# yosungho/LineTR

Hardware: AMD Instinct MI355X
Metric: line_descriptors_per_sec (higher is better)
Workload: dtype f32 in/out; GEMMs as 6 bf16-split MFMA products, fp32 accumulate (fp32-faithful); 1 GPU; cfg3: 64 pairs/GPU of 640x480, 200 lines/image -> 199 sub-lines x 21 tokens, d_model=256, seeded weights; pairs_per_gpu=64, collective=none

## Files before the change

include/linetr_hip.h:

```cpp
#ifndef LINETR_HIP_H
#define LINETR_HIP_H

#include <stdint.h>

#ifdef __cplusplus
extern "C" {
#endif

#define LINETR_ABI_VERSION 6

enum {
  LINETR_OK = 0,
  LINETR_E_ARG = -1,
  LINETR_E_HIP = -2,
  LINETR_E_WEIGHTS = -3,
  LINETR_E_ASSERT = -4,
  LINETR_E_WORKSPACE = -5,
  LINETR_E_CAPACITY = -6
};

typedef struct LinetrHandle LinetrHandle;

typedef struct {
  int32_t d_model;
  int32_t n_heads;
  int32_t d_inner;
  int32_t n_sig_layers;
  int32_t n_desc_layers;
  int32_t enc_channels[4];
  int32_t norm_height;
  int32_t norm_width;
  int32_t bn_batch_stats;
} LinetrModelConfig;

typedef struct {
  double sp[2];
  double ep[2];
  double length;
  double angle[2];
  int32_t first_sub;
  int32_t n_tok;
  int32_t n_sub;
  int32_t image;
  int32_t line_local;
  int32_t first_tok;
} LinetrLineRec;

typedef struct {
  float* klines;
  float* length;
  float* angles;
  float* sublines;
  float* pnt;
  float* mask;
  float* resp;
  float* angle_sub;
  float* desc;
  float* score;
  float* mat;
  const int32_t* h_cu_klines;
} LinetrTokens;


int linetr_abi_version(void);
const char* linetr_last_error(void);

int linetr_create(const LinetrModelConfig* cfg, int32_t n_tensors, const char* const* names,
                  const float* const* h_data, const int64_t* numel, int32_t device,
                  LinetrHandle** out);
void linetr_destroy(LinetrHandle* h);


int linetr_prefilter(const double* h_lines6, int32_t K, int32_t height, int32_t width, int32_t border,
                     double min_length, int32_t max_keylines, const double* h_valid_mask,
                     double token_distance, int32_t max_tokens, int32_t image_index, int32_t sub_base,
                     int32_t tok_base, LinetrLineRec* h_recs, int32_t capacity, int32_t* k_out, int32_t* n_out);

int linetr_prefilter_batch(const double* h_lines6, const int32_t* h_line_off, int32_t n_images, int32_t height,
                           int32_t width, int32_t border, double min_length, int32_t max_keylines,
                           const double* const* h_valid_masks, double token_distance, int32_t max_tokens,
                           int32_t n_threads, LinetrLineRec* h_recs, int32_t capacity, int32_t* h_cu_k,
                           int32_t* h_cu_n);

int32_t linetr_prefilter_tied_images(int32_t* h_images, int32_t capacity);

int linetr_pack_lines(const double* h_klines, const double* h_length, const double* h_angles, int32_t K,
                      double token_distance, int32_t max_tokens, int32_t image_index, int32_t sub_base,
                      int32_t tok_base, LinetrLineRec* h_recs, int32_t* n_out);


int64_t linetr_tokenize_workspace_bytes(int32_t n_images, int32_t height, int32_t width, int32_t N);

int linetr_tokenize(LinetrHandle* h, const LinetrLineRec* d_recs, int32_t K, int32_t N,
                    double token_distance, int32_t max_tokens, const float* d_dense_desc,
                    const float* d_dense_score, int32_t n_images, int32_t height, int32_t width,
                    int32_t clip_height, int32_t clip_width, int32_t align_corners, int32_t dense_is_nhwc,
                    LinetrTokens out, int32_t* d_sub2line, void* d_workspace, int64_t workspace_bytes, void* stream);

int64_t linetr_sample_descriptors_workspace_bytes(int32_t Hc, int32_t Wc, int32_t dense_is_nhwc);
int linetr_sample_descriptors(LinetrHandle* h, const float* d_points, int64_t n, const float* d_dense_desc, int32_t Hc,
                              int32_t Wc, int32_t align_corners, int32_t dense_is_nhwc, float* d_out, void* d_workspace,
                              int64_t workspace_bytes, void* stream);


int64_t linetr_forward_workspace_bytes(const LinetrHandle* h, int32_t N, int32_t max_tokens);

int linetr_forward(LinetrHandle* h, const LinetrTokens* tok, const int32_t* h_cu_sub, const int32_t* d_cu_sub,
                   int32_t n_images, int32_t max_tokens, float* d_line_desc, void* d_workspace,
                   int64_t workspace_bytes, void* stream);


int64_t linetr_bn_stats_floats(const LinetrHandle* h);
int64_t linetr_forward_train_workspace_bytes(const LinetrHandle* h, int32_t N, int32_t max_tokens);
int linetr_forward_train(LinetrHandle* h, const LinetrTokens* tok, const int32_t* h_cu_sub, const int32_t* d_cu_sub,
                         int32_t n_images, int32_t max_tokens, float momentum, float* d_bn_running, float* d_bn_batch,
                         float* d_line_desc, void* d_workspace, int64_t workspace_bytes, void* stream);

int64_t linetr_describe_workspace_bytes(const LinetrHandle* h, int32_t n_images, int32_t height, int32_t width,
                                        int32_t N, int64_t n_real_tokens);

int linetr_describe(LinetrHandle* h, const LinetrLineRec* d_recs, int32_t K, int32_t N, int64_t n_real_tokens,
                    const int32_t* h_cu_sub, const int32_t* d_cu_sub, int32_t n_images, double token_distance,
                    int32_t max_tokens, const float* d_dense_desc, const float* d_dense_score, int32_t height,
                    int32_t width, int32_t align_corners, int32_t dense_is_nhwc, LinetrTokens out,
                    int32_t* d_sub2line, float* d_line_desc, void* d_workspace, int64_t workspace_bytes,
                    void* stream);

int linetr_describe_submit(LinetrHandle* h, const LinetrLineRec* d_recs, int32_t K, int32_t N, int64_t n_real_tokens,
                           const int32_t* h_cu_sub, const int32_t* d_cu_sub, int32_t n_images, double token_distance,
                           int32_t max_tokens, const float* d_dense_desc, const float* d_dense_score, int32_t height,
                           int32_t width, int32_t align_corners, int32_t dense_is_nhwc, LinetrTokens out,
                           int32_t* d_sub2line, float* d_line_desc, void* d_workspace, int64_t workspace_bytes,
                           int32_t slot, int32_t n_slots, void* stream);
int32_t linetr_pipeline_max_slots(void);
int linetr_describe_join(LinetrHandle* h, int32_t slot, void* stream);


int64_t linetr_match_workspace_bytes(int32_t n_pairs, int64_t sum_n0n1, int64_t sum_k0k1, int64_t sum_k);

int linetr_match(LinetrHandle* h, int32_t n_pairs, const int32_t* h_dims, const float* d_desc0,
                 const int64_t* h_off_n0, const int32_t* d_sub2line0, const float* d_desc1,
                 const int64_t* h_off_n1, const int32_t* d_sub2line1, float nn_thresh, int32_t mutual,
                 float* d_dk, const int64_t* h_off_dk, int32_t* d_match01, const int64_t* h_off_k0,
                 void* d_workspace, int64_t workspace_bytes, void* stream);

int linetr_match_gathered(LinetrHandle* h, int32_t n_pairs, const int32_t* h_dims, const float* d_desc0,
                          const int64_t* h_off_n0, const int32_t* d_sub2line0, const int64_t* h_off_s0,
                          const float* d_desc1, const int64_t* h_off_n1, const int32_t* d_sub2line1,
                          const int64_t* h_off_s1, float nn_thresh, int32_t mutual, float* d_dk,
                          const int64_t* h_off_dk, int32_t* d_match01, const int64_t* h_off_k0, void* d_workspace,
                          int64_t workspace_bytes, void* stream);

int64_t linetr_match_distmat_workspace_bytes(int32_t n0, int32_t n1);
int linetr_match_distmat(LinetrHandle* h, const float* d_dist, int32_t n0, int32_t n1, float nn_thresh,
                         int32_t mutual, int32_t* d_match01, void* d_workspace, int64_t workspace_bytes,
                         void* stream);

int64_t linetr_match_distmat_f64_workspace_bytes(int32_t n0, int32_t n1);
int linetr_match_distmat_f64(LinetrHandle* h, const double* d_dist, int32_t n0, int32_t n1, double nn_thresh, int32_t mutual,
                             int32_t* d_match01, void* d_workspace, int64_t workspace_bytes, void* stream);

int64_t linetr_pool_distmat_workspace_bytes(int32_t k0, int32_t k1);
int linetr_pool_distmat(LinetrHandle* h, const float* d_dist, int32_t n0, int32_t n1, const int32_t* d_sub2line0, int32_t k0,
                        const int32_t* d_sub2line1, int32_t k1, float* d_dk, void* d_workspace, int64_t workspace_bytes,
                        void* stream);

int64_t linetr_pool_distmat_dense_workspace_bytes(int32_t k0, int32_t n0, int32_t k1, int32_t n1);
int linetr_pool_distmat_dense(LinetrHandle* h, const float* d_dist, int32_t n0, int32_t n1, const float* d_A0, int32_t k0,
                              const float* d_A1, int32_t k1, float* d_dk, void* d_workspace, int64_t workspace_bytes,
                              void* stream);

int linetr_match_points(LinetrHandle* h, const float* d_desc0_cn, int32_t n0, const float* d_desc1_cn,
                        int32_t n1, float nn_thresh, int32_t mutual, float* d_dist, int32_t* d_match01,
                        void* d_workspace, int64_t workspace_bytes, void* stream);

int64_t linetr_pair_tail_workspace_bytes(int32_t np0, int32_t np1, int32_t n0, int32_t k0, int32_t n1, int32_t k1);
int64_t linetr_pair_tail_output_bytes(int32_t np0, int32_t np1, int32_t k0, int32_t k1, int64_t* h_offsets);
int linetr_pair_tail(LinetrHandle* h, const float* d_pdesc0_cn, int32_t np0, const float* d_pdesc1_cn, int32_t np1, float nn_thresh_points,
                     const float* d_ldesc0, int32_t n0, const int32_t* d_sub2line0, int32_t k0, const float* d_ldesc1, int32_t n1,
                     const int32_t* d_sub2line1, int32_t k1, float nn_thresh_lines, int32_t mutual, void* h_pinned_out,
                     int64_t pinned_bytes, void* d_workspace, int64_t workspace_bytes, void* stream);


int64_t linetr_val_step_workspace_bytes(int32_t B, int32_t n);
int64_t linetr_val_step_output_bytes(int32_t B, int64_t* h_offsets);
int linetr_val_step(LinetrHandle* h, const float* d_desc0, int32_t n0, const float* d_desc1, int32_t n1, const float* d_assign, int32_t B,
                    double nn_thresh, int32_t mutual, float* d_row_pos, float* d_row_neg, int32_t* d_match01, void* h_pinned_out,
                    int64_t pinned_bytes, void* d_workspace, int64_t workspace_bytes, void* stream);

int linetr_assign_from_matches(LinetrHandle* h, const int32_t* d_lmatches, int32_t B, int32_t M, int32_t n, float* d_assign, void* stream);


enum { LINETR_COORD_F32 = 0, LINETR_COORD_F64 = 1 };
int64_t linetr_gt_assign_workspace_bytes(int32_t B, int32_t n0, int32_t n1);
int linetr_gt_assign(LinetrHandle* h, int32_t coord_type, const void* d_lines0, int32_t n0, const void* d_lines1, int32_t n1,
                     const double* d_H, int32_t B, const int32_t* d_count0, const int32_t* d_count1, double thres_reprojected,
                     double thres_angdiff, double min_overlap_ratio, int32_t pad, float* d_assign, int32_t* d_lmatches, int32_t M,
                     int32_t* d_found, uint8_t* d_match_dir, void* d_overlap_dir, void* d_proj0, void* d_proj1, void* d_workspace,
                     int64_t workspace_bytes, void* stream);


int linetr_superpoint_heads(LinetrHandle* h, const float* d_score_logits, const float* d_desc_raw, int32_t B,
                            int32_t Hc, int32_t Wc, float* d_dense_score, float* d_dense_desc_nhwc,
                            float* d_dense_desc_nchw, void* stream);


int64_t linetr_superpoint_keypoints_workspace_bytes(int32_t B, int32_t H, int32_t W, int32_t cap_per_image);
int linetr_superpoint_keypoints(LinetrHandle* h, const float* d_dense_score, int32_t B, int32_t H, int32_t W, int32_t nms_radius,
                                float keypoint_threshold, int32_t remove_borders, int32_t max_keypoints, int32_t cap_per_image,
                                float* d_keypoints, float* d_scores, int32_t* d_cu_kp, int32_t* d_found, void* d_workspace,
                                int64_t workspace_bytes, void* stream);

int64_t linetr_point_descriptors_workspace_bytes(int32_t B, int32_t Hc, int32_t Wc, int32_t dense_is_nhwc);
int linetr_point_descriptors(LinetrHandle* h, const float* d_keypoints, const int32_t* d_cu_kp, int32_t B, int64_t n_total,
                             const float* d_dense_desc, int32_t Hc, int32_t Wc, int32_t align_corners, int32_t dense_is_nhwc,
                             float* d_desc_cn, void* d_workspace, int64_t workspace_bytes, void* stream);


enum { LINETR_PREC_F32 = 0, LINETR_PREC_BF16X3 = 1, LINETR_PREC_BF16X6 = 2, LINETR_PREC_F16X3 = 3 };
int linetr_set_precision(LinetrHandle* h, int32_t mode);
int linetr_get_precision(const LinetrHandle* h);


int linetr_debug_posenc(LinetrHandle* h, int32_t which, const float* d_in0, const float* d_in1, const float* d_in2,
                           int64_t rows, float* d_out, void* stream);

int linetr_debug_gemm(LinetrHandle* h, const float* d_A, int32_t lda, const float* d_W, const float* d_bias,
                      const float* d_residual, float* d_Y, int32_t ldy, int32_t M, int32_t N, int32_t K,
                      int32_t act, int32_t cache_weights, void* stream);

#define LINETR_GEMM_TILE_WS 100
typedef struct {
  const float* A;   int32_t lda;
  const float* A2;  int32_t lda2;  int32_t K1;
  const float* W;
  const float* bias;
  const float* R;
  float* Y;         int32_t ldy;
  int32_t M, N, K, act;
  int32_t groups;   int64_t gA, gY;
  int32_t norm;     const float* gamma;  const float* beta;  const float* add2;  float eps;
  int32_t via_row_norm;
  int32_t tile;
} LinetrGemmCase;
int linetr_debug_gemm_case(LinetrHandle* h, const LinetrGemmCase* c, int32_t* tile_used, void* stream);

int linetr_debug_sig_attention(LinetrHandle* h, int32_t kernel, int32_t layer, const float* d_in, int32_t ld_in,
                               const int32_t* h_cu_sub, int32_t n_images, float* d_msg, int32_t* kernel_used, void* stream);

int linetr_debug_tok_mlp(LinetrHandle* h, int32_t variant, const float* d_pnt, const float* d_score, int64_t rows_word,
                         const float* d_sublines, const float* d_resp, const float* d_angle, int64_t rows_line,
                         float* d_out_word, float* d_out_line, int32_t max_blocks, int32_t* variant_used, void* stream);

int linetr_debug_cls_pool(LinetrHandle* h, int32_t kernel, const LinetrLineRec* d_recs, int32_t K, const int32_t* d_sub2line,
                          int32_t N, int32_t T, const float* d_cpnt, const float* d_a4, int64_t first_pad, int32_t n_images,
                          const float* d_map, int32_t dense_is_nhwc, int32_t Hc, int32_t Wc, int32_t align_corners,
                          const float* d_desc_dense, float* d_pooled, int32_t* kernel_used, void* stream);

#ifdef LINETR_EXPERIMENTS
int64_t linetr_st_bytes(int64_t rows, int32_t K);
int linetr_debug_to_st(LinetrHandle* h, const float* d_X, int32_t ld, int32_t rows, int32_t K, void* d_st, void* stream);
int linetr_debug_from_st(LinetrHandle* h, const void* d_st, int32_t rows, int32_t K, float* d_X, int32_t ld, void* stream);
int linetr_debug_gemm_st(LinetrHandle* h, const void* d_A1, int32_t K1, const void* d_A2, int32_t K2, const void* d_W,
                         const float* d_bias, const void* d_R, void* d_Yst, float* d_Y, int32_t ldy, int32_t M, int32_t N,
                         int32_t act, void* stream);
int linetr_debug_pairnet_stamps(LinetrHandle* h, unsigned long long* d_buf);
#endif

int linetr_allgather_desc(void* nccl_comm, const void* d_slab, void* d_out, int64_t slab_bytes, void* stream);

int linetr_set_allgather_fn(void* nccl_allgather_fn);

int linetr_pack_slab(const float* d_line_desc, int32_t N, const int32_t* d_cu_n, const int32_t* d_cu_k, int32_t n_images,
                     const int32_t* d_sub2line, int32_t n_images_cap, int32_t rows_cap, int32_t zero_tail, float* d_slab,
                     void* stream);


typedef struct {
  const char* name;
  int32_t calls;
  float ms;
  double flops;
  double bytes;
} LinetrProfileEntry;
int linetr_set_profiling(LinetrHandle* h, int32_t on);
int linetr_get_profile(LinetrHandle* h, LinetrProfileEntry* out, int32_t max_entries, int32_t* n_out);

#ifdef __cplusplus
}
#endif
#endif
```

linetr_amd/_native.py:

```python
from __future__ import annotations

import ctypes as C
import os

import numpy as np

_HERE = os.path.dirname(os.path.abspath(__file__))
LIB_PATH = os.path.join(_HERE, "csrc", "liblinetr_hip.so")
EXPERIMENTS_LIB_PATH = os.path.join(os.path.dirname(_HERE), "experiments", "liblinetr_hip_experiments.so")

E_ASSERT = -4


class ModelConfig(C.Structure):
    _fields_ = [("d_model", C.c_int32), ("n_heads", C.c_int32), ("d_inner", C.c_int32),
                ("n_sig_layers", C.c_int32), ("n_desc_layers", C.c_int32), ("enc_channels", C.c_int32 * 4),
                ("norm_height", C.c_int32), ("norm_width", C.c_int32), ("bn_batch_stats", C.c_int32)]


class LineRec(C.Structure):
    _fields_ = [("sp", C.c_double * 2), ("ep", C.c_double * 2), ("length", C.c_double),
                ("angle", C.c_double * 2), ("first_sub", C.c_int32), ("n_tok", C.c_int32),
                ("n_sub", C.c_int32), ("image", C.c_int32), ("line_local", C.c_int32), ("first_tok", C.c_int32)]


REC_DTYPE = np.dtype([("sp", "<f8", 2), ("ep", "<f8", 2), ("length", "<f8"), ("angle", "<f8", 2),
                      ("first_sub", "<i4"), ("n_tok", "<i4"), ("n_sub", "<i4"), ("image", "<i4"),
                      ("line_local", "<i4"), ("first_tok", "<i4")])
assert REC_DTYPE.itemsize == C.sizeof(LineRec) == 80


class Tokens(C.Structure):
    _fields_ = [(k, C.c_void_p) for k in ("klines", "length", "angles", "sublines", "pnt", "mask", "resp",
                                          "angle_sub", "desc", "score", "mat", "h_cu_klines")]


class GemmCase(C.Structure):
    _fields_ = [("A", C.c_void_p), ("lda", C.c_int32), ("A2", C.c_void_p), ("lda2", C.c_int32), ("K1", C.c_int32),
                ("W", C.c_void_p), ("bias", C.c_void_p), ("R", C.c_void_p), ("Y", C.c_void_p), ("ldy", C.c_int32),
                ("M", C.c_int32), ("N", C.c_int32), ("K", C.c_int32), ("act", C.c_int32), ("groups", C.c_int32),
                ("gA", C.c_int64), ("gY", C.c_int64), ("norm", C.c_int32), ("gamma", C.c_void_p), ("beta", C.c_void_p),
                ("add2", C.c_void_p), ("eps", C.c_float), ("via_row_norm", C.c_int32), ("tile", C.c_int32)]


class ProfileEntry(C.Structure):
    _fields_ = [("name", C.c_char_p), ("calls", C.c_int32), ("ms", C.c_float), ("flops", C.c_double),
                ("bytes", C.c_double)]


_libs = {}


def lib(path=None):
    import torch
    path = os.path.abspath(path or os.environ.get("LINETR_LIB", LIB_PATH))
    if path in _libs:
        return _libs[path]
    if not os.path.exists(path):
        raise RuntimeError(
            f"{path} is missing: the HIP extension has not been built (run `python -m linetr_amd.build`). "
            "linetr_amd has no CPU fallback.")
    L = C.CDLL(path)
    vp, i32, i64, f64, f32 = C.c_void_p, C.c_int32, C.c_int64, C.c_double, C.c_float
    L.linetr_abi_version.restype = i32
    L.linetr_last_error.restype = C.c_char_p
    L.linetr_create.argtypes = [C.POINTER(ModelConfig), i32, C.POINTER(C.c_char_p), C.POINTER(vp), C.POINTER(i64), i32,
                                C.POINTER(vp)]
    L.linetr_destroy.argtypes = [vp]
    L.linetr_destroy.restype = None
    L.linetr_prefilter.argtypes = [vp, i32, i32, i32, i32, f64, i32, vp, f64, i32, i32, i32, i32, vp, i32, C.POINTER(i32),
                                   C.POINTER(i32)]
    L.linetr_prefilter_batch.argtypes = [vp, vp, i32, i32, i32, i32, f64, i32, vp, f64, i32, i32, vp, i32, vp, vp]
    L.linetr_prefilter_tied_images.argtypes = [vp, i32]
    L.linetr_prefilter_tied_images.restype = i32
    L.linetr_pack_lines.argtypes = [vp, vp, vp, i32, f64, i32, i32, i32, i32, vp, C.POINTER(i32)]
    L.linetr_describe_workspace_bytes.argtypes = [vp, i32, i32, i32, i32, i64]
    L.linetr_describe_workspace_bytes.restype = i64
    L.linetr_describe.argtypes = [vp, vp, i32, i32, i64, vp, vp, i32, f64, i32, vp, vp, i32, i32, i32, i32, Tokens, vp, vp,
                                  vp, i64, vp]
    L.linetr_describe_submit.argtypes = [vp, vp, i32, i32, i64, vp, vp, i32, f64, i32, vp, vp, i32, i32, i32, i32, Tokens, vp, vp,
                                         vp, i64, i32, i32, vp]
    L.linetr_describe_join.argtypes = [vp, i32, vp]
    L.linetr_pipeline_max_slots.argtypes = []
    L.linetr_tokenize_workspace_bytes.argtypes = [i32, i32, i32, i32]
    L.linetr_tokenize_workspace_bytes.restype = i64
    L.linetr_tokenize.argtypes = [vp, vp, i32, i32, f64, i32, vp, vp, i32, i32, i32, i32, i32, i32, i32, Tokens, vp, vp, i64, vp]
    L.linetr_forward_workspace_bytes.argtypes = [vp, i32, i32]
    L.linetr_forward_workspace_bytes.restype = i64
    L.linetr_forward.argtypes = [vp, C.POINTER(Tokens), vp, vp, i32, i32, vp, vp, i64, vp]
    L.linetr_bn_stats_floats.argtypes = [vp]
    L.linetr_bn_stats_floats.restype = i64
    L.linetr_forward_train_workspace_bytes.argtypes = [vp, i32, i32]
    L.linetr_forward_train_workspace_bytes.restype = i64
    L.linetr_forward_train.argtypes = [vp, C.POINTER(Tokens), vp, vp, i32, i32, f32, vp, vp, vp, vp, i64, vp]
    L.linetr_match_workspace_bytes.argtypes = [i32, i64, i64, i64]
    L.linetr_match_workspace_bytes.restype = i64
    L.linetr_match.argtypes = [vp, i32, vp, vp, vp, vp, vp, vp, vp, f32, i32, vp, vp, vp, vp, vp, i64, vp]
    L.linetr_match_gathered.argtypes = [vp, i32, vp, vp, vp, vp, vp, vp, vp, vp, vp, f32, i32, vp, vp, vp, vp, vp, i64, vp]
    L.linetr_match_points.argtypes = [vp, vp, i32, vp, i32, f32, i32, vp, vp, vp, i64, vp]
    L.linetr_match_distmat.argtypes = [vp, vp, i32, i32, f32, i32, vp, vp, i64, vp]
    L.linetr_match_distmat_workspace_bytes.argtypes = [i32, i32]
    L.linetr_match_distmat_workspace_bytes.restype = i64
    L.linetr_match_distmat_f64.argtypes = [vp, vp, i32, i32, f64, i32, vp, vp, i64, vp]
    L.linetr_match_distmat_f64_workspace_bytes.argtypes = [i32, i32]
    L.linetr_match_distmat_f64_workspace_bytes.restype = i64
    L.linetr_pair_tail_workspace_bytes.argtypes = [i32, i32, i32, i32, i32, i32]
    L.linetr_pair_tail_workspace_bytes.restype = i64
    L.linetr_pair_tail_output_bytes.argtypes = [i32, i32, i32, i32, vp]
    L.linetr_pair_tail_output_bytes.restype = i64
    L.linetr_pair_tail.argtypes = [vp, vp, i32, vp, i32, f32, vp, i32, vp, i32, vp, i32, vp, i32, f32, i32, vp, i64, vp, i64, vp]
    L.linetr_val_step_workspace_bytes.argtypes = [i32, i32]
    L.linetr_val_step_workspace_bytes.restype = i64
    L.linetr_val_step_output_bytes.argtypes = [i32, vp]
    L.linetr_val_step_output_bytes.restype = i64
    L.linetr_val_step.argtypes = [vp, vp, i32, vp, i32, vp, i32, f64, i32, vp, vp, vp, vp, i64, vp, i64, vp]
    L.linetr_assign_from_matches.argtypes = [vp, vp, i32, i32, i32, vp, vp]
    L.linetr_gt_assign_workspace_bytes.argtypes = [i32, i32, i32]
    L.linetr_gt_assign_workspace_bytes.restype = i64
    L.linetr_gt_assign.argtypes = [vp, i32, vp, i32, vp, i32, vp, i32, vp, vp, f64, f64, f64, i32, vp, vp, i32, vp, vp, vp, vp, vp, vp,
                                   i64, vp]
    L.linetr_superpoint_heads.argtypes = [vp, vp, vp, i32, i32, i32, vp, vp, vp, vp]
    L.linetr_superpoint_keypoints_workspace_bytes.argtypes = [i32, i32, i32, i32]
    L.linetr_superpoint_keypoints_workspace_bytes.restype = i64
    L.linetr_superpoint_keypoints.argtypes = [vp, vp, i32, i32, i32, i32, f32, i32, i32, i32, vp, vp, vp, vp, vp, i64, vp]
    L.linetr_point_descriptors_workspace_bytes.argtypes = [i32, i32, i32, i32]
    L.linetr_point_descriptors_workspace_bytes.restype = i64
    L.linetr_point_descriptors.argtypes = [vp, vp, vp, i32, i64, vp, i32, i32, i32, i32, vp, vp, i64, vp]
    L.linetr_set_precision.argtypes = [vp, i32]
    L.linetr_get_precision.argtypes = [vp]
    L.linetr_debug_posenc.argtypes = [vp, i32, vp, vp, vp, i64, vp, vp]
    L.linetr_debug_gemm.argtypes = [vp, vp, i32, vp, vp, vp, vp, i32, i32, i32, i32, i32, i32, vp]
    L.linetr_debug_gemm_case.argtypes = [vp, C.POINTER(GemmCase), vp, vp]
    L.linetr_debug_sig_attention.argtypes = [vp, i32, i32, vp, i32, vp, i32, vp, vp, vp]
    L.linetr_debug_tok_mlp.argtypes = [vp, i32, vp, vp, i64, vp, vp, vp, i64, vp, vp, i32, vp, vp]
    L.linetr_debug_cls_pool.argtypes = [vp, i32, vp, i32, vp, i32, i32, vp, vp, i64, i32, vp, i32, i32, i32, i32, vp, vp, vp, vp]
    if hasattr(L, "linetr_debug_gemm_st"):
        L.linetr_st_bytes.argtypes = [i64, i32]
        L.linetr_st_bytes.restype = i64
        L.linetr_debug_to_st.argtypes = [vp, vp, i32, i32, i32, vp, vp]
        L.linetr_debug_from_st.argtypes = [vp, vp, i32, i32, vp, i32, vp]
        L.linetr_debug_gemm_st.argtypes = [vp, vp, i32, vp, i32, vp, vp, vp, vp, vp, i32, i32, i32, i32, vp]
        L.linetr_debug_pairnet_stamps.argtypes = [vp, vp]
    L.linetr_allgather_desc.argtypes = [vp, vp, vp, i64, vp]
    L.linetr_set_allgather_fn.argtypes = [vp]
    L.linetr_pack_slab.argtypes = [vp, i32, vp, vp, i32, vp, i32, i32, i32, vp, vp]
    L.linetr_sample_descriptors_workspace_bytes.argtypes = [i32, i32, i32]
    L.linetr_sample_descriptors_workspace_bytes.restype = i64
    L.linetr_sample_descriptors.argtypes = [vp, vp, i64, vp, i32, i32, i32, i32, vp, vp, i64, vp]
    L.linetr_pool_distmat_workspace_bytes.argtypes = [i32, i32]
    L.linetr_pool_distmat_workspace_bytes.restype = i64
    L.linetr_pool_distmat.argtypes = [vp, vp, i32, i32, vp, i32, vp, i32, vp, vp, i64, vp]
    L.linetr_pool_distmat_dense_workspace_bytes.argtypes = [i32, i32, i32, i32]
    L.linetr_pool_distmat_dense_workspace_bytes.restype = i64
    L.linetr_pool_distmat_dense.argtypes = [vp, vp, i32, i32, vp, i32, vp, i32, vp, vp, i64, vp]
    L.linetr_set_profiling.argtypes = [vp, i32]
    L.linetr_get_profile.argtypes = [vp, C.POINTER(ProfileEntry), i32, C.POINTER(i32)]
    if L.linetr_abi_version() != 6:
        raise RuntimeError("liblinetr_hip.so ABI version mismatch")
    _libs[path] = L
    return L


EXPORTS = ["linetr_abi_version", "linetr_last_error", "linetr_create", "linetr_destroy", "linetr_prefilter",
           "linetr_prefilter_batch", "linetr_prefilter_tied_images", "linetr_pack_lines", "linetr_tokenize_workspace_bytes", "linetr_tokenize", "linetr_forward_workspace_bytes",
           "linetr_forward", "linetr_bn_stats_floats", "linetr_forward_train_workspace_bytes", "linetr_forward_train", "linetr_describe_workspace_bytes", "linetr_describe", "linetr_describe_submit", "linetr_describe_join", "linetr_pipeline_max_slots", "linetr_match_workspace_bytes", "linetr_match", "linetr_match_gathered", "linetr_match_points",
           "linetr_match_distmat", "linetr_match_distmat_workspace_bytes", "linetr_match_distmat_f64", "linetr_match_distmat_f64_workspace_bytes", "linetr_pair_tail_workspace_bytes", "linetr_pair_tail_output_bytes", "linetr_pair_tail", "linetr_val_step_workspace_bytes", "linetr_val_step_output_bytes", "linetr_val_step", "linetr_assign_from_matches", "linetr_gt_assign_workspace_bytes", "linetr_gt_assign", "linetr_superpoint_heads", "linetr_superpoint_keypoints_workspace_bytes", "linetr_superpoint_keypoints",
           "linetr_point_descriptors_workspace_bytes", "linetr_point_descriptors", "linetr_set_precision", "linetr_get_precision", "linetr_debug_posenc", "linetr_debug_gemm", "linetr_debug_gemm_case", "linetr_debug_sig_attention", "linetr_debug_tok_mlp", "linetr_debug_cls_pool", "linetr_allgather_desc", "linetr_set_allgather_fn", "linetr_pack_slab", "linetr_sample_descriptors_workspace_bytes",
           "linetr_sample_descriptors", "linetr_pool_distmat_workspace_bytes", "linetr_pool_distmat", "linetr_pool_distmat_dense_workspace_bytes", "linetr_pool_distmat_dense", "linetr_set_profiling", "linetr_get_profile"]


EXPERIMENT_EXPORTS = ["linetr_st_bytes", "linetr_debug_to_st", "linetr_debug_from_st", "linetr_debug_gemm_st", "linetr_debug_pairnet_stamps"]


class NativeError(RuntimeError):
    pass


def check(code: int, L=None):
    if code == 0:
        return
    msg = (L if L is not None else lib()).linetr_last_error().decode("utf-8", "replace")
    if code == E_ASSERT:
        raise AssertionError(msg)
    raise NativeError(f"liblinetr_hip error {code}: {msg}")


def np_ptr(a: np.ndarray):
    return a.ctypes.data_as(C.c_void_p)
```

linetr_amd/csrc/linetr_net.hip:

```cpp
#include <algorithm>
#include <array>
#include <numeric>
#include <set>

#include "lt_handle.h"
#include "lt_gemm.h"
#include "lt_gemm_split.h"
#include "lt_gemm_split16.h"
#include "lt_st_image.h"
#include "lt_gemm_small.h"
#include "lt_model.h"
#include "lt_attn.h"
#include "lt_attn_fused.h"
#include "lt_gemm_ws.h"
#include "lt_tokmlp.h"
#include "lt_token.h"
#include "lt_bntrain.h"

using namespace lt;

namespace {

const char* gemm_class_name(int precision, int tile, const GemmArgs& g, int groups) {
  static const auto names = [] {
    const char* kind[4] = {"gemm_f32", "gemm_bf16x3", "gemm_bf16x6", "gemm_f16x3"};
    std::array<std::array<std::string, (int)SplitTile::count>, 4> n;
    for (int p = 0; p < 4; ++p)
      for (int t = 0; t < (p ? (int)SplitTile::count : (int)F32Tile::count); ++t)
        n[p][t] = std::string(kind[p]) + "_" + (p ? tile_name((SplitTile)t) : tile_name((F32Tile)t));
    return n;
  }();
  const std::string& name = names[precision][tile];
  static const bool by_shape = LT_XENV("LINETR_PROFILE_SHAPES") != nullptr;
  if (!by_shape) return name.c_str();
  static std::mutex mu;
  static std::set<std::string> shapes;
  char buf[160];
  snprintf(buf, sizeof buf, "%s[M=%d,N=%d,K=%d,g=%d]", name.c_str(), g.M, g.N, g.K, groups);
  std::lock_guard<std::mutex> lock(mu);
  return shapes.insert(buf).first->c_str();
}

struct GemmA { const float* p; int ld; const float* p2 = nullptr; int ld2 = 0, K1 = 0; };
struct GemmY { float* p; int ld; };
struct GemmGroups { int n, N; int64_t gA, gY; };

struct NormSpec {
  int mode = 0;
  const float* gamma = nullptr;
  const float* beta = nullptr;
  const float* add2 = nullptr;
  float eps = 0.f;
};

#ifdef LINETR_EXPERIMENTS
int x_gemm(LinetrHandle*, hipStream_t, SplitGemmArgs& sa, const GemmW& w, int groups, const NormSpec*, double fl, double by, bool& done);
int x_split_weights(LinetrHandle* H, std::vector<GemmWSpec>& weights);
int64_t x_ws_bytes(const LinetrHandle* h, int N);
#endif

int gemm_args(const GemmW& w, int M, const GemmA& A, const GemmY& Y, int act, const float* R, const GemmGroups* grp,
              const NormSpec* ns, GemmArgs& g) {
  const int groups = grp ? grp->n : 1, N = grp ? grp->N : w.rows;
  if (A.p2 && (A.K1 <= 0 || A.K1 >= w.K)) return fail(LINETR_E_ARG, "gemm: split point K1 = %d outside (0, K = %d)", A.K1, w.K);
  if ((int64_t)N * groups > w.rows) return fail(LINETR_E_ARG, "gemm: %d groups of %d rows exceed the weight's %d", groups, N, w.rows);
  if (groups > 1 && (R || ns)) return fail(LINETR_E_ARG, "gemm: a grouped launch takes no residual and no row normalisation");
  g = GemmArgs{};
  g.A = A.p; g.lda = A.ld; g.A2 = A.p2; g.lda2 = A.ld2; g.K1 = A.K1;
  g.W = w.W; g.ldw = w.K; g.bias = w.b; g.R = R; g.ldr = Y.ld; g.Y = Y.p; g.ldy = Y.ld;
  g.M = M; g.N = N; g.K = w.K; g.act = act;
  if (grp) { g.gA = grp->gA; g.gW = (int64_t)N * w.K; g.gBias = N; g.gY = grp->gY; }
  if (ns) { g.norm = ns->mode; g.gamma = ns->gamma; g.beta = ns->beta; g.add2 = ns->add2; g.ldadd2 = D; g.eps = ns->eps; }
  return LINETR_OK;
}

bool gemm_ws_able(const LinetrHandle* h, const GemmArgs& g, const GemmW& w, int groups, const NormSpec* fused_norm) {
  return h->precision == LINETR_PREC_BF16X6 && groups == 1 && !g.A2 && !g.R && !fused_norm && w.st &&
         gemm_ws_can(g.N, g.K, g.lda, g.ldy, g.act);
}
bool gemm_ws_takes(const LinetrHandle* h, const GemmArgs& g, const GemmW& w, int groups, const NormSpec* fused_norm) {
  return gemm_ws_able(h, g, w, groups, fused_norm) && gemm_ws_fits(g.M, g.N, g.K, g.lda, g.ldy, g.act) && !LT_XENV("LINETR_NO_GEMM_WS");
}

struct GemmForce { int tile = -1; int* used = nullptr; bool launch = true; };

int run_gemm(LinetrHandle* h, hipStream_t st, const GemmW& w, int M, const GemmA& A, const GemmY& Y, int act, const float* R = nullptr,
             const GemmGroups* grp = nullptr, const NormSpec* fused_norm = nullptr, const GemmForce* force = nullptr) {
  GemmArgs g;
  if (int e = gemm_args(w, M, A, Y, act, R, grp, fused_norm, g)) return e;
  const int groups = grp ? grp->n : 1;
  const int forced = force ? force->tile : -1;
  const bool launch = !force || force->launch;
  auto report = [&](int tile) { if (force && force->used) *force->used = tile; };
  const double fl = 2.0 * M * (double)g.N * g.K * groups;
  const double by = 4.0 * groups * ((double)M * g.K + (double)g.N * g.K + (double)M * g.N);
  if (h->precision == LINETR_PREC_F32) {
    if (forced >= (int)F32Tile::count) return fail(LINETR_E_ARG, "gemm: the f32 mode has no tile %d", forced);
    if (fused_norm) return fail(LINETR_E_ARG, "gemm: the f32 kernels have no fused row normalisation");
    const F32Tile tile = f32_tile_launched(g, forced < 0 ? f32_tile(g, groups) : (F32Tile)forced);
    report((int)tile);
    if (!launch) return LINETR_OK;
    ProfScope ps(h, st, gemm_class_name(LINETR_PREC_F32, (int)tile, g, groups), fl, by);
    return gemm_launch(g, groups, tile, st);
  }
  SplitGemmArgs sa;
  sa.g = g;
#ifdef LINETR_EXPERIMENTS
  if (!force) {
    bool done = false;
    if (int e = x_gemm(h, st, sa, w, groups, fused_norm, fl, by, done); e || done) return e;
  }
#endif
  if (forced == LINETR_GEMM_TILE_WS && !gemm_ws_able(h, g, w, groups, fused_norm))
    return fail(LINETR_E_ARG, "gemm: the weight-stationary kernel runs act(A[M,128] W[256,128]^T + b) in bf16x6 only, act none / ReLU");
  if (forced == LINETR_GEMM_TILE_WS || (forced < 0 && gemm_ws_takes(h, g, w, groups, fused_norm))) {
    report(LINETR_GEMM_TILE_WS);
    if (!launch) return LINETR_OK;
    WsGemmArgs a;
    a.A = A.p; a.lda = A.ld; a.Wst = w.st; a.bias = w.b ? w.b : h->zeros; a.Y = Y.p; a.ldy = Y.ld; a.M = M; a.act = act;
    ProfScope ps(h, st, "gemm_bf16x6_ws64x256", fl, by);
    return gemm_ws_launch(a, st);
  }
  const int pl = h->precision == LINETR_PREC_BF16X6 ? 3 : 2;
  SplitTile tile;
  if (forced >= (int)SplitTile::count) return fail(LINETR_E_ARG, "gemm: no split tile %d", forced);
  if (forced >= 0) tile = (SplitTile)forced;
  else if (int e = pick_split_tile(g, groups, pl, tile)) return e;
  if (int e = split_tile_launched(g, groups, pl, tile)) return e;
  report((int)tile);
  if (!launch) return LINETR_OK;
  ProfScope ps(h, st, gemm_class_name(h->precision, (int)tile, g, groups), fl, by);
  switch (h->precision) {
    case LINETR_PREC_BF16X3: sa.Wsp = w.s2; sa.gWsp = g.gW * 4; return gemm_split_launch<2>(sa, groups, tile, st);
    case LINETR_PREC_F16X3: sa.Wsp = w.h2; sa.gWsp = g.gW * 4; return gemm_split_launch<2, 1>(sa, groups, tile, st);
    default: sa.Wsp = w.s3; sa.gWsp = g.gW * 6; return gemm_split_launch<3>(sa, groups, tile, st);
  }
}

bool gemm_norm_fuses(const LinetrHandle* h, const GemmW& w, int M, const GemmA& A, const float* R, float* Y) {
  GemmArgs g;
  return !LT_XENV("LINETR_NO_FUSED_NORM") && h->precision != LINETR_PREC_F32 && !LT_XENV("LINETR_GEMM_TILE") &&
         !gemm_args(w, M, A, {Y, D}, ACT_NONE, R, nullptr, nullptr, g) &&
         split_tile(g, 1, h->precision == LINETR_PREC_BF16X6 ? 3 : 2) == SplitTile::t128x256;
}

int row_norm(LinetrHandle* h, hipStream_t st, const float* x, int M, const NormSpec& ns, float* Y) {
  ProfScope ps(h, st, "row_norm", 0, (double)M * D * (ns.add2 ? 12 : 8));
  hipLaunchKernelGGL(row_norm_kernel, dim3(cdiv(M, 4)), dim3(256), 0, st, x, M, ns.mode == 2 ? 1 : 0, ns.gamma, ns.beta,
                     ns.add2, ns.eps, Y);
  LT_LAUNCH_CHECK();
  return 0;
}

int run_gemm_norm(LinetrHandle* h, hipStream_t st, const GemmW& w, int M, const GemmA& A, const float* R, float* tmp, float* Y,
                  const NormSpec& ns) {
  if (w.rows != D) return fail(LINETR_E_ARG, "gemm_norm: the weight has %d rows, not %d", w.rows, D);
  if (gemm_norm_fuses(h, w, M, A, R, Y)) return run_gemm(h, st, w, M, A, {Y, D}, ACT_NONE, R, nullptr, &ns);
  if (int e = run_gemm(h, st, w, M, A, {tmp, D}, ACT_NONE, R)) return e;
  return row_norm(h, st, tmp, M, ns, Y);
}

struct SplitOffsets { int64_t s2, s3, h2, st = -1; };
SplitOffsets split_offsets(int64_t rows, int K, bool with_st, int64_t& off) {
  SplitOffsets o;
  o.s2 = off; off += align_up(rows * K * 4, 256);
  o.s3 = off; off += align_up(rows * K * 6, 256);
  o.h2 = off; off += align_up(rows * K * 4, 256);
  if (with_st) { off = align_up(off, 1024); o.st = off; off += st_bytes(rows, K); }
  return o;
}

void split_copies(GemmW& w, unsigned char* base, const SplitOffsets& o, bool make, hipStream_t st) {
  w.s2 = base + o.s2; w.s3 = base + o.s3; w.h2 = base + o.h2;
  w.st = o.st >= 0 ? base + o.st : nullptr;
  if (!make) return;
  const dim3 grid((unsigned)cdiv((int)((int64_t)w.rows * w.K / 4), 256));
  hipLaunchKernelGGL(split_rows_kernel<2>, grid, dim3(256), 0, st, w.W, base + o.s2, (int64_t)w.rows, w.K);
  hipLaunchKernelGGL(split_rows_kernel<3>, grid, dim3(256), 0, st, w.W, base + o.s3, (int64_t)w.rows, w.K);
  hipLaunchKernelGGL((split_rows_kernel<2, 1>), grid, dim3(256), 0, st, w.W, base + o.h2, (int64_t)w.rows, w.K);
  if (o.st >= 0) {
    const int64_t thr = st_row_blocks(w.rows) * (w.K / 16) * 32;
    hipLaunchKernelGGL(to_st_kernel, dim3((unsigned)((thr + 255) / 256)), dim3(256), 0, st, w.W, w.K, w.rows, w.K / 16, base + o.st);
  }
}

}

int lt::make_split_copies(LinetrHandle* H, std::vector<GemmWSpec> weights) {
#ifdef LINETR_EXPERIMENTS
  if (int e = x_split_weights(H, weights)) return e;
#endif
  int64_t total = 0;
  std::vector<SplitOffsets> at;
  for (auto& s : weights) at.push_back(split_offsets(s.w->rows, s.w->K, s.st && s.w->rows % 16 == 0 && s.w->K % 32 == 0, total));
  LT_HIP(hipMalloc((void**)&H->split_arena, total));
  LT_HIP(hipMalloc((void**)&H->zeros, 4096 * sizeof(float)));
  LT_HIP(hipMemset(H->zeros, 0, 4096 * sizeof(float)));
  for (size_t i = 0; i < weights.size(); ++i) split_copies(*weights[i].w, H->split_arena, at[i], true, 0);
  LT_LAUNCH_CHECK();
  LT_HIP(hipDeviceSynchronize());
  return LINETR_OK;
}


namespace {
int k2s_table(const LinetrTokens& out, int n_images, int K, int N, const int32_t* h_cu_sub, K2sTable& tab, const char* who) {
  tab = K2sTable{};
  if (!out.mat) return 0;
  if (n_images > K2S_MAX_IMAGES) return fail(LINETR_E_ARG, "%s: mat_klines2sublines is written for calls of up to %d images", who, K2S_MAX_IMAGES);
  if (n_images == 1) {
    for (int i = 0; i < K2S_MAX_IMAGES; ++i) tab.img[i] = K2sImage{0, N, 0};
    return 0;
  }
  if (!out.h_cu_klines || !h_cu_sub) return fail(LINETR_E_ARG, "%s: mat_klines2sublines of several images needs the host prefix sums of key-lines and sub-lines", who);
  if (out.h_cu_klines[n_images] != K) return fail(LINETR_E_ARG, "%s: h_cu_klines does not end at K", who);
  int64_t off = 0;
  for (int i = 0; i < n_images; ++i) {
    const int ki = out.h_cu_klines[i + 1] - out.h_cu_klines[i], ni = h_cu_sub[i + 1] - h_cu_sub[i];
    if (ki < 0 || ni < 0) return fail(LINETR_E_ARG, "%s: prefix sums not monotone", who);
    tab.img[i] = K2sImage{off, ni, h_cu_sub[i]};
    off += (int64_t)ki * ni;
  }
  return 0;
}

int nhwc_map(LinetrHandle* h, hipStream_t st, const float* dense_desc, int dense_is_nhwc, int n_images, int P, float* buf,
             const float*& nhwc) {
  nhwc = dense_desc;
  if (dense_is_nhwc) return LINETR_OK;
  ProfScope ps(h, st, "nchw_to_nhwc", 0, 2.0 * n_images * P * D * 4);
  hipLaunchKernelGGL(nchw_to_nhwc_kernel, dim3(cdiv(P, 64), D / 64, n_images), dim3(256), 0, st, dense_desc, buf, D, P);
  LT_LAUNCH_CHECK();
  nhwc = buf;
  return LINETR_OK;
}

struct TokenFront {
  const LinetrLineRec* recs; int K, N; double td; int T;
  const float *dense_desc, *dense_score;
  int n_images, height, width, align_corners, dense_is_nhwc;
  double clip_x, clip_y;
  float *sublines, *resp, *angle_sub;
  int* s2l_g;
  float* nhwc_buf;
  bool map_always;
  double tokenize_bytes;
  float *cpnt = nullptr, *cscore = nullptr; int n_pad_images = 0; int64_t first_pad = 0;
};
int token_front(LinetrHandle* h, hipStream_t st, const TokenFront& a, const LinetrTokens& out, const K2sTable& k2s, int32_t* d_sub2line,
                const float*& nhwc) {
  {
    ProfScope ps(h, st, "line_fill", 0, (double)a.K * 80 + (double)a.N * 8);
    hipLaunchKernelGGL(line_fill_kernel, dim3(cdiv(a.K, 256)), dim3(256), 0, st, a.recs, a.K, a.clip_x, a.clip_y, out.klines, out.length,
                       out.angles, a.s2l_g, d_sub2line);
    LT_LAUNCH_CHECK();
  }
  {
    ProfScope ps(h, st, "tokenize", 0, a.tokenize_bytes);
    hipLaunchKernelGGL(tokenize_kernel, dim3(a.N + cdiv(a.n_pad_images, 64) + (out.mat ? a.K : 0)), dim3(64), 0, st, a.recs, a.s2l_g, a.N,
                       a.td, a.T, a.height, a.width, a.clip_x, a.clip_y, a.dense_score, a.sublines, out.pnt, out.mask, a.resp, a.angle_sub,
                       out.score, a.cpnt, a.cscore, a.n_pad_images, a.first_pad, out.mat, k2s);
    LT_LAUNCH_CHECK();
  }
  const int Hc = a.height / 8, Wc = a.width / 8;
  nhwc = nullptr;
  if (a.map_always || out.desc)
    if (int e = nhwc_map(h, st, a.dense_desc, a.dense_is_nhwc, a.n_images, Hc * Wc, a.nhwc_buf, nhwc)) return e;
  if (out.desc) {
    const int64_t ntok = (int64_t)a.N * a.T;
    ProfScope ps(h, st, "sample_desc", 0, (double)ntok * D * 4 * 2);
    hipLaunchKernelGGL(sample_desc_kernel, dim3((unsigned)((ntok + 3) / 4)), dim3(256), 0, st, out.pnt, a.s2l_g, a.recs, ntok, a.T, nhwc,
                       Hc, Wc, a.align_corners, out.desc);
    LT_LAUNCH_CHECK();
  }
  return LINETR_OK;
}
}

extern "C" int64_t linetr_tokenize_workspace_bytes(int32_t n_images, int32_t height, int32_t width, int32_t N) {
  const int64_t P = (int64_t)(height / 8) * (width / 8);
  return align_up(n_images * P * D * 4, 256) + align_up((int64_t)std::max(N, 1) * 4, 256) + 256;
}

extern "C" int linetr_tokenize(LinetrHandle* h, const LinetrLineRec* d_recs, int32_t K, int32_t N, double td,
                               int32_t T, const float* d_dense_desc, const float* d_dense_score, int32_t n_images,
                               int32_t height, int32_t width, int32_t clip_height, int32_t clip_width, int32_t align_corners,
                               int32_t dense_is_nhwc, LinetrTokens out, int32_t* d_sub2line, void* d_ws, int64_t ws_bytes,
                               void* stream) {
  if (K <= 0 || N <= 0) return LINETR_OK;
  if (clip_height <= 0) clip_height = height;
  if (clip_width <= 0) clip_width = width;
  if (!d_recs || !d_dense_score || !out.sublines || !out.pnt || !out.mask || !out.resp || !out.angle_sub ||
      !out.score || (out.desc && !d_dense_desc))
    return fail(LINETR_E_ARG, "tokenize: null pointer");
  if (T < 1 || T > 4096 || height % 8 || width % 8) return fail(LINETR_E_ARG, "tokenize: bad max_tokens / image size");
  if (out.mat && n_images != 1) return fail(LINETR_E_ARG, "tokenize: mat_klines2sublines of several images: use linetr_describe (it has the sub-line prefix sums)");
  K2sTable k2s;
  if (int e = k2s_table(out, n_images, K, N, nullptr, k2s, "tokenize")) return e;
  if (ws_bytes < linetr_tokenize_workspace_bytes(n_images, height, width, N))
    return fail(LINETR_E_WORKSPACE, "tokenize: workspace too small");
  hipStream_t st = (hipStream_t)stream;
  if (h) LT_HIP(hipSetDevice(h->device));
  const int64_t P = (int64_t)(height / 8) * (width / 8);
  TokenFront f{d_recs, K, N, td, T, d_dense_desc, d_dense_score, n_images, height, width, align_corners, dense_is_nhwc,
               (double)clip_width - 0.6, (double)clip_height - 0.6, out.sublines, out.resp, out.angle_sub};
  f.nhwc_buf = (float*)d_ws;
  f.s2l_g = (int*)((char*)d_ws + align_up(n_images * P * D * 4, 256));
  f.map_always = false;
  f.tokenize_bytes = (double)N * T * 16;
  const float* nhwc;
  return token_front(h, st, f, out, k2s, d_sub2line, nhwc);
}

extern "C" int64_t linetr_sample_descriptors_workspace_bytes(int32_t Hc, int32_t Wc, int32_t dense_is_nhwc) {
  return dense_is_nhwc ? 0 : align_up((int64_t)Hc * Wc * D * 4, 256);
}

extern "C" int linetr_sample_descriptors(LinetrHandle* h, const float* d_points, int64_t n, const float* d_dense_desc, int32_t Hc,
                                         int32_t Wc, int32_t align_corners, int32_t dense_is_nhwc, float* d_out, void* d_ws,
                                         int64_t ws_bytes, void* stream) {
  if (n < 0 || Hc <= 0 || Wc <= 0) return fail(LINETR_E_ARG, "sample_descriptors: bad shape");
  if (n == 0) return LINETR_OK;
  if (!d_points || !d_dense_desc || !d_out) return fail(LINETR_E_ARG, "sample_descriptors: null pointer");
  if (ws_bytes < linetr_sample_descriptors_workspace_bytes(Hc, Wc, dense_is_nhwc) || (!dense_is_nhwc && !d_ws))
    return fail(LINETR_E_WORKSPACE, "sample_descriptors: workspace too small");
  hipStream_t st = (hipStream_t)stream;
  if (h) LT_HIP(hipSetDevice(h->device));
  const float* nhwc;
  if (int e = nhwc_map(h, st, d_dense_desc, dense_is_nhwc, 1, Hc * Wc, (float*)d_ws, nhwc)) return e;
  ProfScope ps(h, st, "sample_desc", 0, (double)n * D * 4 * 2);
  hipLaunchKernelGGL(sample_desc_kernel, dim3((unsigned)((n + 3) / 4)), dim3(256), 0, st, d_points, (const int*)nullptr,
                     (const LinetrLineRec*)nullptr, n, 1, nhwc, Hc, Wc, align_corners, d_out);
  LT_LAUNCH_CHECK();
  return LINETR_OK;
}

extern "C" int64_t linetr_point_descriptors_workspace_bytes(int32_t B, int32_t Hc, int32_t Wc, int32_t dense_is_nhwc) {
  return dense_is_nhwc ? 0 : align_up((int64_t)std::max(B, 0) * std::max(Hc, 0) * std::max(Wc, 0) * D * 4, 256);
}

extern "C" int linetr_point_descriptors(LinetrHandle* h, const float* d_keypoints, const int32_t* d_cu_kp, int32_t B, int64_t n_total,
                                        const float* d_dense_desc, int32_t Hc, int32_t Wc, int32_t align_corners, int32_t dense_is_nhwc,
                                        float* d_desc_cn, void* d_ws, int64_t ws_bytes, void* stream) {
  if (B < 0 || n_total < 0 || Hc <= 0 || Wc <= 0 || n_total > INT32_MAX) return fail(LINETR_E_ARG, "point_descriptors: bad shape");
  if (B == 0 || n_total == 0) return LINETR_OK;
  if (!d_keypoints || !d_cu_kp || !d_dense_desc || !d_desc_cn) return fail(LINETR_E_ARG, "point_descriptors: null pointer");
  if (ws_bytes < linetr_point_descriptors_workspace_bytes(B, Hc, Wc, dense_is_nhwc) || (!dense_is_nhwc && !d_ws))
    return fail(LINETR_E_WORKSPACE, "point_descriptors: workspace too small");
  hipStream_t st = (hipStream_t)stream;
  if (h) LT_HIP(hipSetDevice(h->device));
  LT_HIP(allow_dynamic_lds<sp_kp_desc_kernel>((int)KP_DESC_LDS));
  const float* nhwc;
  if (int e = nhwc_map(h, st, d_dense_desc, dense_is_nhwc, B, Hc * Wc, (float*)d_ws, nhwc)) return e;
  ProfScope ps(h, st, "sp_kp_desc", 0, (double)n_total * D * 4 * 5);
  hipLaunchKernelGGL(sp_kp_desc_kernel, dim3((unsigned)((n_total + KP_DESC_N - 1) / KP_DESC_N + B)), dim3(256), KP_DESC_LDS, st, d_keypoints,
                     d_cu_kp, B, nhwc, Hc, Wc, align_corners, d_desc_cn);
  LT_LAUNCH_CHECK();
  return LINETR_OK;
}


namespace {
constexpr int SIG_FOLD_MAX_ROWS = 960;
struct FwdWs {
  float* act[2][4];
  float *pooled, *att, *fc, *o, *f1, *f2, *lpos, *zA, *zB, *qkv, *msgp, *msg, *hid;
  float *zqA, *zqB;
  int* cu;
  char* x = nullptr;
  int64_t total;
};
FwdWs fwd_layout(const LinetrHandle* h, int N, int64_t rows, int n_images, char* base) {
  const LinetrModelConfig& c = h->cfg;
  FwdWs w;
  int64_t off = 0;
  auto take = [&](int64_t floats) { float* p = (float*)(base + off); off += align_up(floats * 4, 256); return p; };
  for (int i = 0; i < 4; ++i) w.act[ENC_WORD][i] = take(rows * c.enc_channels[i]);
  w.pooled = take((int64_t)N * HEADS * POOLW);
  w.att = take((int64_t)N * D); w.fc = take((int64_t)N * D); w.o = take((int64_t)N * D);
  w.f1 = take((int64_t)N * c.d_inner); w.f2 = take((int64_t)N * D);
  for (int i = 0; i < 4; ++i) w.act[ENC_LINE][i] = take((int64_t)N * c.enc_channels[i]);
  w.lpos = take((int64_t)N * D);
  w.zA = take((int64_t)N * D); w.zB = take((int64_t)N * D);
  w.qkv = take((int64_t)N * 3 * D); w.msgp = take((int64_t)N * D); w.msg = take((int64_t)N * D);
  w.hid = take((int64_t)N * 2 * D);
  const int64_t nq = N <= SIG_FOLD_MAX_ROWS ? (int64_t)N * 4 * D : 0;
  w.zqA = take(nq); w.zqB = take(nq);
  w.cu = (int*)take(n_images + 1);
#ifdef LINETR_EXPERIMENTS
  w.x = base + off; off += x_ws_bytes(h, N);
#endif
  w.total = off;
  return w;
}
}

extern "C" int64_t linetr_forward_workspace_bytes(const LinetrHandle* h, int32_t N, int32_t T) {
  if (!h) return -1;
  return fwd_layout(h, std::max(N, 1), (int64_t)std::max(N, 1) * T, std::max(N, 1), nullptr).total;
}

namespace {
enum {
  CUT_TOKENS = 0,
  CUT_MLP = 1,
  CUT_POOL = 2,
  CUT_SENTENCE = 3,
  CUT_SIG0 = 4
};
struct PipeStages {
  hipStream_t stream[LinetrHandle::PIPE_STREAMS];
  hipEvent_t ev[LinetrHandle::PIPE_STREAMS - 1];
  int cut[LinetrHandle::PIPE_STREAMS - 1];
  int n_cuts = 0, next = 0;
};
int pipe_boundary(PipeStages* p, int pos, hipStream_t& st) {
  if (!p || p->next >= p->n_cuts || p->cut[p->next] != pos) return LINETR_OK;
  LT_HIP(hipEventRecord(p->ev[p->next], st));
  LT_HIP(hipStreamWaitEvent(p->stream[p->next + 1], p->ev[p->next], 0));
  st = p->stream[++p->next];
  return LINETR_OK;
}

struct TokenStage {
  const float *pnt = nullptr, *score = nullptr, *desc = nullptr;
  const float *cpnt = nullptr, *cscore = nullptr, *nhwc = nullptr;
  const LinetrLineRec* recs = nullptr;
  const int* sub2line_g = nullptr;
  int64_t rows = 0;
  int64_t first_pad = 0;
  int Hc = 0, Wc = 0, align_corners = 0;
  const BnTrain* bn = nullptr;
  PipeStages* pipe = nullptr;
};

bool fused_mlp_enabled(const LinetrModelConfig& c) { return c.enc_channels[1] == 64 && c.enc_channels[2] == 128; }

int mlp123_rows_per_wave(int64_t rows) {
  const int64_t waves = 256 * 4;
  return (int)std::max<int64_t>(cdiv((int)cdiv((int)rows, (int)waves), 32) * 32, 32);
}

double attn_flops(const int32_t* h_cu, int n_images) {
  double fl = 0;
  for (int i = 0; i < n_images; ++i) { const double n = h_cu[i + 1] - h_cu[i]; fl += 2.0 * 2.0 * n * n * D; }
  return fl;
}

struct EncCall {
  int which;
  const float *p0, *p1, *p2;
  int64_t rows;
  float* const* act;
};
constexpr struct { int in, in_bytes; const char *tok_mlp, *mlp123; } ENC_KIND[2] = {{3, 12, "tok_mlp_bf16x6", "mlp123"},
                                                                                   {5, 28, "line_mlp_bf16x6", "mlp123_line"}};

struct EncNorm { float cx, cy, scale; };
EncNorm enc_norm(const LinetrModelConfig& c) {
  return {c.norm_width / 2.f, c.norm_height / 2.f, (float)std::max(c.norm_width, c.norm_height) * 0.7f};
}

template <bool RELU>
int enc_layer1(LinetrHandle* h, hipStream_t st, const EncCall& c, float* out) {
  const PosEncoder& E = h->enc[c.which];
  const EncNorm n = enc_norm(h->cfg);
  const dim3 grid((unsigned)cdiv((int)(c.rows * 8), 256));
  if (c.which == ENC_WORD)
    hipLaunchKernelGGL(word_mlp1_kernel<RELU>, grid, dim3(256), 0, st, c.p0, c.p1, c.rows, n.cx, n.cy, n.scale, E.W1, E.b1, out);
  else
    hipLaunchKernelGGL(line_mlp1_kernel<RELU>, grid, dim3(256), 0, st, c.p0, c.p1, c.p2, (int)c.rows, n.cx, n.cy, n.scale, E.W1, E.b1, out);
  LT_LAUNCH_CHECK();
  return LINETR_OK;
}

int enc_mlp123(LinetrHandle* h, hipStream_t st, const EncCall& c, float* out) {
  const PosEncoder& E = h->enc[c.which];
  const EncNorm n = enc_norm(h->cfg);
  const int rpw = mlp123_rows_per_wave(c.rows);
  const dim3 grid((unsigned)cdiv((int)cdiv((int)c.rows, rpw), 4));
  if (c.which == ENC_WORD)
    hipLaunchKernelGGL(mlp123_kernel<true>, grid, dim3(256), 0, st, c.p0, c.p1, c.p2, c.rows, rpw, n.cx, n.cy, n.scale, E.W1, E.b1,
                       E.W2.W, E.W2.b, E.W3.W, E.W3.b, out);
  else
    hipLaunchKernelGGL(mlp123_kernel<false>, grid, dim3(256), 0, st, c.p0, c.p1, c.p2, c.rows, rpw, n.cx, n.cy, n.scale, E.W1, E.b1,
                       E.W2.W, E.W2.b, E.W3.W, E.W3.b, out);
  LT_LAUNCH_CHECK();
  return LINETR_OK;
}

TokMlpArgs tok_mlp_args(const LinetrHandle* h, const EncCall& c) {
  const PosEncoder& E = h->enc[c.which];
  const EncNorm n = enc_norm(h->cfg);
  TokMlpArgs a;
  a.p0 = c.p0; a.p1 = c.p1; a.p2 = c.p2; a.rows = c.rows; a.cx = n.cx; a.cy = n.cy; a.scale = n.scale;
  a.W1 = E.W1; a.b1 = E.b1; a.W2st = E.W2.st; a.b2 = E.W2.b; a.W3st = E.W3.st; a.b3 = E.W3.b; a.W4st = E.W4.st; a.b4 = E.W4.b;
  a.Y = c.act[3]; a.ldy = h->cfg.enc_channels[3];
  return a;
}

int pos_encoder(LinetrHandle* h, hipStream_t st, const EncCall& c, bool tok_mlp) {
  const int *ch = h->cfg.enc_channels, e0 = ch[0], e1 = ch[1], e2 = ch[2], e3 = ch[3];
  const PosEncoder& E = h->enc[c.which];
  const auto& kind = ENC_KIND[c.which];
  const int64_t rows = c.rows;
  int e;
  if (tok_mlp) {
    ProfScope ps(h, st, kind.tok_mlp, 2.0 * rows * (kind.in * e0 + e0 * e1 + e1 * e2 + e2 * e3), (double)rows * (kind.in_bytes + 4 * e3));
    return tok_mlp_launch(tok_mlp_args(h, c), c.which == ENC_WORD, st);
  }
  if (fused_mlp_enabled(h->cfg)) {
    ProfScope ps(h, st, kind.mlp123, 2.0 * rows * (kind.in * e0 + e0 * e1 + e1 * e2), (double)rows * (kind.in_bytes + 4 * e2));
    if ((e = enc_mlp123(h, st, c, c.act[2]))) return e;
  } else {
    {
      ProfScope ps(h, st, "mlp_first", 2.0 * rows * kind.in * e0, (double)rows * (kind.in_bytes + 4 * e0));
      if ((e = enc_layer1<true>(h, st, c, c.act[0]))) return e;
    }
    if ((e = run_gemm(h, st, E.W2, (int)rows, {c.act[0], e0}, {c.act[1], e1}, ACT_RELU))) return e;
    if ((e = run_gemm(h, st, E.W3, (int)rows, {c.act[1], e1}, {c.act[2], e2}, ACT_RELU))) return e;
  }
  return run_gemm(h, st, E.W4, (int)rows, {c.act[2], e2}, {c.act[3], e3}, ACT_RELU);
}

int pos_encoder_bn(LinetrHandle* h, hipStream_t st, const EncCall& c, const BnTrain& bt, int64_t& off) {
  const PosEncoder& E = h->enc[c.which];
  const GemmW* const W[4] = {nullptr, &E.W2, &E.W3, &E.W4};
  const int* ch = h->cfg.enc_channels;
  int e;
  for (int i = 0; i < 4; ++i) {
    e = i == 0 ? enc_layer1<false>(h, st, c, c.act[0])
               : run_gemm(h, st, *W[i], (int)c.rows, {c.act[i - 1], ch[i - 1]}, {c.act[i], ch[i]}, ACT_NONE);
    if (e) return e;
    const int layer = 4 * c.which + i;
    if ((e = bn_train_layer(st, bt, c.act[i], c.rows, ch[i], ch[i], h->bn_g[layer], h->bn_b[layer], off))) return e;
    off += 2 * ch[i];
  }
  return LINETR_OK;
}

enum { TOKV_WORD = 0, TOKV_LINE = 1, TOKV_DUAL = 2, TOKV_SEQ = 3, TOKV_CHAIN = 4 };
struct TokMlpPlan { bool word, line; int both; };
bool tok_mlp_has_images(const PosEncoder& E) { return E.W2.st && E.W3.st && E.W4.st; }
TokMlpPlan tok_mlp_plan(const LinetrHandle* h, int64_t rows_word, int64_t rows_line) {
  const int* ch = h->cfg.enc_channels;
  const bool ok = fused_mlp_enabled(h->cfg) && h->precision == LINETR_PREC_BF16X6 && ch[0] == 32 && ch[1] == 64 && ch[2] == 128 && ch[3] == 256 &&
                  !LT_XENV("LINETR_NO_TOKMLP");
  TokMlpPlan p;
  p.word = ok && tok_mlp_has_images(h->enc[ENC_WORD]);
  p.line = ok && tok_mlp_has_images(h->enc[ENC_LINE]);
  p.both = !(p.word && p.line && rows_word > 0 && rows_line > 0) ? -1 : tok_mlp_dual_fits(rows_word, rows_line) ? TOKV_DUAL : TOKV_SEQ;
  return p;
}

int pos_encoders(LinetrHandle* h, hipStream_t& st, const TokenStage& ts, const float* sublines, const float* resp,
                 const float* angle_sub, int N, FwdWs& w) {
  const LinetrModelConfig& c = h->cfg;
  const int e0 = c.enc_channels[0], e1 = c.enc_channels[1], e2 = c.enc_channels[2], e3 = c.enc_channels[3];
  const EncCall word{ENC_WORD, ts.cpnt ? ts.cpnt : ts.pnt, ts.cpnt ? ts.cscore : ts.score, nullptr, ts.rows, w.act[ENC_WORD]};
  const EncCall line{ENC_LINE, sublines, resp, angle_sub, N, w.act[ENC_LINE]};
  const int64_t rows = ts.rows;
  int e;
  const TokMlpPlan plan = tok_mlp_plan(h, rows, N);
  if (ts.bn) {
    int64_t off = 0;
    if ((e = pos_encoder_bn(h, st, word, *ts.bn, off))) return e;
    if ((e = pos_encoder_bn(h, st, line, *ts.bn, off))) return e;
  } else if (plan.both >= 0) {
    ProfScope ps(h, st, "pos_mlp_dual_bf16x6", 2.0 * rows * (3 * e0 + e0 * e1 + e1 * e2 + e2 * e3) + 2.0 * N * (5 * e0 + e0 * e1 + e1 * e2 + e2 * e3),
                 (double)rows * (12 + 4 * e3) + (double)N * (28 + 4 * e3));
    if ((e = tok_mlp_launch_dual(tok_mlp_args(h, word), tok_mlp_args(h, line), st))) return e;
  } else {
    if ((e = pos_encoder(h, st, word, plan.word))) return e;
    if ((e = pos_encoder(h, st, line, plan.line))) return e;
  }
  return run_gemm(h, st, h->lW5, N, {w.act[ENC_LINE][3], e3}, {w.lpos, D}, ACT_NONE);
}

enum { POOLK_DENSE = 0, POOLK_ONLINE = 1, POOLK_ONLINE_REV = 2, POOLK_SPLIT4 = 3 };
int cls_pool_plan(bool online, int N) { return !online ? POOLK_DENSE : N <= 2048 ? POOLK_SPLIT4 : POOLK_ONLINE_REV; }

int cls_pool_launch(LinetrHandle* h, hipStream_t st, int kernel, const TokenStage& ts, int n_images, int N, int T, const float* a4,
                    float* pooled) {
  const int64_t rows = ts.rows;
  if (kernel != POOLK_DENSE) {
    const double tap_bytes = std::min((double)n_images * ts.Hc * ts.Wc * D * 4, (double)rows * D * 4 * 4);
    ProfScope ps(h, st, "cls_pool_online", 2.0 * rows * (2.0 * HEADS * D * 2), tap_bytes + (double)rows * D * 4 + (double)N * HEADS * POOLW * 4);
    if (kernel == POOLK_SPLIT4)
      hipLaunchKernelGGL(cls_pool_online_kernel<4>, dim3(N), dim3(256), 0, st, ts.recs, ts.sub2line_g, ts.cpnt,
                         a4, ts.first_pad, N, T, ts.nhwc, ts.Hc, ts.Wc, ts.align_corners, h->pool, pooled, 0);
    else
      hipLaunchKernelGGL(cls_pool_online_kernel<1>, dim3(cdiv(N, 4)), dim3(256), 0, st, ts.recs, ts.sub2line_g, ts.cpnt,
                         a4, ts.first_pad, N, T, ts.nhwc, ts.Hc, ts.Wc, ts.align_corners, h->pool, pooled, kernel == POOLK_ONLINE_REV ? 1 : 0);
    LT_LAUNCH_CHECK();
  } else {
    ProfScope ps(h, st, "cls_pool", 2.0 * rows * (2.0 * HEADS * D * 2), (double)rows * D * 8);
    hipLaunchKernelGGL(cls_pool_kernel, dim3(N), dim3(256), HEADS * (T + 1) * sizeof(float), st, ts.desc, a4, T, h->pool, pooled);
    LT_LAUNCH_CHECK();
  }
  return LINETR_OK;
}

int cls_pooling(LinetrHandle* h, hipStream_t& st, const TokenStage& ts, int n_images, int N, int T, FwdWs& w) {
  if (int e = cls_pool_launch(h, st, cls_pool_plan(ts.cpnt != nullptr, N), ts, n_images, N, T, w.act[ENC_WORD][3], w.pooled)) return e;
  const GemmGroups heads{HEADS, DH, POOLW, DH};
  return run_gemm(h, st, h->Watt, N, {w.pooled, HEADS * POOLW}, {w.att, D}, ACT_NONE, nullptr, &heads);
}

int sentence(LinetrHandle* h, hipStream_t& st, int N, FwdWs& w) {
  const LinetrModelConfig& c = h->cfg;
  int e;
  {
    NormSpec ns; ns.mode = 1; ns.gamma = h->ln1g; ns.beta = h->ln1b; ns.eps = 1e-6f;
    if ((e = run_gemm_norm(h, st, h->Wfc, N, {w.att, D}, nullptr, w.fc, w.o, ns))) return e;
  }
  if ((e = run_gemm(h, st, h->Wf1, N, {w.o, D}, {w.f1, c.d_inner}, ACT_GELU))) return e;
  NormSpec ns; ns.mode = 1; ns.gamma = h->ln2g; ns.beta = h->ln2b; ns.add2 = w.lpos; ns.eps = 1e-6f;
  return run_gemm_norm(h, st, h->Wf2, N, {w.f1, c.d_inner}, w.o, w.f2, w.zA, ns);
}

enum { SIGK_F32 = 0, SIGK_SMALL = 1, SIGK_SPLIT4 = 2, SIGK_SPLIT8 = 3, SIGK_FUSED = 4 };
struct SigAttnPlan {
  int attn;
  bool fold_next, fused;
  int kernel() const { return fused ? SIGK_FUSED : attn; }
};
SigAttnPlan sig_attn_plan(const LinetrHandle* h, int n_images, int N, int max_n) {
  SigAttnPlan p;
  const bool small_attn = h->precision != LINETR_PREC_F32 && (int64_t)n_images * HEADS * cdiv(max_n, 256) < 64;
  p.attn = h->precision == LINETR_PREC_F32 ? SIGK_F32 : small_attn ? SIGK_SMALL : max_n <= 128 ? SIGK_SPLIT4 : SIGK_SPLIT8;
  p.fold_next = small_attn && N <= SIG_FOLD_MAX_ROWS && !LT_XENV("LINETR_NO_SIG_FOLD");
  p.fused = !p.fold_next && !LT_XENV("LINETR_NO_FUSED_QKV_ATTN") && h->precision == LINETR_PREC_BF16X6 && max_n <= 256 &&
            (int64_t)n_images * HEADS >= 128;
  return p;
}

int sig_attention(LinetrHandle* h, hipStream_t st, int kernel, const float* qkv, int ldq, const int* cu_dev, int n_images, int N,
                  int max_n, double fl, float* msg) {
  if (kernel == SIGK_F32) {
    ProfScope ps(h, st, "sig_attn", fl, (double)N * D * 16);
    hipLaunchKernelGGL(sig_attn_kernel, dim3(n_images, HEADS, cdiv(max_n, ATT_QT)), dim3(256), 0, st, qkv, cu_dev, msg);
  } else {
    ProfScope ps(h, st, "sig_attn_bf16x6", fl, (double)N * D * 16);
    if (kernel == SIGK_SMALL)
      hipLaunchKernelGGL(sig_attn_small_kernel, dim3(n_images, HEADS, cdiv(max_n, 32)), dim3(256), 0, st, qkv, cu_dev, msg, ldq);
    else if (kernel == SIGK_SPLIT4)
      hipLaunchKernelGGL(sig_attn_split_kernel<4>, dim3(n_images, HEADS, cdiv(max_n, ATT_QT)), dim3(256), 0, st, qkv, cu_dev, msg);
    else
      hipLaunchKernelGGL(sig_attn_split_kernel<8>, dim3(n_images, HEADS, cdiv(max_n, 256)), dim3(512), 0, st, qkv, cu_dev, msg);
  }
  LT_LAUNCH_CHECK();
  return LINETR_OK;
}

int sig_qkv_attention(LinetrHandle* h, hipStream_t st, const SigLayer& S, const float* z, const int* cu_dev, int n_images, int N,
                      double attn_fl, float* msg) {
  LT_HIP(allow_dynamic_lds<sig_qkv_attn_kernel>(FQA_LDS));
  ProfScope ps(h, st, "sig_qkv_attn_bf16x6", 2.0 * N * 3.0 * D * D + attn_fl, (double)N * D * 8);
  hipLaunchKernelGGL(sig_qkv_attn_kernel, dim3(n_images, HEADS), dim3(512), FQA_LDS, st, z, S.Wqkv.st, S.Wqkv.b,
                     cu_dev, msg);
  LT_LAUNCH_CHECK();
  return LINETR_OK;
}

int sig_network(LinetrHandle* h, hipStream_t& st, const TokenStage& ts, const int32_t* h_cu, const int* cu_dev, int n_images, int N,
                float* d_line_desc, FwdWs& w) {
  const LinetrModelConfig& c = h->cfg;
  int max_n = 0;
  for (int i = 0; i < n_images; ++i) max_n = std::max(max_n, h_cu[i + 1] - h_cu[i]);
  int e;
  const double attn_fl = attn_flops(h_cu, n_images);
  const int64_t sig_bn_off = 4 * (int64_t)(c.enc_channels[0] + c.enc_channels[1] + c.enc_channels[2] + c.enc_channels[3]);
  const SigAttnPlan plan = sig_attn_plan(h, n_images, N, max_n);
  const bool fold_next = plan.fold_next, fused_qkv_attn = plan.fused;
  float *z = w.zA, *zn = w.zB;
  int ldz = D;
  float *zq = w.zqA, *zq_next = w.zqB;
  const float* qkv = w.qkv;
  int ldq = 3 * D;
  for (size_t l = 0; l < h->sig.size(); ++l) {
    const SigLayer& S = h->sig[l];
    if (fused_qkv_attn && S.Wqkv.st) {
      if ((e = sig_qkv_attention(h, st, S, z, cu_dev, n_images, N, attn_fl, w.msgp))) return e;
    } else {
      if (!fold_next || l == 0)
        if ((e = run_gemm(h, st, S.Wqkv, N, {z, ldz}, {w.qkv, 3 * D}, ACT_NONE))) return e;
      if ((e = sig_attention(h, st, plan.attn, qkv, ldq, cu_dev, n_images, N, max_n, attn_fl, w.msgp))) return e;
    }
    if ((e = run_gemm(h, st, S.W1, N, {z, ldz, w.msgp, D, D}, {w.hid, 2 * D}, ts.bn ? ACT_NONE : ACT_RELU))) return e;
    if (ts.bn && (e = bn_train_layer(st, *ts.bn, w.hid, N, 2 * D, 2 * D, h->bn_g[8 + l], h->bn_b[8 + l], sig_bn_off + (int64_t)l * 4 * D))) return e;
    if (l + 1 == h->sig.size()) break;
    if (fold_next) {
      if ((e = run_gemm(h, st, S.Wnext, N, {z, ldz, w.hid, 2 * D, D}, {zq, 4 * D}, ACT_NONE))) return e;
      z = zq; ldz = 4 * D; qkv = zq + D; ldq = 4 * D;
      std::swap(zq, zq_next);
    } else {
      if ((e = run_gemm(h, st, S.W2, N, {w.hid, 2 * D}, {zn, D}, ACT_NONE, z))) return e;
      std::swap(z, zn);
    }
    if ((e = pipe_boundary(ts.pipe, CUT_SIG0 + (int)l, st))) return e;
  }
  NormSpec l2; l2.mode = 2;
  if (h->sig.empty()) return run_gemm_norm(h, st, h->Wfin, N, {z, D}, nullptr, zn, d_line_desc, l2);
  return run_gemm_norm(h, st, h->Wfin2, N, {z, ldz, w.hid, 2 * D, D}, nullptr, zn, d_line_desc, l2);
}
}

#ifdef LINETR_EXPERIMENTS
#include "lt_x_net.h"
#endif

namespace {
int forward_core(LinetrHandle* h, hipStream_t st, const TokenStage& ts, const float* sublines, const float* resp,
                 const float* angle_sub, const int32_t* h_cu, const int* cu_dev, int n_images, int N, int T,
                 float* d_line_desc, FwdWs& w) {
  int e;
#ifdef LINETR_EXPERIMENTS
  XPath xp;
  if ((e = x_begin(h, st, n_images, N, h_cu, w, xp))) return e;
#endif
  if ((e = pos_encoders(h, st, ts, sublines, resp, angle_sub, N, w))) return e;
  if ((e = pipe_boundary(ts.pipe, CUT_MLP, st))) return e;
  if ((e = cls_pooling(h, st, ts, n_images, N, T, w))) return e;
  if ((e = pipe_boundary(ts.pipe, CUT_POOL, st))) return e;
#ifdef LINETR_EXPERIMENTS
  if (xp != X_NONE) return x_rest(h, st, ts, h_cu, cu_dev, n_images, N, d_line_desc, w, xp);
#endif
  if ((e = sentence(h, st, N, w))) return e;
  if ((e = pipe_boundary(ts.pipe, CUT_SENTENCE, st))) return e;
  return sig_network(h, st, ts, h_cu, cu_dev, n_images, N, d_line_desc, w);
}

int check_cu(const int32_t* h_cu, int n_images) {
  if (!h_cu || n_images < 1) return fail(LINETR_E_ARG, "null / empty cu_sub");
  if (h_cu[0] != 0) return fail(LINETR_E_ARG, "cu_sub[0] != 0");
  for (int i = 0; i < n_images; ++i)
    if (h_cu[i + 1] < h_cu[i]) return fail(LINETR_E_ARG, "cu_sub not monotone");
  return 0;
}

int cu_on_device(const int32_t* h_cu, const int32_t* d_cu, int n_images, const FwdWs& w, hipStream_t st, const int*& cu_dev) {
  cu_dev = d_cu;
  if (cu_dev) return LINETR_OK;
  LT_HIP(hipMemcpyAsync(w.cu, h_cu, (n_images + 1) * sizeof(int), hipMemcpyHostToDevice, st));
  cu_dev = w.cu;
  return LINETR_OK;
}

int forward_dense(LinetrHandle* h, const char* who, const LinetrTokens& tok, const int32_t* h_cu, const int32_t* d_cu, int n_images,
                  int T, float* d_line_desc, void* d_ws, int64_t ws_bytes, hipStream_t st, BnTrain* bt) {
  if (int e = check_cu(h_cu, n_images)) return e;
  const int N = h_cu[n_images];
  if (N <= 0) return LINETR_OK;
  if (!tok.sublines || !tok.pnt || !tok.resp || !tok.angle_sub || !tok.desc || !tok.score || !d_line_desc)
    return fail(LINETR_E_ARG, "%s: null tensor", who);
  if (ws_bytes < (bt ? linetr_forward_train_workspace_bytes(h, N, T) : linetr_forward_workspace_bytes(h, N, T)))
    return fail(LINETR_E_WORKSPACE, "%s: workspace too small", who);
  if ((int64_t)N * T > INT32_MAX / 8) return fail(LINETR_E_ARG, "%s: batch too large", who);
  LT_HIP(hipSetDevice(h->device));
  FwdWs w = fwd_layout(h, N, (int64_t)N * T, std::max(N, 1), (char*)d_ws);
  if (bt) {
    bt->partial = (double*)((char*)d_ws + align_up(w.total, 256));
    bt->affine = (float*)((char*)bt->partial + (int64_t)BN_MAX_BLOCKS * 2 * BN_MAX_CHANNELS * 8);
  }
  const int* cu_dev;
  if (int e = cu_on_device(h_cu, d_cu, n_images, w, st, cu_dev)) return e;
  TokenStage ts;
  ts.pnt = tok.pnt; ts.score = tok.score; ts.desc = tok.desc; ts.rows = (int64_t)N * T;
  ts.bn = bt;
  return forward_core(h, st, ts, tok.sublines, tok.resp, tok.angle_sub, h_cu, cu_dev, n_images, N, T, d_line_desc, w);
}
}

extern "C" int linetr_forward(LinetrHandle* h, const LinetrTokens* tok, const int32_t* h_cu, const int32_t* d_cu,
                              int32_t n_images, int32_t T, float* d_line_desc, void* d_ws, int64_t ws_bytes,
                              void* stream) {
  if (!h || !tok) return fail(LINETR_E_ARG, "forward: null argument");
  if (h->cfg.bn_batch_stats) return fail(LINETR_E_ARG, "forward: a training-mode handle (bn_batch_stats = 1) runs linetr_forward_train only");
  return forward_dense(h, "forward", *tok, h_cu, d_cu, n_images, T, d_line_desc, d_ws, ws_bytes, (hipStream_t)stream, nullptr);
}

extern "C" int64_t linetr_bn_stats_floats(const LinetrHandle* h) {
  if (!h) return -1;
  const LinetrModelConfig& c = h->cfg;
  return 4 * (int64_t)(c.enc_channels[0] + c.enc_channels[1] + c.enc_channels[2] + c.enc_channels[3]) + (int64_t)c.n_sig_layers * 4 * D;
}

extern "C" int64_t linetr_forward_train_workspace_bytes(const LinetrHandle* h, int32_t N, int32_t T) {
  if (!h) return -1;
  return linetr_forward_workspace_bytes(h, N, T) + (int64_t)BN_MAX_BLOCKS * 2 * BN_MAX_CHANNELS * 8 + 2 * BN_MAX_CHANNELS * 4 + 512;
}

extern "C" int linetr_forward_train(LinetrHandle* h, const LinetrTokens* tok, const int32_t* h_cu, const int32_t* d_cu, int32_t n_images,
                                    int32_t T, float momentum, float* d_bn_running, float* d_bn_batch, float* d_line_desc, void* d_ws,
                                    int64_t ws_bytes, void* stream) {
  if (!h || !tok) return fail(LINETR_E_ARG, "forward_train: null argument");
  if (!h->cfg.bn_batch_stats) return fail(LINETR_E_ARG, "forward_train: the handle was created for inference (bn_batch_stats = 0)");
  if (!d_bn_running) return fail(LINETR_E_ARG, "forward_train: null running statistics");
  if (!(momentum >= 0.f && momentum <= 1.f)) return fail(LINETR_E_ARG, "forward_train: momentum out of [0, 1]");
  BnTrain bt;
  bt.running = d_bn_running; bt.batch = d_bn_batch; bt.momentum = momentum;
  return forward_dense(h, "forward_train", *tok, h_cu, d_cu, n_images, T, d_line_desc, d_ws, ws_bytes, (hipStream_t)stream, &bt);
}


namespace {
struct DescWs { float *nhwc, *cpnt, *cscore, *sublines, *resp, *angle_sub; int* s2l_g; int64_t fwd_off, total; };
DescWs desc_layout(int n_images, int height, int width, int N, int64_t rows, char* base) {
  DescWs d;
  int64_t off = 0;
  auto take = [&](int64_t bytes) { char* p = base + off; off += align_up(bytes, 256); return p; };
  const int64_t P = (int64_t)(height / 8) * (width / 8);
  d.nhwc = (float*)take(n_images * P * D * 4);
  d.cpnt = (float*)take(rows * 8);
  d.cscore = (float*)take(rows * 4);
  d.sublines = (float*)take((int64_t)N * 16);
  d.resp = (float*)take((int64_t)N * 4);
  d.angle_sub = (float*)take((int64_t)N * 8);
  d.s2l_g = (int*)take((int64_t)N * 4);
  d.fwd_off = off;
  d.total = off;
  return d;
}
}

extern "C" int64_t linetr_describe_workspace_bytes(const LinetrHandle* h, int32_t n_images, int32_t height, int32_t width,
                                                   int32_t N, int64_t n_real) {
  if (!h) return -1;
  const int64_t rows = n_real + n_images;
  return desc_layout(n_images, height, width, std::max(N, 1), rows, nullptr).total +
         fwd_layout(h, std::max(N, 1), rows, n_images, nullptr).total;
}

namespace {
int describe_impl(LinetrHandle* h, const LinetrLineRec* d_recs, int32_t K, int32_t N, int64_t n_real,
                  const int32_t* h_cu, const int32_t* d_cu, int32_t n_images, double td, int32_t T,
                  const float* d_dense_desc, const float* d_dense_score, int32_t height, int32_t width,
                  int32_t align_corners, int32_t dense_is_nhwc, const LinetrTokens& out, int32_t* d_sub2line,
                  float* d_line_desc, void* d_ws, int64_t ws_bytes, hipStream_t st, PipeStages* pipe) {
  if (!h) return fail(LINETR_E_ARG, "describe: null handle");
  if (h->cfg.bn_batch_stats) return fail(LINETR_E_ARG, "describe: a training-mode handle (bn_batch_stats = 1) runs linetr_forward_train only");
  if (int e = check_cu(h_cu, n_images)) return e;
  if (h_cu[n_images] != N) return fail(LINETR_E_ARG, "describe: cu_sub does not end at N");
  if (K <= 0 || N <= 0) return LINETR_OK;
  if (!d_recs || !d_dense_desc || !d_dense_score || !d_line_desc || !d_ws) return fail(LINETR_E_ARG, "describe: null pointer");
  if (T < 1 || T > 4096 || height % 8 || width % 8) return fail(LINETR_E_ARG, "describe: bad max_tokens / image size");
  if (n_real < N || n_real > (int64_t)N * T) return fail(LINETR_E_ARG, "describe: implausible real-token count");
  if (out.desc && !out.pnt) return fail(LINETR_E_ARG, "describe: out.desc requires out.pnt");
  K2sTable k2s;
  if (int e = k2s_table(out, n_images, K, N, h_cu, k2s, "describe")) return e;
  if (ws_bytes < linetr_describe_workspace_bytes(h, n_images, height, width, N, n_real))
    return fail(LINETR_E_WORKSPACE, "describe: workspace too small");
  const int64_t rows = n_real + n_images;
  if (rows > INT32_MAX / 8) return fail(LINETR_E_ARG, "describe: batch too large");
  LT_HIP(hipSetDevice(h->device));
  DescWs dw = desc_layout(n_images, height, width, N, rows, (char*)d_ws);
  FwdWs w = fwd_layout(h, N, rows, n_images, (char*)d_ws + dw.fwd_off);
  const int* cu_dev;
  if (int e = cu_on_device(h_cu, d_cu, n_images, w, st, cu_dev)) return e;
  TokenFront f{d_recs, K, N, td, T, d_dense_desc, d_dense_score, n_images, height, width, align_corners, dense_is_nhwc,
               (double)width - 0.6, (double)height - 0.6, out.sublines ? out.sublines : dw.sublines, out.resp ? out.resp : dw.resp,
               out.angle_sub ? out.angle_sub : dw.angle_sub};
  f.s2l_g = dw.s2l_g; f.nhwc_buf = dw.nhwc;
  f.map_always = true;
  f.tokenize_bytes = (double)n_real * 16;
  f.cpnt = dw.cpnt; f.cscore = dw.cscore; f.n_pad_images = n_images; f.first_pad = n_real;
  const float* nhwc_map;
  if (int e = token_front(h, st, f, out, k2s, d_sub2line, nhwc_map)) return e;
  TokenStage ts;
  ts.cpnt = dw.cpnt; ts.cscore = dw.cscore; ts.nhwc = nhwc_map; ts.recs = d_recs; ts.sub2line_g = dw.s2l_g;
  ts.rows = rows; ts.first_pad = n_real; ts.Hc = height / 8; ts.Wc = width / 8; ts.align_corners = align_corners;
  ts.pipe = pipe;
  if (int e = pipe_boundary(pipe, CUT_TOKENS, st)) return e;
  return forward_core(h, st, ts, f.sublines, f.resp, f.angle_sub, h_cu, cu_dev, n_images, N, T, d_line_desc, w);
}

int pipe_ready(LinetrHandle* h) {
  LinetrHandle::Pipe& p = h->pipe;
  if (p.stream[0]) return LINETR_OK;
  if (p.failed) return fail(LINETR_E_HIP, "describe_submit: the pipeline's streams could not be created");
  constexpr int NS = LinetrHandle::PIPE_STREAMS, NL = LinetrHandle::PIPE_SLOTS, NE = NL * (NS + 1);
  hipStream_t s[NS] = {};
  hipEvent_t ev[NE] = {};
  bool ok = true;
  for (int i = 0; ok && i < NS; ++i) ok = hipStreamCreateWithFlags(&s[i], hipStreamNonBlocking) == hipSuccess;
  for (int i = 0; ok && i < NE; ++i) ok = hipEventCreateWithFlags(&ev[i], hipEventDisableTiming) == hipSuccess;
  if (!ok) {
    for (hipEvent_t e : ev) if (e) (void)hipEventDestroy(e);
    for (hipStream_t x : s) if (x) (void)hipStreamDestroy(x);
    (void)hipGetLastError();
    p.failed = true;
    return fail(LINETR_E_HIP, "describe_submit: the pipeline's streams could not be created");
  }
  for (int i = 0; i < NS; ++i) p.stream[i] = s[i];
  for (int l = 0, k = 0; l < NL; ++l) {
    p.fork[l] = ev[k++]; p.done[l] = ev[k++];
    for (int c = 0; c < NS - 1; ++c) p.cut[l][c] = ev[k++];
  }
  return LINETR_OK;
}

struct PipePlan { int n_cuts = 0; int cut[LinetrHandle::PIPE_STREAMS - 1] = {0, 0, 0}; };
PipePlan pipe_plan(const LinetrHandle* h, int n_slots) {
  PipePlan pl;
  const int n_sig = (int)h->sig.size();
  if (n_slots == 2 || n_sig < 5) { pl.n_cuts = 1; pl.cut[0] = n_sig >= 3 ? CUT_SIG0 + 2 : CUT_SENTENCE; }
  else { pl.n_cuts = 2; pl.cut[0] = CUT_SIG0; pl.cut[1] = CUT_SIG0 + 3; }
  return pl;
}
}

extern "C" int linetr_describe(LinetrHandle* h, const LinetrLineRec* d_recs, int32_t K, int32_t N, int64_t n_real,
                               const int32_t* h_cu, const int32_t* d_cu, int32_t n_images, double td, int32_t T,
                               const float* d_dense_desc, const float* d_dense_score, int32_t height, int32_t width,
                               int32_t align_corners, int32_t dense_is_nhwc, LinetrTokens out, int32_t* d_sub2line,
                               float* d_line_desc, void* d_ws, int64_t ws_bytes, void* stream) {
  return describe_impl(h, d_recs, K, N, n_real, h_cu, d_cu, n_images, td, T, d_dense_desc, d_dense_score, height, width, align_corners,
                       dense_is_nhwc, out, d_sub2line, d_line_desc, d_ws, ws_bytes, (hipStream_t)stream, nullptr);
}

extern "C" int32_t linetr_pipeline_max_slots(void) { return LinetrHandle::PIPE_SLOTS; }

extern "C" int linetr_describe_submit(LinetrHandle* h, const LinetrLineRec* d_recs, int32_t K, int32_t N, int64_t n_real,
                                      const int32_t* h_cu, const int32_t* d_cu, int32_t n_images, double td, int32_t T,
                                      const float* d_dense_desc, const float* d_dense_score, int32_t height, int32_t width,
                                      int32_t align_corners, int32_t dense_is_nhwc, LinetrTokens out, int32_t* d_sub2line,
                                      float* d_line_desc, void* d_ws, int64_t ws_bytes, int32_t slot, int32_t n_slots, void* stream) {
  if (!h) return fail(LINETR_E_ARG, "describe_submit: null handle");
  if (n_slots < 1 || n_slots > LinetrHandle::PIPE_SLOTS || slot < 0 || slot >= n_slots)
    return fail(LINETR_E_ARG, "describe_submit: need 0 <= slot < n_slots <= %d", LinetrHandle::PIPE_SLOTS);
  LT_HIP(hipSetDevice(h->device));
  if (int e = pipe_ready(h)) return e;
  LinetrHandle::Pipe& p = h->pipe;
  hipStream_t st = (hipStream_t)stream;
  if (p.submitted[slot]) LT_HIP(hipEventSynchronize(p.done[slot]));
  const PipePlan plan = pipe_plan(h, n_slots);
  PipeStages stg;
  for (int i = 0; i < LinetrHandle::PIPE_STREAMS; ++i) stg.stream[i] = p.stream[i];
  stg.n_cuts = plan.n_cuts;
  for (int i = 0; i < plan.n_cuts; ++i) { stg.cut[i] = plan.cut[i]; stg.ev[i] = p.cut[slot][i]; }
  LT_HIP(hipEventRecord(p.fork[slot], st));
  LT_HIP(hipStreamWaitEvent(stg.stream[0], p.fork[slot], 0));
  const int e = describe_impl(h, d_recs, K, N, n_real, h_cu, d_cu, n_images, td, T, d_dense_desc, d_dense_score, height, width,
                              align_corners, dense_is_nhwc, out, d_sub2line, d_line_desc, d_ws, ws_bytes, stg.stream[0], &stg);
  if (e) {
    for (hipStream_t x : p.stream) (void)hipStreamSynchronize(x);
    p.submitted[slot] = false;
    return e;
  }
  LT_HIP(hipEventRecord(p.done[slot], stg.stream[stg.next]));
  p.submitted[slot] = true;
  return LINETR_OK;
}

extern "C" int linetr_describe_join(LinetrHandle* h, int32_t slot, void* stream) {
  if (!h) return fail(LINETR_E_ARG, "describe_join: null handle");
  if (slot < 0 || slot >= LinetrHandle::PIPE_SLOTS) return fail(LINETR_E_ARG, "describe_join: bad slot");
  if (!h->pipe.stream[0] || !h->pipe.submitted[slot]) return fail(LINETR_E_ARG, "describe_join: nothing was submitted to this slot");
  LT_HIP(hipStreamWaitEvent((hipStream_t)stream, h->pipe.done[slot], 0));
  return LINETR_OK;
}

extern "C" int linetr_debug_posenc(LinetrHandle* h, int32_t which, const float* d_in0, const float* d_in1,
                                      const float* d_in2, int64_t rows, float* d_out, void* stream) {
  if (!h || !d_in0 || !d_in1 || !d_out || (which == 1 && !d_in2) || which < 0 || which > 1)
    return fail(LINETR_E_ARG, "debug_posenc: bad argument");
  if (!fused_mlp_enabled(h->cfg)) return fail(LINETR_E_ARG, "debug_posenc: needs keyline_encoder [32,64,128,256]");
  if (rows <= 0) return LINETR_OK;
  LT_HIP(hipSetDevice(h->device));
  return enc_mlp123(h, (hipStream_t)stream, EncCall{which, d_in0, d_in1, which == ENC_WORD ? nullptr : d_in2, rows, nullptr}, d_out);
}

extern "C" int linetr_debug_gemm(LinetrHandle* h, const float* A, int32_t lda, const float* W, const float* bias,
                                 const float* R, float* Y, int32_t ldy, int32_t M, int32_t N, int32_t K, int32_t act,
                                 int32_t cache_weights, void* stream) {
  if (lda < K || ldy < N || lda % 4 || ldy % 4) return fail(LINETR_E_ARG, "debug_gemm: bad leading dimension");
  if (!h || !A || !W || !Y) return fail(LINETR_E_ARG, "debug_gemm: null argument");
  if (K % 32 || N % 64) return fail(LINETR_E_ARG, "debug_gemm: N %% 64 == 0 and K %% 32 == 0 required");
  LT_HIP(hipSetDevice(h->device));
  hipStream_t st = (hipStream_t)stream;
  GemmW w;
  w.W = W; w.b = bias; w.rows = N; w.K = K;
  unsigned char* buf = nullptr;
  if (h->precision != LINETR_PREC_F32) {
    int64_t bytes = 0;
    const SplitOffsets at = split_offsets(N, K, N == WS_N && K == WS_K, bytes);
    auto it = h->debug_split.find(W);
    const bool make = it == h->debug_split.end();
    if (make) LT_HIP(hipMalloc((void**)&buf, bytes));
    split_copies(w, make ? buf : it->second, at, make, st);
    LT_LAUNCH_CHECK();
    if (make && cache_weights) { h->debug_split[W] = buf; buf = nullptr; }
  }
  const int e = run_gemm(h, st, w, M, {A, lda}, {Y, ldy}, act, R);
  if (buf) {
    (void)hipStreamSynchronize(st);
    (void)hipFree(buf);
  }
  return e;
}

extern "C" int linetr_debug_gemm_case(LinetrHandle* h, const LinetrGemmCase* c, int32_t* tile_used, void* stream) {
  if (!h || !c) return fail(LINETR_E_ARG, "debug_gemm_case: null argument");
  const bool query = !c->A && !c->W && !c->Y;
  const int M = c->M, N = c->N, K = c->K, groups = c->groups;
  if (M < 0 || N <= 0 || K <= 0 || groups < 1) return fail(LINETR_E_ARG, "debug_gemm_case: bad shape M=%d N=%d K=%d groups=%d", M, N, K, groups);
  if (K % 32 || N % 64) return fail(LINETR_E_ARG, "debug_gemm_case: N %% 64 == 0 and K %% 32 == 0 required");
  if (c->lda % 4 || c->ldy % 4 || c->ldy < N || (c->A2 && (c->lda2 % 4 || c->lda2 < K - c->K1)) || c->lda < (c->A2 ? c->K1 : K))
    return fail(LINETR_E_ARG, "debug_gemm_case: bad leading dimension");
  if (c->A2 && (c->K1 <= 0 || c->K1 >= K || c->K1 % 32))
    return fail(LINETR_E_ARG, "debug_gemm_case: the split point K1 = %d must be a multiple of 32 inside (0, K = %d)", c->K1, K);
  if (c->gA % 4 || c->gY % 4 || c->gA < 0 || c->gY < 0) return fail(LINETR_E_ARG, "debug_gemm_case: group strides must be non-negative multiples of 4 floats");
  if (c->act < ACT_NONE || c->act > ACT_DIST) return fail(LINETR_E_ARG, "debug_gemm_case: act must be 0 .. 3");
  if (c->tile < -1 || (c->tile >= (int)SplitTile::count && c->tile != LINETR_GEMM_TILE_WS))
    return fail(LINETR_E_ARG, "debug_gemm_case: no tile %d", c->tile);
  NormSpec ns;
  if (c->norm) {
    if (c->norm != 1 && c->norm != 2) return fail(LINETR_E_ARG, "debug_gemm_case: norm must be 0, 1 (LayerNorm) or 2 (L2)");
    if (N != D || c->ldy != D || groups != 1) return fail(LINETR_E_ARG, "debug_gemm_case: a row normalisation needs N = ldy = 256 and one group");
    if (!query && c->norm == 1 && (!c->gamma || !c->beta)) return fail(LINETR_E_ARG, "debug_gemm_case: LayerNorm needs gamma and beta");
    ns.mode = c->norm; ns.gamma = c->gamma; ns.beta = c->beta; ns.add2 = c->add2; ns.eps = c->eps;
  } else if (c->via_row_norm) {
    return fail(LINETR_E_ARG, "debug_gemm_case: via_row_norm without a norm");
  }
  if (!query) {
    if (!c->A || !c->W || !c->Y) return fail(LINETR_E_ARG, "debug_gemm_case: null tensor");
    uintptr_t al = (uintptr_t)c->A | (uintptr_t)c->A2 | (uintptr_t)c->W | (uintptr_t)c->bias | (uintptr_t)c->R | (uintptr_t)c->Y |
                   (uintptr_t)c->gamma | (uintptr_t)c->beta | (uintptr_t)c->add2;
    if (al % 16) return fail(LINETR_E_ARG, "debug_gemm_case: tensors must be 16-byte aligned");
  }
  const int64_t rows = (int64_t)N * groups;
  const bool with_st = groups == 1 && N == WS_N && K == WS_K;
  GemmW w;
  w.W = c->W; w.b = c->bias; w.rows = (int)rows; w.K = K;
  const GemmA A{c->A, c->lda, c->A2, c->lda2, c->A2 ? c->K1 : 0};
  const GemmGroups grp{groups, N, c->gA, c->gY};
  const GemmGroups* pg = groups > 1 ? &grp : nullptr;
  GemmForce force;
  force.tile = c->tile; force.used = tile_used; force.launch = false;
  const bool fuse = c->norm && !c->via_row_norm && (c->tile >= 0 || gemm_norm_fuses(h, w, M, A, c->R, c->Y));
  if (with_st) w.st = reinterpret_cast<const unsigned char*>(h);
  if (int e = run_gemm(h, nullptr, w, M, A, {c->Y, c->ldy}, c->act, c->R, pg, fuse ? &ns : nullptr, &force)) return e;
  if (query || M == 0) return LINETR_OK;
  LT_HIP(hipSetDevice(h->device));
  hipStream_t st = (hipStream_t)stream;
  unsigned char* buf = nullptr;
  int64_t bytes = 0;
  SplitOffsets at{};
  if (h->precision != LINETR_PREC_F32) at = split_offsets(rows, K, with_st, bytes);
  bytes = align_up(bytes, 256);
  const int64_t tmp_at = bytes;
  if (c->norm && !fuse) bytes += (int64_t)M * D * sizeof(float);
  if (bytes > 0) LT_HIP(hipMalloc((void**)&buf, bytes));
  if (h->precision != LINETR_PREC_F32) split_copies(w, buf, at, true, st);
  int e = LINETR_OK;
  if (hipGetLastError() != hipSuccess) e = fail(LINETR_E_HIP, "debug_gemm_case: splitting the weights failed");
  force.launch = true;
  if (!e && c->norm && !fuse) {
    float* tmp = reinterpret_cast<float*>(buf + tmp_at);
    e = run_gemm(h, st, w, M, A, {tmp, D}, c->act, c->R, nullptr, nullptr, &force);
    if (!e) e = row_norm(h, st, tmp, M, ns, c->Y);
  } else if (!e) {
    e = run_gemm(h, st, w, M, A, {c->Y, c->ldy}, c->act, c->R, pg, fuse ? &ns : nullptr, &force);
  }
  (void)hipStreamSynchronize(st);
  if (buf) (void)hipFree(buf);
  return e;
}

extern "C" int linetr_debug_sig_attention(LinetrHandle* h, int32_t kernel, int32_t layer, const float* d_in, int32_t ld_in,
                                          const int32_t* h_cu, int32_t n_images, float* d_msg, int32_t* kernel_used, void* stream) {
  if (!h) return fail(LINETR_E_ARG, "debug_sig_attention: null handle");
  if (h->cfg.bn_batch_stats) return fail(LINETR_E_ARG, "debug_sig_attention: a training-mode handle (bn_batch_stats = 1) is not served");
  if (kernel < -1 || kernel > SIGK_FUSED) return fail(LINETR_E_ARG, "debug_sig_attention: kernel must be -1 .. 4");
  if (int e = check_cu(h_cu, n_images)) return e;
  const int N = h_cu[n_images];
  int max_n = 0;
  for (int i = 0; i < n_images; ++i) max_n = std::max(max_n, h_cu[i + 1] - h_cu[i]);
  const bool query_only = kernel == -1 && !d_in && !d_msg;
  if (kernel == -1) kernel = sig_attn_plan(h, n_images, N, max_n).kernel();
  if (kernel_used) *kernel_used = kernel;
  if (query_only) return LINETR_OK;
  if (kernel == SIGK_FUSED) {
    if (h->precision != LINETR_PREC_BF16X6) return fail(LINETR_E_ARG, "debug_sig_attention: the fused kernel runs in bf16x6 mode only");
    if (max_n > 256) return fail(LINETR_E_ARG, "debug_sig_attention: the fused kernel takes images of up to 256 sub-lines");
    if (layer < 0 || layer >= (int)h->sig.size()) return fail(LINETR_E_ARG, "debug_sig_attention: layer out of range");
    if (!h->sig[layer].Wqkv.st) return fail(LINETR_E_ARG, "debug_sig_attention: the layer has no split-tile weight image");
    if (ld_in != D) return fail(LINETR_E_ARG, "debug_sig_attention: the fused kernel reads z rows, ld_in must be 256");
  } else if (ld_in != 3 * D && !(kernel == SIGK_SMALL && ld_in == 4 * D)) {
    return fail(LINETR_E_ARG, "debug_sig_attention: ld_in must be 768 (or 1024, sig_attn_small only)");
  }
  if (N <= 0) return LINETR_OK;
  if (!d_in || !d_msg) return fail(LINETR_E_ARG, "debug_sig_attention: null tensor");
  if (((uintptr_t)d_in | (uintptr_t)d_msg) % 16) return fail(LINETR_E_ARG, "debug_sig_attention: tensors must be 16-byte aligned");
  LT_HIP(hipSetDevice(h->device));
  hipStream_t st = (hipStream_t)stream;
  int* cu_dev = nullptr;
  LT_HIP(hipMalloc((void**)&cu_dev, (n_images + 1) * sizeof(int)));
  int e = LINETR_OK;
  if (hipMemcpyAsync(cu_dev, h_cu, (n_images + 1) * sizeof(int), hipMemcpyHostToDevice, st) != hipSuccess)
    e = fail(LINETR_E_HIP, "debug_sig_attention: cu_sub upload failed");
  const double fl = attn_flops(h_cu, n_images);
  if (!e)
    e = kernel == SIGK_FUSED ? sig_qkv_attention(h, st, h->sig[layer], d_in, cu_dev, n_images, N, fl, d_msg)
                             : sig_attention(h, st, kernel, d_in, ld_in, cu_dev, n_images, N, max_n, fl, d_msg);
  (void)hipStreamSynchronize(st);
  (void)hipFree(cu_dev);
  return e;
}

extern "C" int linetr_debug_tok_mlp(LinetrHandle* h, int32_t variant, const float* d_pnt, const float* d_score, int64_t rows_word,
                                    const float* d_sublines, const float* d_resp, const float* d_angle, int64_t rows_line,
                                    float* d_out_word, float* d_out_line, int32_t max_blocks, int32_t* variant_used, void* stream) {
  if (!h) return fail(LINETR_E_ARG, "debug_tok_mlp: null handle");
  if (h->cfg.bn_batch_stats) return fail(LINETR_E_ARG, "debug_tok_mlp: a training-mode handle (bn_batch_stats = 1) is not served");
  if (variant < -1 || variant > TOKV_CHAIN) return fail(LINETR_E_ARG, "debug_tok_mlp: variant must be -1 .. 4");
  if (rows_word < 0 || rows_line < 0 || rows_word > INT32_MAX / 8 || rows_line > INT32_MAX / 8)
    return fail(LINETR_E_ARG, "debug_tok_mlp: row counts must be 0 .. %d", INT32_MAX / 8);
  if (max_blocks < 0) return fail(LINETR_E_ARG, "debug_tok_mlp: max_blocks must be 0 (one block per compute unit) or positive");
  if (!fused_mlp_enabled(h->cfg) || h->cfg.enc_channels[0] != 32 || h->cfg.enc_channels[3] != D)
    return fail(LINETR_E_ARG, "debug_tok_mlp: needs keyline_encoder [32,64,128,256]");
  const bool query_only = variant == -1 && !d_out_word && !d_out_line;
  bool word = rows_word > 0 && variant != TOKV_LINE, line = rows_line > 0 && variant != TOKV_WORD;
  if (variant == -1) {
    const TokMlpPlan plan = tok_mlp_plan(h, rows_word, rows_line);
    variant = plan.both >= 0 ? plan.both : (word && !plan.word) || (line && !plan.line) ? (int)TOKV_CHAIN : word ? (int)TOKV_WORD : line ? (int)TOKV_LINE : -1;
  }
  if (variant_used) *variant_used = variant;
  if (query_only || variant < 0) return LINETR_OK;
  if (variant == TOKV_DUAL || variant == TOKV_SEQ) {
    if (rows_word <= 0 || rows_line <= 0) return fail(LINETR_E_ARG, "debug_tok_mlp: the two-encoder launches need rows of both encoders");
    if (variant == TOKV_DUAL && !tok_mlp_dual_fits(rows_word, rows_line))
      return fail(LINETR_E_ARG, "debug_tok_mlp: %lld + %lld rows do not fit the chip side by side (one block per 64-row tile, %d compute units)",
                  (long long)rows_word, (long long)rows_line, cu_count());
  }
  if (variant != TOKV_CHAIN && ((word && !tok_mlp_has_images(h->enc[ENC_WORD])) || (line && !tok_mlp_has_images(h->enc[ENC_LINE]))))
    return fail(LINETR_E_ARG, "debug_tok_mlp: the encoder has no split-tile weight images");
  if (!word && !line) return LINETR_OK;
  if ((word && (!d_pnt || !d_score || !d_out_word)) || (line && (!d_sublines || !d_resp || !d_angle || !d_out_line)))
    return fail(LINETR_E_ARG, "debug_tok_mlp: null tensor");
  if (((uintptr_t)d_pnt | (uintptr_t)d_score | (uintptr_t)d_sublines | (uintptr_t)d_resp | (uintptr_t)d_angle) % 4 ||
      ((uintptr_t)d_out_word | (uintptr_t)d_out_line) % 16)
    return fail(LINETR_E_ARG, "debug_tok_mlp: outputs must be 16-byte aligned, inputs 4-byte aligned");
  LT_HIP(hipSetDevice(h->device));
  hipStream_t st = (hipStream_t)stream;
  float* scratch = nullptr;
  const int64_t off_line = align_up((word ? rows_word : 0) * h->cfg.enc_channels[2] * 4, 256);
  if (variant == TOKV_CHAIN) LT_HIP(hipMalloc((void**)&scratch, off_line + align_up((line ? rows_line : 0) * h->cfg.enc_channels[2] * 4, 256) + 256));
  float* act_w[4] = {nullptr, nullptr, scratch, d_out_word};
  float* act_l[4] = {nullptr, nullptr, scratch ? (float*)((char*)scratch + off_line) : nullptr, d_out_line};
  const EncCall cw{ENC_WORD, d_pnt, d_score, nullptr, rows_word, act_w};
  const EncCall cl{ENC_LINE, d_sublines, d_resp, d_angle, rows_line, act_l};
  int e = LINETR_OK;
  switch (variant) {
    case TOKV_WORD: e = tok_mlp_launch(tok_mlp_args(h, cw), true, st, max_blocks); break;
    case TOKV_LINE: e = tok_mlp_launch(tok_mlp_args(h, cl), false, st, max_blocks); break;
    case TOKV_DUAL: e = tok_mlp_launch_dual(tok_mlp_args(h, cw), tok_mlp_args(h, cl), st, max_blocks, 0); break;
    case TOKV_SEQ: e = tok_mlp_launch_dual(tok_mlp_args(h, cw), tok_mlp_args(h, cl), st, max_blocks, 1); break;
    default:
      if (word) e = pos_encoder(h, st, cw, false);
      if (!e && line) e = pos_encoder(h, st, cl, false);
  }
  (void)hipStreamSynchronize(st);
  if (scratch) (void)hipFree(scratch);
  return e;
}

extern "C" int linetr_debug_cls_pool(LinetrHandle* h, int32_t kernel, const LinetrLineRec* d_recs, int32_t K, const int32_t* d_sub2line,
                                     int32_t N, int32_t T, const float* d_cpnt, const float* d_a4, int64_t first_pad, int32_t n_images,
                                     const float* d_map, int32_t dense_is_nhwc, int32_t Hc, int32_t Wc, int32_t align_corners,
                                     const float* d_desc_dense, float* d_pooled, int32_t* kernel_used, void* stream) {
  if (!h) return fail(LINETR_E_ARG, "debug_cls_pool: null handle");
  if (h->cfg.bn_batch_stats) return fail(LINETR_E_ARG, "debug_cls_pool: a training-mode handle (bn_batch_stats = 1) is not served");
  if (kernel < -1 || kernel > POOLK_SPLIT4) return fail(LINETR_E_ARG, "debug_cls_pool: kernel must be -1 .. 3");
  if (N < 0) return fail(LINETR_E_ARG, "debug_cls_pool: negative sub-line count");
  if (kernel == -1) kernel = cls_pool_plan(d_desc_dense == nullptr, N);
  if (kernel_used) *kernel_used = kernel;
  if (!d_pooled) return LINETR_OK;
  if (T < 1 || T > 4096) return fail(LINETR_E_ARG, "debug_cls_pool: max_tokens must be 1 .. 4096");
  if (N == 0) return LINETR_OK;
  if (!d_a4) return fail(LINETR_E_ARG, "debug_cls_pool: null tensor");
  if (((uintptr_t)d_a4 | (uintptr_t)d_pooled) % 16) return fail(LINETR_E_ARG, "debug_cls_pool: tensors must be 16-byte aligned");
  hipStream_t st = (hipStream_t)stream;
  TokenStage ts;
  if (kernel == POOLK_DENSE) {
    if (!d_desc_dense || (uintptr_t)d_desc_dense % 16) return fail(LINETR_E_ARG, "debug_cls_pool: the dense kernel reads d_desc_dense [N][T][256], 16-byte aligned");
    if ((int64_t)N * T > INT32_MAX / 8) return fail(LINETR_E_ARG, "debug_cls_pool: batch too large");
    LT_HIP(hipSetDevice(h->device));
    ts.desc = d_desc_dense; ts.rows = (int64_t)N * T;
    const int e = cls_pool_launch(h, st, kernel, ts, 1, N, T, d_a4, d_pooled);
    (void)hipStreamSynchronize(st);
    return e;
  }
  if (!d_recs || !d_sub2line || !d_cpnt || !d_map) return fail(LINETR_E_ARG, "debug_cls_pool: null tensor");
  if (K < 1 || n_images < 1 || Hc < 1 || Wc < 1 || first_pad < 0 || first_pad > INT32_MAX / 8 || (int64_t)n_images * Hc * Wc > INT32_MAX / D)
    return fail(LINETR_E_ARG, "debug_cls_pool: bad shape");
  if ((uintptr_t)d_recs % 8 || ((uintptr_t)d_sub2line | (uintptr_t)d_cpnt | (uintptr_t)d_map) % 4 || (dense_is_nhwc && (uintptr_t)d_map % 16))
    return fail(LINETR_E_ARG, "debug_cls_pool: misaligned tensor (records 8 bytes, an NHWC map 16, the others 4)");
  LT_HIP(hipSetDevice(h->device));
  {
    std::vector<LinetrLineRec> recs(K);
    std::vector<int32_t> s2l(N);
    LT_HIP(hipStreamSynchronize(st));
    LT_HIP(hipMemcpy(recs.data(), d_recs, (size_t)K * sizeof(LinetrLineRec), hipMemcpyDeviceToHost));
    LT_HIP(hipMemcpy(s2l.data(), d_sub2line, (size_t)N * sizeof(int32_t), hipMemcpyDeviceToHost));
    for (int n = 0; n < N; ++n) {
      if (s2l[n] < 0 || s2l[n] >= K) return fail(LINETR_E_ARG, "debug_cls_pool: sub-line %d maps to key-line %d, outside [0, %d)", n, s2l[n], K);
      const LinetrLineRec& r = recs[s2l[n]];
      const int64_t j = (int64_t)n - r.first_sub;
      if (j < 0 || j >= r.n_sub || j * T >= r.n_tok)
        return fail(LINETR_E_ARG, "debug_cls_pool: sub-line %d is not one of key-line %d's (first_sub %d, n_sub %d, n_tok %d)", n, s2l[n], r.first_sub, r.n_sub, r.n_tok);
      if (r.first_tok < 0 || (int64_t)r.first_tok + r.n_tok > first_pad)
        return fail(LINETR_E_ARG, "debug_cls_pool: key-line %d's tokens [%d, %d + %d) reach past first_pad = %lld", s2l[n], r.first_tok, r.first_tok, r.n_tok, (long long)first_pad);
      if (r.image < 0 || r.image >= n_images) return fail(LINETR_E_ARG, "debug_cls_pool: key-line %d's image %d outside [0, %d)", s2l[n], r.image, n_images);
    }
  }
  float* buf = nullptr;
  if (!dense_is_nhwc) LT_HIP(hipMalloc((void**)&buf, (size_t)n_images * Hc * Wc * D * sizeof(float)));
  ts.cpnt = d_cpnt; ts.recs = d_recs; ts.sub2line_g = d_sub2line; ts.rows = first_pad + n_images; ts.first_pad = first_pad;
  ts.Hc = Hc; ts.Wc = Wc; ts.align_corners = align_corners;
  int e = nhwc_map(h, st, d_map, dense_is_nhwc, n_images, Hc * Wc, buf, ts.nhwc);
  if (!e) e = cls_pool_launch(h, st, kernel, ts, n_images, N, T, d_a4, d_pooled);
  (void)hipStreamSynchronize(st);
  if (buf) (void)hipFree(buf);
  return e;
}
```

linetr_amd/csrc/lt_model.h:

```cpp
#pragma once
#include "lt_common.h"
#include "lt_token.h"
#include "lt_gemm_split.h"

namespace lt {

template <bool RELU = true>
__global__ void word_mlp1_kernel(const float* __restrict__ pnt, const float* __restrict__ score, int64_t rows,
                                 float cx, float cy, float scale, const float* __restrict__ W ,
                                 const float* __restrict__ b, float* __restrict__ out ) {
#pragma clang fp contract(off)
  const int64_t gid = (int64_t)blockIdx.x * blockDim.x + threadIdx.x;
  const int64_t row = gid >> 3;
  if (row >= rows) return;
  const int c0 = (int)(gid & 7) * 4;
  const float x = (pnt[row * 2 + 0] - cx) / scale;
  const float y = (pnt[row * 2 + 1] - cy) / scale;
  const float s = score[row];
  f32x4 o;
#pragma unroll
  for (int c = 0; c < 4; ++c) {
    const float* w = W + (c0 + c) * 3;
    float v = b[c0 + c] + w[0] * x + w[1] * y + w[2] * s;
    o[c] = RELU ? fmaxf(v, 0.f) : v;
  }
  *reinterpret_cast<f32x4*>(out + row * 32 + c0) = o;
}

template <bool RELU = true>
__global__ void line_mlp1_kernel(const float* __restrict__ sublines , const float* __restrict__ resp,
                                 const float* __restrict__ angle, int N, float cx, float cy, float scale,
                                 const float* __restrict__ W , const float* __restrict__ b,
                                 float* __restrict__ out ) {
#pragma clang fp contract(off)
  const int gid = blockIdx.x * blockDim.x + threadIdx.x;
  const int row = gid >> 3;
  if (row >= N) return;
  const int c0 = (gid & 7) * 4;
  const float* sl = sublines + (int64_t)row * 4;
  const float sx = (sl[0] - cx) / scale, sy = (sl[1] - cy) / scale;
  const float ex = (sl[2] - cx) / scale, ey = (sl[3] - cy) / scale;
  const float in[5] = {(sx + ex) / 2.f, (sy + ey) / 2.f, resp[row], angle[row * 2], angle[row * 2 + 1]};
  f32x4 o;
#pragma unroll
  for (int c = 0; c < 4; ++c) {
    const float* w = W + (c0 + c) * 5;
    float v = b[c0 + c];
#pragma unroll
    for (int i = 0; i < 5; ++i) v += w[i] * in[i];
    o[c] = RELU ? fmaxf(v, 0.f) : v;
  }
  *reinterpret_cast<f32x4*>(out + (int64_t)row * 32 + c0) = o;
}

__device__ __forceinline__ void word_feat(const float* __restrict__ pnt, const float* __restrict__ score, int64_t row,
                                          float cx, float cy, float scale, float (&in)[3]) {
#pragma clang fp contract(off)
  in[0] = (pnt[row * 2 + 0] - cx) / scale;
  in[1] = (pnt[row * 2 + 1] - cy) / scale;
  in[2] = score[row];
}
__device__ __forceinline__ void line_feat(const float* __restrict__ sublines, const float* __restrict__ resp,
                                          const float* __restrict__ angle, int64_t row, float cx, float cy, float scale,
                                          float (&in)[5]) {
#pragma clang fp contract(off)
  const float* sl = sublines + row * 4;
  const float sx = (sl[0] - cx) / scale, sy = (sl[1] - cy) / scale;
  const float ex = (sl[2] - cx) / scale, ey = (sl[3] - cy) / scale;
  in[0] = (sx + ex) / 2.f; in[1] = (sy + ey) / 2.f; in[2] = resp[row]; in[3] = angle[row * 2]; in[4] = angle[row * 2 + 1];
}

template <bool WORD>
__global__ __launch_bounds__(256) void mlp123_kernel(const float* __restrict__ p0, const float* __restrict__ p1,
                                                     const float* __restrict__ p2, int64_t rows, int rows_per_wave,
                                                     float cx, float cy, float scale,
                                                     const float* __restrict__ W1 , const float* __restrict__ b1,
                                                     const float* __restrict__ W2 , const float* __restrict__ b2,
                                                     const float* __restrict__ W3 , const float* __restrict__ b3,
                                                     float* __restrict__ out ) {
  constexpr int IN = WORD ? 3 : 5;
  const int lane = threadIdx.x & 63, col = lane & 31, h = lane >> 5;
  const int64_t wave = (int64_t)blockIdx.x * 4 + (threadIdx.x >> 6);
  const int64_t r_begin = wave * rows_per_wave;
  const int64_t r_end = r_begin + rows_per_wave < rows ? r_begin + rows_per_wave : rows;
  __shared__ __attribute__((aligned(16))) float sAll[64 * 33 + 128 * 65];
  __shared__ __attribute__((aligned(16))) float sW1[32 * 8];
  __shared__ __attribute__((aligned(16))) float sB[64 + 128];
  float* sW2 = sAll;
  float* sW3 = sAll + 64 * 33;
  float* stg = sAll + (threadIdx.x >> 6) * (32 * 68);
  static_assert(4 * 32 * 68 <= 64 * 33 + 128 * 65, "staging tiles must fit into the dead weight images");
  {
    f32x4 v2[2], v3[8];
#pragma unroll
    for (int u = 0; u < 2; ++u) v2[u] = *reinterpret_cast<const f32x4*>(W2 + (threadIdx.x + 256 * u) * 4);
#pragma unroll
    for (int u = 0; u < 8; ++u) v3[u] = *reinterpret_cast<const f32x4*>(W3 + (threadIdx.x + 256 * u) * 4);
#pragma unroll
    for (int u = 0; u < 2; ++u) {
      const int idx = threadIdx.x + 256 * u, r = idx / 8, c = (idx % 8) * 4;
#pragma unroll
      for (int q = 0; q < 4; ++q) sW2[r * 33 + c + q] = v2[u][q];
    }
#pragma unroll
    for (int u = 0; u < 8; ++u) {
      const int idx = threadIdx.x + 256 * u, r = idx / 16, c = (idx % 16) * 4;
#pragma unroll
      for (int q = 0; q < 4; ++q) sW3[r * 65 + c + q] = v3[u][q];
    }
  }
  {
    const int k = threadIdx.x >> 3, c = threadIdx.x & 7;
    sW1[threadIdx.x] = c < IN ? W1[k * IN + c] : (c == 7 ? b1[k] : 0.f);
  }
  if (threadIdx.x < 64) sB[threadIdx.x] = b2[threadIdx.x];
  else if (threadIdx.x < 192) sB[threadIdx.x] = b3[threadIdx.x - 64];
  __syncthreads();
  float w2[2][16], w3[4][32];
#pragma unroll
  for (int i = 0; i < 2; ++i)
#pragma unroll
    for (int s2 = 0; s2 < 16; ++s2) w2[i][s2] = sW2[(32 * i + col) * 33 + 2 * s2 + h];
#pragma unroll
  for (int j = 0; j < 4; ++j)
#pragma unroll
    for (int i = 0; i < 2; ++i)
#pragma unroll
      for (int r = 0; r < 16; ++r) w3[j][i * 16 + r] = sW3[(32 * j + col) * 65 + 32 * i + cd_row(r, h)];
  __syncthreads();
  if (r_begin >= r_end) return;
  float feat[IN], feat_next[IN];
  {
    int64_t row = r_begin + col;
    row = row < r_end ? row : r_end - 1;
    if constexpr (WORD) word_feat(p0, p1, row, cx, cy, scale, feat);
    else line_feat(p0, p1, p2, row, cx, cy, scale, feat);
  }
  for (int64_t base = r_begin; base < r_end; base += 32) {
    {
      int64_t row = base + 32 + col;
      row = row < r_end ? row : r_end - 1;
      if constexpr (WORD) word_feat(p0, p1, row, cx, cy, scale, feat_next);
      else line_feat(p0, p1, p2, row, cx, cy, scale, feat_next);
    }
    float a1[16];
    {
#pragma clang fp contract(off)
#pragma unroll
      for (int s1 = 0; s1 < 16; ++s1) {
        const float* wr = sW1 + (2 * s1 + h) * 8;
        const f32x4 wa = *reinterpret_cast<const f32x4*>(wr), wb = *reinterpret_cast<const f32x4*>(wr + 4);
        const float wv[8] = {wa[0], wa[1], wa[2], wa[3], wb[0], wb[1], wb[2], wb[3]};
        float t = wv[7];
#pragma unroll
        for (int i = 0; i < IN; ++i) t += wv[i] * feat[i];
        a1[s1] = fmaxf(t, 0.f);
      }
    }
    f32x16 acc2[2];
#pragma unroll
    for (int i = 0; i < 2; ++i)
#pragma unroll
      for (int r = 0; r < 16; r += 4) {
        const f32x4 bv = *reinterpret_cast<const f32x4*>(sB + 32 * i + cd_row(r, h));
        acc2[i][r] = bv[0]; acc2[i][r + 1] = bv[1]; acc2[i][r + 2] = bv[2]; acc2[i][r + 3] = bv[3];
      }
#pragma unroll
    for (int s2 = 0; s2 < 16; ++s2)
#pragma unroll
      for (int i = 0; i < 2; ++i) acc2[i] = __builtin_amdgcn_mfma_f32_32x32x2f32(w2[i][s2], a1[s2], acc2[i], 0, 0, 0);
#pragma unroll
    for (int i = 0; i < 2; ++i)
#pragma unroll
      for (int r = 0; r < 16; ++r) acc2[i][r] = fmaxf(acc2[i][r], 0.f);
#pragma unroll
    for (int jp = 0; jp < 2; ++jp) {
      f32x16 acc3[2];
#pragma unroll
      for (int q = 0; q < 2; ++q)
#pragma unroll
        for (int r = 0; r < 16; r += 4) {
          const f32x4 bv = *reinterpret_cast<const f32x4*>(sB + 64 + 32 * (2 * jp + q) + cd_row(r, h));
          acc3[q][r] = bv[0]; acc3[q][r + 1] = bv[1]; acc3[q][r + 2] = bv[2]; acc3[q][r + 3] = bv[3];
        }
#pragma unroll
      for (int i = 0; i < 2; ++i)
#pragma unroll
        for (int r = 0; r < 16; ++r)
#pragma unroll
          for (int q = 0; q < 2; ++q)
            acc3[q] = __builtin_amdgcn_mfma_f32_32x32x2f32(w3[2 * jp + q][i * 16 + r], acc2[i][r], acc3[q], 0, 0, 0);
#pragma unroll
      for (int q = 0; q < 2; ++q)
#pragma unroll
        for (int r = 0; r < 16; r += 4)
          *reinterpret_cast<f32x4*>(stg + col * 68 + 32 * q + cd_row(r, h)) =
              f32x4{fmaxf(acc3[q][r], 0.f), fmaxf(acc3[q][r + 1], 0.f), fmaxf(acc3[q][r + 2], 0.f), fmaxf(acc3[q][r + 3], 0.f)};
      __builtin_amdgcn_wave_barrier();
#pragma unroll
      for (int i = 0; i < 8; ++i) {
        const int t = 4 * i + (lane >> 4), pc = (lane & 15) * 4;
        if (base + t < r_end)
          *reinterpret_cast<f32x4*>(out + (base + t) * 128 + 64 * jp + pc) = *reinterpret_cast<const f32x4*>(stg + t * 68 + pc);
      }
      __builtin_amdgcn_wave_barrier();
    }
#pragma unroll
    for (int i = 0; i < IN; ++i) feat[i] = feat_next[i];
  }
}


__global__ __launch_bounds__(256) void cls_pool_kernel(const float* __restrict__ desc ,
                                                       const float* __restrict__ a4 , int T,
                                                       ClsPoolConst cc, float* __restrict__ pooled ) {
  extern __shared__ float sm[];
  const int S = T + 1;
  const int n = blockIdx.x;
  const int tid = threadIdx.x, lane = tid & 63, wave = tid >> 6;
  const float* dn = desc + (int64_t)n * T * D;
  const float* an = a4 + (int64_t)n * T * D;
  f32x4 u[4], u2[4];
#pragma unroll
  for (int h = 0; h < 4; ++h) {
    u[h] = *reinterpret_cast<const f32x4*>(cc.U + h * D + lane * 4);
    u2[h] = *reinterpret_cast<const f32x4*>(cc.U2 + h * D + lane * 4);
  }
  for (int j = wave; j < T; j += 4) {
    const f32x4 dv = *reinterpret_cast<const f32x4*>(dn + j * D + lane * 4);
    const f32x4 av = *reinterpret_cast<const f32x4*>(an + j * D + lane * 4);
#pragma unroll
    for (int h = 0; h < 4; ++h) {
      float p = 0.f;
#pragma unroll
      for (int c = 0; c < 4; ++c) p += dv[c] * u[h][c] + av[c] * u2[h][c];
      p = wave_sum(p);
      if (lane == 0) sm[h * S + 1 + j] = p + cc.c_tok[h];
    }
  }
  if (tid < 4) sm[tid * S] = cc.s_cls[tid];
  __syncthreads();
  if (tid < 4) {
    float* s = sm + tid * S;
    float mx = s[0];
    for (int j = 1; j < S; ++j) mx = fmaxf(mx, s[j]);
    float sum = 0.f;
    for (int j = 0; j < S; ++j) { s[j] = expf(s[j] - mx); sum += s[j]; }
    for (int j = 0; j < S; ++j) s[j] = s[j] / sum;
  }
  __syncthreads();
  float db[4] = {0.f, 0.f, 0.f, 0.f}, ab[4] = {0.f, 0.f, 0.f, 0.f};
  for (int j = 0; j < T; ++j) {
    const float dv = dn[j * D + tid], av = an[j * D + tid];
#pragma unroll
    for (int h = 0; h < 4; ++h) {
      const float p = sm[h * S + 1 + j];
      db[h] += p * dv;
      ab[h] += p * av;
    }
  }
  float* out = pooled + (int64_t)n * 4 * POOLW;
#pragma unroll
  for (int h = 0; h < 4; ++h) {
    out[h * POOLW + tid] = db[h];
    out[h * POOLW + 256 + tid] = ab[h];
  }
  if (tid < 4 * 32) {
    const int h = tid >> 5, i = tid & 31;
    out[h * POOLW + 512 + i] = i == 0 ? sm[h * S] : 0.f;
  }
}

template <int SPLIT>
__global__ __launch_bounds__(256, 3) void cls_pool_online_kernel(
    const LinetrLineRec* __restrict__ recs, const int* __restrict__ sub2line_g, const float* __restrict__ cpnt,
    const float* __restrict__ a4, int64_t first_pad, int N, int T, const float* __restrict__ nhwc, int Hc, int Wc,
    int align_corners, ClsPoolConst cc, float* __restrict__ pooled , int reverse) {
  const int lane = threadIdx.x & 63;
  const int wv = threadIdx.x >> 6;
  const int n_fwd = SPLIT == 1 ? blockIdx.x * 4 + wv : blockIdx.x;
  if (n_fwd >= N) return;
  const int n = reverse ? N - 1 - n_fwd : n_fwd;
  const LinetrLineRec r = recs[sub2line_g[n]];
  const int j = n - r.first_sub;
  const int n_valid = min(T, r.n_tok - j * T);
  const int n_pad = T - n_valid;
  const int ntk = n_valid + (n_pad > 0 ? 1 : 0);
  const int64_t tok0 = (int64_t)r.first_tok + (int64_t)j * T;
  const int64_t padrow = first_pad + r.image;
  const float* nhwc_img = nhwc + (int64_t)r.image * Hc * Wc * D;
  f32x4 u[4], u2[4];
#pragma unroll
  for (int h = 0; h < 4; ++h) {
    u[h] = *reinterpret_cast<const f32x4*>(cc.U + h * D + lane * 4);
    u2[h] = *reinterpret_cast<const f32x4*>(cc.U2 + h * D + lane * 4);
  }
  float m[4], l[4], w0[4];
  f32x4 db[4], ab[4];
#pragma unroll
  for (int h = 0; h < 4; ++h) {
    m[h] = cc.s_cls[h] * LOG2E; l[h] = 1.f; w0[h] = 1.f;
    if (SPLIT > 1 && wv != 0) { m[h] = -INFINITY; l[h] = 0.f; w0[h] = 0.f; }
    db[h] = f32x4{0.f, 0.f, 0.f, 0.f};
    ab[h] = f32x4{0.f, 0.f, 0.f, 0.f};
  }
  auto row_of = [&](int jj) -> int64_t { return jj < n_valid ? tok0 + jj : padrow; };
  int t_off[4];
  float t_w[4];
  auto fill_taps = [&](int chunk) {
    const int jj = chunk + lane;
    const int64_t row = row_of(jj < ntk ? jj : ntk - 1);
    tap_coords(cpnt[row * 2], cpnt[row * 2 + 1], Hc, Wc, align_corners, t_off, t_w);
  };
  auto issue = [&](int jj, TapSet& t, f32x4& a) {
    int off[4];
    float wt[4];
#pragma unroll
    for (int k = 0; k < 4; ++k) {
      off[k] = __builtin_amdgcn_readlane(t_off[k], jj & 63);
      wt[k] = __builtin_bit_cast(float, __builtin_amdgcn_readlane(__builtin_bit_cast(int, t_w[k]), jj & 63));
    }
    taps_load(nhwc_img, off, wt, lane, t);
    a = *reinterpret_cast<const f32x4*>(a4 + row_of(jj) * D + lane * 4);
  };
  TapSet cur, nxt;
  f32x4 a_cur, a_nxt;
  const int jj0 = SPLIT == 1 ? 0 : wv;
  fill_taps(0);
  if (jj0 < ntk) issue(jj0, cur, a_cur);
  for (int jj = jj0; jj < ntk; jj += SPLIT) {
    if (jj + SPLIT < ntk) {
      if (((jj + SPLIT) >> 6) != (jj >> 6)) fill_taps((jj + SPLIT) & ~63);
      issue(jj + SPLIT, nxt, a_nxt);
    }
    const f32x4 dv = taps_finish<true>(cur);
    const float mult = jj < n_valid ? 1.f : (float)n_pad;
    float sc[4];
#pragma unroll
    for (int h = 0; h < 4; ++h) {
      float p = 0.f;
#pragma unroll
      for (int c = 0; c < 4; ++c) p += dv[c] * u[h][c] + a_cur[c] * u2[h][c];
      sc[h] = p;
    }
    wave_sum_n<4>(sc);
#pragma unroll
    for (int h = 0; h < 4; ++h) {
      const float sh = (sc[h] + cc.c_tok[h]) * LOG2E;
      if (__any(sh > m[h])) {
        const float alpha = __builtin_amdgcn_exp2f(m[h] - sh);
        m[h] = sh;
        l[h] *= alpha;
        w0[h] *= alpha;
#pragma unroll
        for (int c = 0; c < 4; ++c) { db[h][c] *= alpha; ab[h][c] *= alpha; }
      }
      const float e = __builtin_amdgcn_exp2f(sh - m[h]) * mult;
      l[h] += e;
#pragma unroll
      for (int c = 0; c < 4; ++c) {
        db[h][c] += e * dv[c];
        ab[h][c] += e * a_cur[c];
      }
    }
    cur = nxt;
    a_cur = a_nxt;
  }
  float* out = pooled + (int64_t)n * 4 * POOLW;
  if constexpr (SPLIT > 1) {
    __shared__ float st_ml[4][4][4];
    __shared__ f32x4 st_v[4][4][2][64];
#pragma unroll
    for (int h = 0; h < 4; ++h) {
      if (lane == 0) { st_ml[wv][h][0] = m[h]; st_ml[wv][h][1] = l[h]; st_ml[wv][h][2] = w0[h]; }
      st_v[wv][h][0][lane] = db[h];
      st_v[wv][h][1][lane] = ab[h];
    }
    __syncthreads();
    const int h = wv;
    float M = st_ml[0][h][0];
#pragma unroll
    for (int w = 1; w < 4; ++w) M = fmaxf(M, st_ml[w][h][0]);
    float L = 0.f, W0 = 0.f;
    f32x4 d = {0.f, 0.f, 0.f, 0.f}, a = {0.f, 0.f, 0.f, 0.f};
#pragma unroll
    for (int w = 0; w < 4; ++w) {
      const float sc = __builtin_amdgcn_exp2f(st_ml[w][h][0] - M);
      L += st_ml[w][h][1] * sc;
      W0 += st_ml[w][h][2] * sc;
      const f32x4 dv = st_v[w][h][0][lane], av = st_v[w][h][1][lane];
#pragma unroll
      for (int c = 0; c < 4; ++c) { d[c] += dv[c] * sc; a[c] += av[c] * sc; }
    }
    const float inv = 1.f / L;
#pragma unroll
    for (int c = 0; c < 4; ++c) { d[c] *= inv; a[c] *= inv; }
    *reinterpret_cast<f32x4*>(out + h * POOLW + lane * 4) = d;
    *reinterpret_cast<f32x4*>(out + h * POOLW + 256 + lane * 4) = a;
    if (lane < 8) {
      f32x4 z = {0.f, 0.f, 0.f, 0.f};
      if (lane == 0) z[0] = W0 * inv;
      *reinterpret_cast<f32x4*>(out + h * POOLW + 512 + lane * 4) = z;
    }
    return;
  }
#pragma unroll
  for (int h = 0; h < 4; ++h) {
    const float inv = 1.f / l[h];
    f32x4 d = db[h], a = ab[h];
#pragma unroll
    for (int c = 0; c < 4; ++c) { d[c] *= inv; a[c] *= inv; }
    *reinterpret_cast<f32x4*>(out + h * POOLW + lane * 4) = d;
    *reinterpret_cast<f32x4*>(out + h * POOLW + 256 + lane * 4) = a;
    if (lane < 8) {
      f32x4 z = {0.f, 0.f, 0.f, 0.f};
      if (lane == 0) z[0] = w0[h] * inv;
      *reinterpret_cast<f32x4*>(out + h * POOLW + 512 + lane * 4) = z;
    }
  }
}

__global__ __launch_bounds__(256) void row_norm_kernel(const float* __restrict__ x, int rows, int mode,
                                                       const float* __restrict__ gamma, const float* __restrict__ beta,
                                                       const float* __restrict__ add, float eps, float* __restrict__ y) {
  const int row = blockIdx.x * 4 + (threadIdx.x >> 6);
  if (row >= rows) return;
  const int lane = threadIdx.x & 63;
  f32x4 v = *reinterpret_cast<const f32x4*>(x + (int64_t)row * D + lane * 4);
  f32x4 o;
  if (mode == 0) {
    float mean = wave_sum(v[0] + v[1] + v[2] + v[3]) * (1.f / D);
    float q = 0.f;
#pragma unroll
    for (int c = 0; c < 4; ++c) { float d = v[c] - mean; q += d * d; }
    const float rstd = 1.f / sqrtf(wave_sum(q) * (1.f / D) + eps);
    const f32x4 g = *reinterpret_cast<const f32x4*>(gamma + lane * 4);
    const f32x4 b = *reinterpret_cast<const f32x4*>(beta + lane * 4);
#pragma unroll
    for (int c = 0; c < 4; ++c) o[c] = (v[c] - mean) * rstd * g[c] + b[c];
  } else {
    float q = 0.f;
#pragma unroll
    for (int c = 0; c < 4; ++c) q += v[c] * v[c];
    const float nrm = fmaxf(sqrtf(wave_sum(q)), 1e-12f);
#pragma unroll
    for (int c = 0; c < 4; ++c) o[c] = v[c] / nrm;
  }
  if (add) {
    const f32x4 a = *reinterpret_cast<const f32x4*>(add + (int64_t)row * D + lane * 4);
#pragma unroll
    for (int c = 0; c < 4; ++c) o[c] += a[c];
  }
  *reinterpret_cast<f32x4*>(y + (int64_t)row * D + lane * 4) = o;
}

}
```

linetr_amd/csrc/lt_token.h:

```cpp
#pragma once
#include "lt_common.h"

namespace lt {

__global__ __launch_bounds__(256) void nchw_to_nhwc_kernel(const float* __restrict__ in, float* __restrict__ out,
                                                           int C, int P) {
  __shared__ float tile[64][65];
  const int b = blockIdx.z;
  const int p0 = blockIdx.x * 64, c0 = blockIdx.y * 64;
  const float* src = in + (int64_t)b * C * P;
  float* dst = out + (int64_t)b * C * P;
  const int tid = threadIdx.x;
  {
    const int pq = (tid & 15) * 4;
#pragma unroll
    for (int i = 0; i < 4; ++i) {
      const int c = (tid >> 4) + i * 16;
      const float* row = src + (int64_t)(c0 + c) * P + p0 + pq;
      f32x4 v;
      if (p0 + pq + 3 < P && (((uintptr_t)row) & 15) == 0) v = *reinterpret_cast<const f32x4*>(row);
      else {
#pragma unroll
        for (int k = 0; k < 4; ++k) v[k] = p0 + pq + k < P ? row[k] : 0.f;
      }
#pragma unroll
      for (int k = 0; k < 4; ++k) tile[c][pq + k] = v[k];
    }
  }
  __syncthreads();
  {
    const int cq = (tid & 15) * 4;
#pragma unroll
    for (int i = 0; i < 4; ++i) {
      const int p = (tid >> 4) + i * 16;
      if (p0 + p < P) {
        f32x4 v;
#pragma unroll
        for (int k = 0; k < 4; ++k) v[k] = tile[cq + k][p];
        *reinterpret_cast<f32x4*>(dst + (int64_t)(p0 + p) * C + c0 + cq) = v;
      }
    }
  }
}

__global__ void line_fill_kernel(const LinetrLineRec* __restrict__ recs, int K, double wclip, double hclip,
                                 float* __restrict__ klines, float* __restrict__ length,
                                 float* __restrict__ angles, int* __restrict__ sub2line_g,
                                 int* __restrict__ sub2line_l) {
  int k = blockIdx.x * blockDim.x + threadIdx.x;
  if (k >= K) return;
  const LinetrLineRec r = recs[k];
  if (klines) {
    klines[k * 4 + 0] = (float)r.sp[0];
    klines[k * 4 + 1] = (float)r.sp[1];
    klines[k * 4 + 2] = (float)fmin(r.ep[0], wclip);
    klines[k * 4 + 3] = (float)fmin(r.ep[1], hclip);
    length[k] = (float)r.length;
    angles[k * 2 + 0] = (float)r.angle[0];
    angles[k * 2 + 1] = (float)r.angle[1];
  }
  for (int s = 0; s < r.n_sub; ++s) {
    sub2line_g[r.first_sub + s] = k;
    if (sub2line_l) sub2line_l[r.first_sub + s] = r.line_local;
  }
}

constexpr int K2S_MAX_IMAGES = 8;
struct K2sImage { int64_t off; int n_sub; int sub_base; };
struct K2sTable { K2sImage img[K2S_MAX_IMAGES]; };

__device__ __forceinline__ void walk_along(const double sp[2], const double ep[2], double d, double& x, double& y) {
#pragma clang fp contract(off)
  const double vx = ep[0] - sp[0], vy = ep[1] - sp[1];
  double dx, dy;
  if (vx != 0.0) {
    const double m = vy / vx;
    dx = sqrt(d * d / (1.0 + m * m));
    dy = m * dx;
  } else {
    dx = 0.0;
    dy = vy > 0.0 ? d : -d;
  }
  x = dx + sp[0];
  y = dy + sp[1];
}

__global__ __launch_bounds__(64) void tokenize_kernel(
    const LinetrLineRec* __restrict__ recs, const int* __restrict__ sub2line_g, int N, double td, int T,
    int height, int width, double clip_x, double clip_y, const float* __restrict__ dense_score, float* __restrict__ sublines,
    float* __restrict__ pnt, float* __restrict__ mask, float* __restrict__ resp,
    float* __restrict__ angle_sub, float* __restrict__ score, float* __restrict__ cpnt,
    float* __restrict__ cscore, int n_pad_images, int64_t first_pad, float* __restrict__ mat_k2s, const K2sTable k2s) {
#pragma clang fp contract(off)
  const int n = blockIdx.x;
  if (n >= N) {
    const int pad_blocks = (n_pad_images + 63) / 64;
    if (n - N < pad_blocks) {
      const int i = (n - N) * 64 + threadIdx.x;
      if (i < n_pad_images) {
        cpnt[(first_pad + i) * 2 + 0] = 0.f;
        cpnt[(first_pad + i) * 2 + 1] = 0.f;
        cscore[first_pad + i] = dense_score[(int64_t)i * height * width];
      }
      return;
    }
    const int k = n - N - pad_blocks;
    const LinetrLineRec r = recs[k];
    const K2sImage im = k2s.img[r.image & (K2S_MAX_IMAGES - 1)];
    float* row = mat_k2s + im.off + (int64_t)r.line_local * im.n_sub;
    const float w = (float)(1.0 / (double)r.n_sub);
    const int j0 = r.first_sub - im.sub_base;
    for (int j = threadIdx.x; j < im.n_sub; j += 64) row[j] = (j >= j0 && j < j0 + r.n_sub) ? w : 0.f;
    return;
  }
  const LinetrLineRec r = recs[sub2line_g[n]];
  const int j = n - r.first_sub;
  const double epc[2] = {fmin(r.ep[0], clip_x), fmin(r.ep[1], clip_y)};
  for (int t = threadIdx.x; t < T; t += 64) {
    const int ti = j * T + t;
    double x = 0.0, y = 0.0;
    float mk = 0.f;
    if (ti < r.n_tok - 1) {
      walk_along(r.sp, r.ep, (double)ti * td, x, y);
      mk = 1.f;
    } else if (ti == r.n_tok - 1) {
      x = epc[0];
      y = epc[1];
      mk = 1.f;
    }
    const float fx = (float)x, fy = (float)y;
    const int64_t o = (int64_t)n * T + t;
    if (pnt) { pnt[o * 2 + 0] = fx; pnt[o * 2 + 1] = fy; }
    if (mask) mask[(int64_t)n * (T + 1) + 1 + t] = mk;
    int ix = (int)rintf(fx), iy = (int)rintf(fy);
    ix = ix < width - 1 ? ix : width - 1;
    iy = iy < height - 1 ? iy : height - 1;
    ix = ix < 0 ? 0 : ix;
    iy = iy < 0 ? 0 : iy;
    const float sc = dense_score[(int64_t)r.image * height * width + (int64_t)iy * width + ix];
    if (score) score[o] = sc;
    if (cpnt && mk != 0.f) {
      const int64_t c = (int64_t)r.first_tok + ti;
      cpnt[c * 2 + 0] = fx;
      cpnt[c * 2 + 1] = fy;
      cscore[c] = sc;
    }
  }
  if (threadIdx.x == 0) {
    if (mask) mask[(int64_t)n * (T + 1)] = 1.f;
    double s[2], e[2];
    if (j == 0) { s[0] = r.sp[0]; s[1] = r.sp[1]; }
    else walk_along(r.sp, r.ep, (double)(j * T - 1) * td, s[0], s[1]);
    if (j == r.n_sub - 1) { e[0] = epc[0]; e[1] = epc[1]; }
    else walk_along(r.sp, r.ep, (double)((j + 1) * T - 1) * td, e[0], e[1]);
    sublines[(int64_t)n * 4 + 0] = (float)s[0];
    sublines[(int64_t)n * 4 + 1] = (float)s[1];
    sublines[(int64_t)n * 4 + 2] = (float)e[0];
    sublines[(int64_t)n * 4 + 3] = (float)e[1];
    const double dx = e[0] - s[0], dy = e[1] - s[1];
    const double geo = sqrt(dx * dx + dy * dy);
    resp[n] = (float)(geo / (td * (double)T));
    angle_sub[(int64_t)n * 2 + 0] = (float)r.angle[0];
    angle_sub[(int64_t)n * 2 + 1] = (float)r.angle[1];
  }
}

struct TapSet { f32x4 v[4]; float w[4]; };

__device__ __forceinline__ float grid_unnormalize(float g, int size, int align_corners) {
#pragma clang fp contract(off)
  if (align_corners) return (g + 1.f) * ((float)(size - 1) / 2.f);
  return __builtin_fmaf(g + 1.f, (float)size / 2.f, -0.5f);
}

__device__ __forceinline__ void tap_coords(float px, float py, int Hc, int Wc, int align_corners, int (&off)[4],
                                           float (&wt)[4]) {
#pragma clang fp contract(off)
  const float s = 8.f;
  float gx = ((px - s / 2) + 0.5f) / ((float)Wc * s - s / 2 - 0.5f);
  float gy = ((py - s / 2) + 0.5f) / ((float)Hc * s - s / 2 - 0.5f);
  gx = gx * 2.f - 1.f;
  gy = gy * 2.f - 1.f;
  const float ix = grid_unnormalize(gx, Wc, align_corners), iy = grid_unnormalize(gy, Hc, align_corners);
  const float x_w = floorf(ix), y_n = floorf(iy);
  const float w = ix - x_w, e = 1.f - w, nn = iy - y_n, ss = 1.f - nn;
  const float wv[4] = {ss * e, ss * w, nn * e, nn * w};
  const int x0 = (int)x_w, y0 = (int)y_n;
#pragma unroll
  for (int k = 0; k < 4; ++k) {
    const int yy = y0 + (k >> 1), xx = x0 + (k & 1);
    const bool in = xx >= 0 && xx < Wc && yy >= 0 && yy < Hc;
    const int yc = min(max(yy, 0), Hc - 1), xc = min(max(xx, 0), Wc - 1);
    off[k] = yc * Wc + xc;
    wt[k] = in ? wv[k] : 0.f;
  }
}

__device__ __forceinline__ void taps_load(const float* __restrict__ nhwc_img, const int (&off)[4], const float (&wt)[4],
                                          int lane, TapSet& t) {
  const float* base = nhwc_img + lane * 4;
#pragma unroll
  for (int k = 0; k < 4; ++k) {
    t.v[k] = *reinterpret_cast<const f32x4*>(base + (int64_t)off[k] * D);
    t.w[k] = wt[k];
  }
}

__device__ __forceinline__ void taps_issue(float px, float py, const float* __restrict__ nhwc_img, int Hc, int Wc,
                                           int align_corners, int lane, TapSet& t) {
  int off[4];
  float wt[4];
  tap_coords(px, py, Hc, Wc, align_corners, off, wt);
  taps_load(nhwc_img, off, wt, lane, t);
}

template <bool RCP = false>
__device__ __forceinline__ f32x4 taps_finish(const TapSet& t) {
#pragma clang fp contract(off)
  f32x4 o;
  float sq = 0.f;
#pragma unroll
  for (int c = 0; c < 4; ++c) {
    float v = t.v[0][c] * t.w[0];
    v = __builtin_fmaf(t.v[1][c], t.w[1], v);
    v = __builtin_fmaf(t.v[2][c], t.w[2], v);
    v = __builtin_fmaf(t.v[3][c], t.w[3], v);
    o[c] = v;
    sq += v * v;
  }
  sq = wave_sum(sq);
  const float nrm = fmaxf(sqrtf(sq), 1e-12f);
  if constexpr (RCP) {
    const float inv = 1.f / nrm;
#pragma unroll
    for (int c = 0; c < 4; ++c) o[c] = o[c] * inv;
  } else {
#pragma unroll
    for (int c = 0; c < 4; ++c) o[c] = o[c] / nrm;
  }
  return o;
}

__device__ __forceinline__ f32x4 sample_one(float px, float py, const float* __restrict__ nhwc_img, int Hc, int Wc,
                                            int align_corners, int lane) {
#pragma clang fp contract(off)
  const float s = 8.f;
  float gx = ((px - s / 2) + 0.5f) / ((float)Wc * s - s / 2 - 0.5f);
  float gy = ((py - s / 2) + 0.5f) / ((float)Hc * s - s / 2 - 0.5f);
  gx = gx * 2.f - 1.f;
  gy = gy * 2.f - 1.f;
  const float ix = grid_unnormalize(gx, Wc, align_corners), iy = grid_unnormalize(gy, Hc, align_corners);
  const float x_w = floorf(ix), y_n = floorf(iy);
  const float w = ix - x_w, e = 1.f - w, nn = iy - y_n, ss = 1.f - nn;
  const float nw = ss * e, ne = ss * w, sw = nn * e, se = nn * w;
  const int x0 = (int)x_w, y0 = (int)y_n, x1 = x0 + 1, y1 = y0 + 1;
  const float* base = nhwc_img + lane * 4;
  auto tap = [&](int yy, int xx) -> f32x4 {
    if (xx < 0 || xx >= Wc || yy < 0 || yy >= Hc) return f32x4{0.f, 0.f, 0.f, 0.f};
    return *reinterpret_cast<const f32x4*>(base + ((int64_t)yy * Wc + xx) * D);
  };
  const f32x4 v_nw = tap(y0, x0), v_ne = tap(y0, x1), v_sw = tap(y1, x0), v_se = tap(y1, x1);
  f32x4 o;
  float sq = 0.f;
#pragma unroll
  for (int c = 0; c < 4; ++c) {
    float v = v_nw[c] * nw;
    v = __builtin_fmaf(v_ne[c], ne, v);
    v = __builtin_fmaf(v_sw[c], sw, v);
    v = __builtin_fmaf(v_se[c], se, v);
    o[c] = v;
    sq += v * v;
  }
  sq = wave_sum(sq);
  const float nrm = fmaxf(sqrtf(sq), 1e-12f);
#pragma unroll
  for (int c = 0; c < 4; ++c) o[c] = o[c] / nrm;
  return o;
}

__global__ __launch_bounds__(256) void sample_desc_kernel(
    const float* __restrict__ pnt, const int* __restrict__ sub2line_g, const LinetrLineRec* __restrict__ recs,
    int64_t n_tokens, int T, const float* __restrict__ nhwc, int Hc, int Wc, int align_corners,
    float* __restrict__ desc) {
  const int64_t tok = (int64_t)blockIdx.x * 4 + (threadIdx.x >> 6);
  if (tok >= n_tokens) return;
  const int lane = threadIdx.x & 63;
  const int n = (int)(tok / T);
  const int img = recs ? recs[sub2line_g[n]].image : 0;
  const f32x4 o = sample_one(pnt[tok * 2 + 0], pnt[tok * 2 + 1], nhwc + (int64_t)img * Hc * Wc * D, Hc, Wc,
                             align_corners, lane);
  *reinterpret_cast<f32x4*>(desc + tok * D + lane * 4) = o;
}

constexpr int KP_DESC_N = 64;
constexpr int KP_DESC_LS = KP_DESC_N + 1;
constexpr size_t KP_DESC_LDS = (size_t)D * KP_DESC_LS * 4;

__global__ __launch_bounds__(256) void sp_kp_desc_kernel(const float* __restrict__ kp, const int* __restrict__ cu_kp, int B,
                                                         const float* __restrict__ nhwc, int Hc, int Wc, int align_corners,
                                                         float* __restrict__ out) {
  extern __shared__ __attribute__((aligned(16))) float kp_tile[];
  int chunk = blockIdx.x, b = 0, start = 0, n_b = 0;
  for (; b < B; ++b) {
    start = cu_kp[b];
    n_b = cu_kp[b + 1] - start;
    const int nch = (n_b + KP_DESC_N - 1) / KP_DESC_N;
    if (chunk < nch) break;
    chunk -= nch;
  }
  if (b >= B) return;
  const int j0 = chunk * KP_DESC_N, nj = min(KP_DESC_N, n_b - j0);
  const int lane = threadIdx.x & 63, w = threadIdx.x >> 6;
  const float* img = nhwc + (int64_t)b * Hc * Wc * D;
  for (int j = w; j < nj; j += 4) {
    const int64_t g = (int64_t)start + j0 + j;
    const f32x4 o = sample_one(kp[g * 2 + 0], kp[g * 2 + 1], img, Hc, Wc, align_corners, lane);
#pragma unroll
    for (int c = 0; c < 4; ++c) kp_tile[(lane * 4 + c) * KP_DESC_LS + j] = o[c];
  }
  __syncthreads();
  float* dst = out + (int64_t)D * start + j0;
  if (lane < nj)
    for (int ch = w * 64; ch < w * 64 + 64; ++ch) dst[(int64_t)ch * n_b + lane] = kp_tile[ch * KP_DESC_LS + lane];
}

}
```

linetr_amd/engine.py:

```python
from __future__ import annotations

import ctypes as C
import math
from dataclasses import dataclass, field

import numpy as np
import torch

from . import _native as nat

D = 256

DEFAULT_MODEL = dict(descriptor_dim=256, keyline_encoder=[32, 64, 128, 256], n_heads=4,
                     n_line_descriptive_layers=1, d_inner=1024, n_sig_layers=7, image_shape=[480, 640], bn_batch_stats=False)


def _as_numpy_f32(v):
    if torch.is_tensor(v):
        v = v.detach().cpu().numpy()
    return np.ascontiguousarray(v, dtype=np.float32)


@dataclass
class TokenBatch:
# ... 754 lines not shown
        out = {"assign": assign, "lmatches": lm, "found": found}
        if directions:
            out["match_dir"], out["overlap_dir"] = mdir, odir
        if projected:
            out["proj0"], out["proj1"] = p0, p1
        return out

    def match_points(self, desc0_cn: torch.Tensor, desc1_cn: torch.Tensor, thr, mutual=True):
        d0, d1 = self._f32(desc0_cn), self._f32(desc1_cn)
        n0, n1 = int(d0.shape[1]), int(d1.shape[1])
        dist = torch.empty((n0, n1), dtype=torch.float32, device=self.device)
        m01 = torch.full((n0,), -1, dtype=torch.int32, device=self.device)
        if n0 == 0 or n1 == 0:
            return dist, m01
        need = 4 * (n0 + n1) * (D + 1) + 2048 + self._L.linetr_match_workspace_bytes(1, n0 * n1, 0, n0 + n1)
        ws = self._workspace("match", need)
        nat.check(self._L.linetr_match_points(self._h, d0.data_ptr(), n0, d1.data_ptr(), n1, float(thr),
                                              int(bool(mutual)), dist.data_ptr(), m01.data_ptr(), ws.data_ptr(),
                                              ws.numel(), self._stream()), self._L)
        return dist, m01

    def superpoint_heads(self, score_logits: torch.Tensor = None, desc_raw: torch.Tensor = None, *, nhwc=True,
                         nchw=False):
        sl = self._f32(score_logits) if score_logits is not None else None
        dr = self._f32(desc_raw) if desc_raw is not None else None
        ref = sl if sl is not None else dr
        if ref is None:
            raise ValueError("superpoint_heads needs at least one head")
        B, _, Hc, Wc = (int(v) for v in ref.shape)
        if sl is not None and tuple(sl.shape) != (B, 65, Hc, Wc):
            raise ValueError(f"score_logits must be [B,65,Hc,Wc], got {tuple(sl.shape)}")
        if dr is not None and tuple(dr.shape) != (B, D, Hc, Wc):
            raise ValueError(f"desc_raw must be [B,{D},Hc,Wc], got {tuple(dr.shape)}")
        score = torch.empty((B, Hc * 8, Wc * 8), dtype=torch.float32, device=self.device) if sl is not None else None
        o_nhwc = torch.empty((B, Hc, Wc, D), dtype=torch.float32, device=self.device) if (dr is not None and nhwc) else None
        o_nchw = torch.empty((B, D, Hc, Wc), dtype=torch.float32, device=self.device) if (dr is not None and nchw) else None
        ptr = lambda t: t.data_ptr() if t is not None else None
        with torch.cuda.device(self.device):
            nat.check(self._L.linetr_superpoint_heads(self._h, ptr(sl), ptr(dr), B, Hc, Wc, ptr(score), ptr(o_nhwc),
                                                      ptr(o_nchw), self._stream()), self._L)
        return score, o_nhwc, o_nchw

    def superpoint_keypoints(self, dense_score: torch.Tensor, dense_desc: torch.Tensor = None, *, nms_radius=4,
                             keypoint_threshold=0.005, remove_borders=4, max_keypoints=-1, align_corners=False,
                             dense_layout="nhwc"):
        ds = self._f32(dense_score)
        if ds.dim() != 3:
            raise ValueError(f"dense_score must be [B,H,W], got {tuple(ds.shape)}")
        B, H, W = (int(v) for v in ds.shape)
        r, k, border = int(nms_radius), int(max_keypoints), int(remove_borders)
        thr = float(np.float32(keypoint_threshold))
        if not 0 <= r <= 8:
            raise ValueError(f"nms_radius must be 0..8, got {r}")
        if k < -1 or k == 0 or k > 4096:
            raise ValueError(f"max_keypoints must be -1 (all) or 1..4096, got {k}")
        if not thr >= 0 or border < 0:
            raise ValueError("keypoint_threshold and remove_borders must be >= 0")
        if dense_layout not in ("nhwc", "nchw"):
            raise ValueError("dense_layout must be 'nhwc' or 'nchw'")
        dd = None
        if dense_desc is not None:
            dd = self._f32(dense_desc)
            nhwc = dense_layout == "nhwc"
            if dd.dim() != 4 or int(dd.shape[0]) != B or int(dd.shape[3 if nhwc else 1]) != D:
                raise ValueError(f"dense_desc must be [B,Hc,Wc,{D}] (nhwc) or [B,{D},Hc,Wc] (nchw), got {tuple(dd.shape)}")
            Hc, Wc = (int(dd.shape[1]), int(dd.shape[2])) if nhwc else (int(dd.shape[2]), int(dd.shape[3]))
        if B == 0 or H == 0 or W == 0:
            e = lambda *shape: torch.empty(shape, dtype=torch.float32, device=self.device)
            return ([e(0, 2) for _ in range(B)], [e(0) for _ in range(B)],
                    [e(D, 0) for _ in range(B)] if dd is not None else None)
        cap = min(H * W, -(-H // (r + 1)) * -(-W // (r + 1)))
        with torch.cuda.device(self.device):
            cu = torch.empty(B + 1, dtype=torch.int32, device=self.device)
            found = torch.empty(B, dtype=torch.int32, device=self.device)
            while True:
                kp = torch.empty((B * cap, 2), dtype=torch.float32, device=self.device)
                sc = torch.empty((B * cap,), dtype=torch.float32, device=self.device)
                ws = self._workspace("keypoints", self._L.linetr_superpoint_keypoints_workspace_bytes(B, H, W, cap))
                nat.check(self._L.linetr_superpoint_keypoints(self._h, ds.data_ptr(), B, H, W, r, thr, border, k, cap, kp.data_ptr(),
                                                              sc.data_ptr(), cu.data_ptr(), found.data_ptr(), ws.data_ptr(), ws.numel(),
                                                              self._stream()), self._L)
                h_cu, h_found = self.collect(self.to_host_async(cu, found))
                if int(h_found.max()) <= cap:
                    break
                cap = int(h_found.max())
            n_total = int(h_cu[-1])
            desc = None
            if dd is not None:
                desc = torch.empty((D * n_total,), dtype=torch.float32, device=self.device)
                if n_total > 0:
                    wd = self._workspace("sample", self._L.linetr_point_descriptors_workspace_bytes(B, Hc, Wc, int(nhwc)) + 256)
                    nat.check(self._L.linetr_point_descriptors(self._h, kp.data_ptr(), cu.data_ptr(), B, n_total, dd.data_ptr(), Hc, Wc,
                                                               int(bool(align_corners)), int(nhwc), desc.data_ptr(), wd.data_ptr(),
                                                               wd.numel(), self._stream()), self._L)
        o = h_cu.tolist()
        kps = [kp[o[b]:o[b + 1]] for b in range(B)]
        scs = [sc[o[b]:o[b + 1]] for b in range(B)]
        descs = [desc[D * o[b]:D * o[b + 1]].view(D, o[b + 1] - o[b]) for b in range(B)] if desc is not None else None
        return kps, scs, descs

    PRECISIONS = {"f32": 0, "bf16x3": 1, "bf16x6": 2, "f16x3": 3}

    def set_precision(self, mode: str):
        nat.check(self._L.linetr_set_precision(self._h, self.PRECISIONS[mode]), self._L)

    def get_precision(self) -> str:
        code = self._L.linetr_get_precision(self._h)
        return {v: k for k, v in self.PRECISIONS.items()}[code]

    def debug_posenc(self, which: str, in0, in1, in2=None):
        a, b = self._f32(in0), self._f32(in1)
        c = self._f32(in2) if in2 is not None else None
        rows = int(b.shape[0])
        out = torch.empty((rows, 128), dtype=torch.float32, device=self.device)
        nat.check(self._L.linetr_debug_posenc(self._h, {"word": 0, "line": 1}[which], a.data_ptr(), b.data_ptr(),
                                                 c.data_ptr() if c is not None else None, rows, out.data_ptr(),
                                                 self._stream()), self._L)
        return out

    def debug_gemm(self, A, W, bias=None, residual=None, act=0, cache_weights=False, out=None):
        W = self._f32(W)
        if A.dtype != torch.float32 or A.device != self.device or A.stride(1) != 1:
            A = self._f32(A)
        M, K = A.shape
        N = W.shape[0]
        Y = out if out is not None else torch.empty((M, N), dtype=torch.float32, device=self.device)
        b = self._f32(bias) if bias is not None else None
        r = residual
        if r is not None and (r.stride(0) != Y.stride(0) or r.stride(1) != 1):
            r = self._f32(r) if Y.stride(0) == N else None
            assert r is not None, "residual must share the output's row stride"
        nat.check(self._L.linetr_debug_gemm(self._h, A.data_ptr(), A.stride(0), W.data_ptr(),
                                            b.data_ptr() if b is not None else None,
                                            r.data_ptr() if r is not None else None, Y.data_ptr(), Y.stride(0), M, N, K,
                                            int(act), int(cache_weights), self._stream()), self._L)
        return Y

    GEMM_SPLIT_TILES = ("32x32k4", "112x256", "128x64", "256x128", "128x256", "64x256", "128x128", "128x128s", "256x256", "64x64",
                        "64x128")
    GEMM_F32_TILES = ("128x64", "128x128", "64x128")
    GEMM_WS = "ws64x256"
    _GEMM_TILE_WS = 100

    def _gemm_tile_code(self, tile):
        if tile is None or tile == -1:
            return -1
        if tile == self.GEMM_WS:
            return self._GEMM_TILE_WS
        names = self.GEMM_F32_TILES if self.get_precision() == "f32" else self.GEMM_SPLIT_TILES
        if tile not in names:
            raise ValueError(f"no GEMM tile {tile!r} in {self.get_precision()} mode")
        return names.index(tile)

    def _gemm_tile_name(self, code):
        if code == self._GEMM_TILE_WS:
            return self.GEMM_WS
        return (self.GEMM_F32_TILES if self.get_precision() == "f32" else self.GEMM_SPLIT_TILES)[code]

    def gemm_tile(self, M, N, K, *, groups=1, act=0, residual=False, concat=False, norm=0, lda=None, ldy=None, tile=-1) -> str:
        flag = C.c_void_p(16)
        c = nat.GemmCase(A=None, lda=int(lda or K), A2=flag if concat else None, lda2=int(K), K1=32 if concat else 0, W=None, bias=None,
                         R=flag if residual else None, Y=None, ldy=int(ldy or N), M=int(M), N=int(N), K=int(K), act=int(act),
                         groups=int(groups), gA=0, gY=0, norm=int(norm), gamma=None, beta=None, add2=None, eps=0.0, via_row_norm=0,
                         tile=self._gemm_tile_code(tile))
        used = C.c_int32(-1)
        nat.check(self._L.linetr_debug_gemm_case(self._h, C.byref(c), C.byref(used), None), self._L)
        return self._gemm_tile_name(used.value)

    def debug_gemm_case(self, A, W, bias=None, residual=None, act=0, *, A2=None, groups=1, gA=0, gY=None, norm=0, gamma=None,
                        beta=None, add2=None, eps=0.0, via_row_norm=False, tile=-1, out=None):
        W = self._f32(W)
        M, K1 = (int(v) for v in A.shape)
        K = K1 + (int(A2.shape[1]) if A2 is not None else 0)
        N = int(W.shape[0]) // groups
        if W.shape != (groups * N, K) or not W.is_contiguous():
            raise ValueError(f"W must be a contiguous [{groups} * N, {K}] tensor")
        if out is None:
            full = torch.empty((groups, M, N), dtype=torch.float32, device=self.device)
            out, gY = full[0], M * N
        else:
            full = out
        gY = int(gY or 0)

        def extent(t, rows, cols, gstride, what):
            if t.dtype != torch.float32 or t.device != self.device or t.dim() != 2 or t.stride(1) != 1:
                raise ValueError(f"{what}: a float32 matrix on the engine's device with unit column stride expected")
            if t.shape[0] < rows or t.shape[1] < cols:
                raise ValueError(f"{what}: shape {tuple(t.shape)} is smaller than [{rows}, {cols}]")
            have = t.untyped_storage().nbytes() // 4 - t.storage_offset()
            need = (groups - 1) * gstride + (rows - 1) * t.stride(0) + cols if rows > 0 else 0
            if need > have:
                raise ValueError(f"{what}: {need} floats needed behind its first element, the storage holds {have}")
            return t

        extent(A, M, K1, int(gA), "A")
        if A2 is not None:
            extent(A2, M, K - K1, int(gA), "A2")
        extent(out, M, N, gY, "out")
        if groups > 1 and gY < (M - 1) * out.stride(0) + N:
            raise ValueError("gY: the groups' outputs overlap")
        if residual is not None and extent(residual, M, N, 0, "residual").stride(0) != out.stride(0):
            raise ValueError("residual must share the output's row stride")
        vec = lambda t, n, what: None if t is None else extent(self._f32(t).reshape(1, -1), 1, n, 0, what)
        b, ga, be = vec(bias, groups * N, "bias"), vec(gamma, N, "gamma"), vec(beta, N, "beta")
        if add2 is not None and (extent(add2, M, N, 0, "add2").stride(0) != D or N != D):
            raise ValueError("add2 must have row stride 256")
        ptr = lambda t: t.data_ptr() if t is not None else None
        c = nat.GemmCase(A=ptr(A), lda=A.stride(0), A2=ptr(A2), lda2=A2.stride(0) if A2 is not None else 0, K1=K1 if A2 is not None else 0,
                         W=ptr(W), bias=ptr(b), R=ptr(residual), Y=ptr(out), ldy=out.stride(0), M=M, N=N, K=K, act=int(act),
                         groups=int(groups), gA=int(gA), gY=gY, norm=int(norm), gamma=ptr(ga), beta=ptr(be), add2=ptr(add2),
                         eps=float(eps), via_row_norm=int(bool(via_row_norm)), tile=self._gemm_tile_code(tile))
        used = C.c_int32(-1)
        nat.check(self._L.linetr_debug_gemm_case(self._h, C.byref(c), C.byref(used), self._stream()), self._L)
        return (full if groups > 1 or full is out else out), self._gemm_tile_name(used.value)

    SIG_KERNELS = ("sig_attn", "sig_attn_small", "sig_attn_split4", "sig_attn_split8", "sig_qkv_attn")

    def sig_attention_kernel(self, cu_sub) -> int:
        cu = np.ascontiguousarray(np.asarray(cu_sub, dtype=np.int32))
        used = C.c_int32(-1)
        nat.check(self._L.linetr_debug_sig_attention(self._h, -1, 0, None, 0, cu.ctypes.data, len(cu) - 1, None,
                                                     C.byref(used), self._stream()), self._L)
        return used.value

    def debug_sig_attention(self, kernel, x, cu_sub, layer=0, out=None):
        if x.dtype != torch.float32 or x.device != self.device or x.stride(1) != 1:
            x = self._f32(x)
        cu = np.ascontiguousarray(np.asarray(cu_sub, dtype=np.int32))
        N = int(cu[-1]) if len(cu) else 0
        if int(x.shape[0]) < N:
            raise ValueError(f"{N} rows expected, got {int(x.shape[0])}")
        msg = out if out is not None else torch.empty((N, D), dtype=torch.float32, device=self.device)
        if msg.dtype != torch.float32 or msg.device != self.device or not msg.is_contiguous():
            raise ValueError("out must be a contiguous float32 tensor on the engine's device")
        used = C.c_int32(-1)
        nat.check(self._L.linetr_debug_sig_attention(self._h, int(kernel), int(layer), x.data_ptr(), x.stride(0), cu.ctypes.data,
                                                     len(cu) - 1, msg.data_ptr(), C.byref(used), self._stream()), self._L)
        return msg, used.value

    TOK_MLP_VARIANTS = ("tok_mlp_word", "tok_mlp_line", "tok_mlp_dual", "tok_mlp_seq", "mlp123_gemm_chain")

    def tok_mlp_variant(self, rows_word, rows_line) -> int:
        used = C.c_int32(-1)
        nat.check(self._L.linetr_debug_tok_mlp(self._h, -1, None, None, int(rows_word), None, None, None, int(rows_line), None, None, 0,
                                               C.byref(used), self._stream()), self._L)
        return used.value

    def debug_tok_mlp(self, variant, word=None, line=None, out_word=None, out_line=None, max_blocks=0):
        def f32(t, n, what):
            if t.dtype != torch.float32 or t.device != self.device or not t.is_contiguous() or t.numel() < n:
                raise ValueError(f"{what}: a contiguous float32 tensor of at least {n} elements on the engine's device expected")
            return t.data_ptr()
        pw = [None, None]; pl = [None, None, None]
        rw = rl = 0
        if word is not None:
            rw = int(word[2])
            pw = [f32(word[0], 2 * rw, "pnt"), f32(word[1], rw, "score")]
            if out_word is None:
                out_word = torch.empty((rw, D), dtype=torch.float32, device=self.device)
            f32(out_word, rw * D, "out_word")
        if line is not None:
            rl = int(line[3])
            pl = [f32(line[0], 4 * rl, "sublines"), f32(line[1], rl, "resp"), f32(line[2], 2 * rl, "angle")]
            if out_line is None:
                out_line = torch.empty((rl, D), dtype=torch.float32, device=self.device)
            f32(out_line, rl * D, "out_line")
        used = C.c_int32(-1)
        nat.check(self._L.linetr_debug_tok_mlp(self._h, int(variant), pw[0], pw[1], rw, pl[0], pl[1], pl[2], rl,
                                               out_word.data_ptr() if out_word is not None else None,
                                               out_line.data_ptr() if out_line is not None else None, int(max_blocks), C.byref(used),
                                               self._stream()), self._L)
        return out_word, out_line, used.value

    CLS_POOL_KERNELS = ("cls_pool", "cls_pool_online", "cls_pool_online_reverse", "cls_pool_online_split4")

    def cls_pool_kernel(self, N, dense=False) -> int:
        used = C.c_int32(-1)
        nat.check(self._L.linetr_debug_cls_pool(self._h, -1, None, 0, None, int(N), 1, None, None, 0, 1, None, 1, 1, 1, 0,
                                                C.c_void_p(16) if dense else None, None, C.byref(used), self._stream()), self._L)
        return used.value

    def debug_cls_pool(self, kernel, a4, out, N, T, *, recs=None, sub2line=None, cpnt=None, first_pad=0, n_images=1, dense_map=None,
                       nhwc=True, Hc=0, Wc=0, align_corners=False, desc_dense=None):
        for t in (a4, out, cpnt, dense_map, desc_dense):
            if t is not None and (t.dtype != torch.float32 or t.device != self.device or not t.is_contiguous()):
                raise ValueError("contiguous float32 tensors on the engine's device expected")
        if out.numel() < N * 4 * 544:
            raise ValueError("out is smaller than [N, 4, 544]")
        if desc_dense is None:
            if recs.dtype != torch.uint8 or sub2line.dtype != torch.int32 or sub2line.numel() < N:
                raise ValueError("recs: uint8 bytes of LineRec[K]; sub2line: int32 [N]")
            if a4.numel() < (first_pad + n_images) * D or cpnt.numel() < (first_pad + n_images) * 2 or dense_map.numel() < n_images * Hc * Wc * D:
                raise ValueError("a4 / cpnt / dense_map are smaller than first_pad + n_images rows / n_images maps")
        elif a4.numel() < N * T * D or desc_dense.numel() < N * T * D:
            raise ValueError("a4 / desc_dense are smaller than [N * T, 256]")
        ptr = lambda t: t.data_ptr() if t is not None else None
        used = C.c_int32(-1)
        nat.check(self._L.linetr_debug_cls_pool(self._h, int(kernel), ptr(recs), recs.numel() // nat.REC_DTYPE.itemsize if recs is not None else 0,
                                                ptr(sub2line), int(N), int(T), ptr(cpnt), ptr(a4), int(first_pad), int(n_images),
                                                ptr(dense_map), int(bool(nhwc)), int(Hc), int(Wc), int(bool(align_corners)),
                                                ptr(desc_dense), ptr(out), C.byref(used), self._stream()), self._L)
        return out, used.value

    def to_st(self, X):
        X = self._f32(X)
        rows, K = X.shape
        out = torch.empty(int(self._L.linetr_st_bytes(rows, K)), dtype=torch.uint8, device=self.device)
        nat.check(self._L.linetr_debug_to_st(self._h, X.data_ptr(), X.stride(0), rows, K, out.data_ptr(), self._stream()), self._L)
        return out

    def from_st(self, st, rows, K):
        X = torch.empty((rows, K), dtype=torch.float32, device=self.device)
        nat.check(self._L.linetr_debug_from_st(self._h, st.data_ptr(), rows, K, X.data_ptr(), K, self._stream()), self._L)
        return X

    def gemm_st(self, A1, K1, W, M, N, A2=None, K2=0, bias=None, residual=None, act=0, out_st=None, out=None):
        b = self._f32(bias) if bias is not None else None
        nat.check(self._L.linetr_debug_gemm_st(
            self._h, A1.data_ptr(), K1, A2.data_ptr() if A2 is not None else None, K2, W.data_ptr(),
            b.data_ptr() if b is not None else None, residual.data_ptr() if residual is not None else None,
            out_st.data_ptr() if out_st is not None else None, out.data_ptr() if out is not None else None,
            out.stride(0) if out is not None else 0, M, N, int(act), self._stream()), self._L)
        return out_st if out_st is not None else out

    def set_profiling(self, on: bool):
        nat.check(self._L.linetr_set_profiling(self._h, int(on)), self._L)

    def get_profile(self):
        arr = (nat.ProfileEntry * 64)()
        n = C.c_int32()
        nat.check(self._L.linetr_get_profile(self._h, arr, 64, C.byref(n)), self._L)
        return [dict(name=arr[i].name.decode(), calls=arr[i].calls, ms=arr[i].ms, flops=arr[i].flops,
                     bytes=arr[i].bytes) for i in range(min(n.value, 64))]


class DescribePipeline:

    def __init__(self, engine: "Engine", depth: int = 2):
        if not 2 <= depth <= engine._L.linetr_pipeline_max_slots():
            raise ValueError(f"depth must be 2 .. {engine._L.linetr_pipeline_max_slots()}")
        self.eng, self.depth = engine, int(depth)
        self.i = 0
        self.inflight = []

    def _join(self, entry):
        slot, (tb, ld) = entry
        if tb.K > 0 and tb.N > 0:
            self.eng.describe_join(slot)
        return tb, ld

    def submit(self, *args, **kw):
        slot = self.i % self.depth
        self.i += 1
        self.inflight.append((slot, self.eng.describe_lines(*args, pipeline_slot=(slot, self.depth), **kw)))
        return self._join(self.inflight.pop(0)) if len(self.inflight) >= self.depth else None

    def drain(self):
        out = [self._join(e) for e in self.inflight]
        self.inflight = []
        return out

    def __del__(self):
        try:
            self.drain()
        except Exception:
            pass
```

Baseline: 10.44 million line-descriptors/s.

## Sample descriptor taps from LDS-staged NCHW planes instead of an NHWC relayout

For NCHW dense maps that fit in LDS, a new kernel stages 8 channel planes per block in shared memory and bilinearly samples every token and CLS row into a compact per-row buffer. This replaces the full NHWC transpose of the dense map. The desc output and the cls_pool taps then read the pre-sampled rows rather than gathering four taps from the map. The change aims to remove the layout pass and the scattered 4-tap global gathers, at the cost of a large-LDS kernel with 1024 threads per block and an extra rows buffer.

```diff
diff --git a/include/linetr_hip.h b/include/linetr_hip.h
--- a/include/linetr_hip.h
+++ b/include/linetr_hip.h
@@ -257,6 +257,10 @@
                           const float* d_map, int32_t dense_is_nhwc, int32_t Hc, int32_t Wc, int32_t align_corners,
                           const float* d_desc_dense, float* d_pooled, int32_t* kernel_used, void* stream);
 
+int linetr_debug_sample_rows(LinetrHandle* h, const LinetrLineRec* d_recs, int32_t K, const int32_t* d_sub2line, int32_t N, int32_t T,
+                             const float* d_cpnt, int64_t first_pad, int32_t n_images, const float* d_map_nchw, int32_t Hc, int32_t Wc,
+                             int32_t align_corners, float* d_rows, void* stream);
+
 #ifdef LINETR_EXPERIMENTS
 int64_t linetr_st_bytes(int64_t rows, int32_t K);
 int linetr_debug_to_st(LinetrHandle* h, const float* d_X, int32_t ld, int32_t rows, int32_t K, void* d_st, void* stream);
diff --git a/linetr_amd/_native.py b/linetr_amd/_native.py
--- a/linetr_amd/_native.py
+++ b/linetr_amd/_native.py
@@ -134,6 +134,7 @@
     L.linetr_debug_sig_attention.argtypes = [vp, i32, i32, vp, i32, vp, i32, vp, vp, vp]
     L.linetr_debug_tok_mlp.argtypes = [vp, i32, vp, vp, i64, vp, vp, vp, i64, vp, vp, i32, vp, vp]
     L.linetr_debug_cls_pool.argtypes = [vp, i32, vp, i32, vp, i32, i32, vp, vp, i64, i32, vp, i32, i32, i32, i32, vp, vp, vp, vp]
+    L.linetr_debug_sample_rows.argtypes = [vp, vp, i32, vp, i32, i32, vp, i64, i32, vp, i32, i32, i32, vp, vp]
     if hasattr(L, "linetr_debug_gemm_st"):
         L.linetr_st_bytes.argtypes = [i64, i32]
         L.linetr_st_bytes.restype = i64
@@ -165,7 +166,7 @@
            "linetr_prefilter_batch", "linetr_prefilter_tied_images", "linetr_pack_lines", "linetr_tokenize_workspace_bytes", "linetr_tokenize", "linetr_forward_workspace_bytes",
            "linetr_forward", "linetr_bn_stats_floats", "linetr_forward_train_workspace_bytes", "linetr_forward_train", "linetr_describe_workspace_bytes", "linetr_describe", "linetr_describe_submit", "linetr_describe_join", "linetr_pipeline_max_slots", "linetr_match_workspace_bytes", "linetr_match", "linetr_match_gathered", "linetr_match_points",
            "linetr_match_distmat", "linetr_match_distmat_workspace_bytes", "linetr_match_distmat_f64", "linetr_match_distmat_f64_workspace_bytes", "linetr_pair_tail_workspace_bytes", "linetr_pair_tail_output_bytes", "linetr_pair_tail", "linetr_val_step_workspace_bytes", "linetr_val_step_output_bytes", "linetr_val_step", "linetr_assign_from_matches", "linetr_gt_assign_workspace_bytes", "linetr_gt_assign", "linetr_superpoint_heads", "linetr_superpoint_keypoints_workspace_bytes", "linetr_superpoint_keypoints",
-           "linetr_point_descriptors_workspace_bytes", "linetr_point_descriptors", "linetr_set_precision", "linetr_get_precision", "linetr_debug_posenc", "linetr_debug_gemm", "linetr_debug_gemm_case", "linetr_debug_sig_attention", "linetr_debug_tok_mlp", "linetr_debug_cls_pool", "linetr_allgather_desc", "linetr_set_allgather_fn", "linetr_pack_slab", "linetr_sample_descriptors_workspace_bytes",
+           "linetr_point_descriptors_workspace_bytes", "linetr_point_descriptors", "linetr_set_precision", "linetr_get_precision", "linetr_debug_posenc", "linetr_debug_gemm", "linetr_debug_gemm_case", "linetr_debug_sig_attention", "linetr_debug_tok_mlp", "linetr_debug_cls_pool", "linetr_debug_sample_rows", "linetr_allgather_desc", "linetr_set_allgather_fn", "linetr_pack_slab", "linetr_sample_descriptors_workspace_bytes",
            "linetr_sample_descriptors", "linetr_pool_distmat_workspace_bytes", "linetr_pool_distmat", "linetr_pool_distmat_dense_workspace_bytes", "linetr_pool_distmat_dense", "linetr_set_profiling", "linetr_get_profile"]
 
 
diff --git a/linetr_amd/csrc/linetr_net.hip b/linetr_amd/csrc/linetr_net.hip
--- a/linetr_amd/csrc/linetr_net.hip
+++ b/linetr_amd/csrc/linetr_net.hip
@@ -235,6 +235,19 @@
   return LINETR_OK;
 }
 
+constexpr int64_t SR_LDS_MAX = 160 * 1024;
+bool sample_rows_fits(int Hc, int Wc) { return Hc > 0 && Wc > 0 && sample_rows_lds_bytes(Hc, Wc) <= SR_LDS_MAX; }
+
+int sample_rows_launch(LinetrHandle* h, hipStream_t st, const float* cpnt, const LinetrLineRec* recs, const int* s2l_g, const int* cu_sub,
+                       int64_t first_pad, int n_images, const float* nchw, int Hc, int Wc, int align_corners, float* rows) {
+  LT_HIP(allow_dynamic_lds<sample_rows_nchw_kernel>((int)SR_LDS_MAX));
+  ProfScope ps(h, st, "sample_desc", 0, ((double)n_images * Hc * Wc + (double)(first_pad + n_images)) * D * 4);
+  hipLaunchKernelGGL(sample_rows_nchw_kernel, dim3((unsigned)n_images * SR_GROUPS), dim3(SR_THREADS), (size_t)sample_rows_lds_bytes(Hc, Wc), st,
+                     cpnt, recs, s2l_g, cu_sub, first_pad, nchw, Hc, Wc, align_corners, rows);
+  LT_LAUNCH_CHECK();
+  return LINETR_OK;
+}
+
 struct TokenFront {
   const LinetrLineRec* recs; int K, N; double td; int T;
   const float *dense_desc, *dense_score;
@@ -246,9 +259,11 @@
   bool map_always;
   double tokenize_bytes;
   float *cpnt = nullptr, *cscore = nullptr; int n_pad_images = 0; int64_t first_pad = 0;
+  float* rows_buf = nullptr;
+  const int* cu_sub = nullptr;
 };
 int token_front(LinetrHandle* h, hipStream_t st, const TokenFront& a, const LinetrTokens& out, const K2sTable& k2s, int32_t* d_sub2line,
-                const float*& nhwc) {
+                const float*& nhwc, const float*& trows) {
   {
     ProfScope ps(h, st, "line_fill", 0, (double)a.K * 80 + (double)a.N * 8);
     hipLaunchKernelGGL(line_fill_kernel, dim3(cdiv(a.K, 256)), dim3(256), 0, st, a.recs, a.K, a.clip_x, a.clip_y, out.klines, out.length,
@@ -263,7 +278,20 @@
     LT_LAUNCH_CHECK();
   }
   const int Hc = a.height / 8, Wc = a.width / 8;
-  nhwc = nullptr;
+  nhwc = trows = nullptr;
+  if (a.rows_buf) {
+    if (int e = sample_rows_launch(h, st, a.cpnt, a.recs, a.s2l_g, a.cu_sub, a.first_pad, a.n_images, a.dense_desc, Hc, Wc, a.align_corners,
+                                   a.rows_buf)) return e;
+    trows = a.rows_buf;
+    if (out.desc) {
+      const int64_t ntok = (int64_t)a.N * a.T;
+      ProfScope ps(h, st, "desc_from_rows", 0, (double)ntok * D * 4 * 2);
+      hipLaunchKernelGGL(desc_from_rows_kernel, dim3((unsigned)((ntok + 3) / 4)), dim3(256), 0, st, trows, a.s2l_g, a.recs, ntok, a.T,
+                         a.first_pad, out.desc);
+      LT_LAUNCH_CHECK();
+    }
+    return LINETR_OK;
+  }
   if (a.map_always || out.desc)
     if (int e = nhwc_map(h, st, a.dense_desc, a.dense_is_nhwc, a.n_images, Hc * Wc, a.nhwc_buf, nhwc)) return e;
   if (out.desc) {
@@ -308,8 +336,8 @@
   f.s2l_g = (int*)((char*)d_ws + align_up(n_images * P * D * 4, 256));
   f.map_always = false;
   f.tokenize_bytes = (double)N * T * 16;
-  const float* nhwc;
-  return token_front(h, st, f, out, k2s, d_sub2line, nhwc);
+  const float *nhwc, *trows;
+  return token_front(h, st, f, out, k2s, d_sub2line, nhwc, trows);
 }
 
 extern "C" int64_t linetr_sample_descriptors_workspace_bytes(int32_t Hc, int32_t Wc, int32_t dense_is_nhwc) {
@@ -425,6 +453,7 @@
 struct TokenStage {
   const float *pnt = nullptr, *score = nullptr, *desc = nullptr;
   const float *cpnt = nullptr, *cscore = nullptr, *nhwc = nullptr;
+  const float* trows = nullptr;
   const LinetrLineRec* recs = nullptr;
   const int* sub2line_g = nullptr;
   int64_t rows = 0;
@@ -584,14 +613,20 @@
                     float* pooled) {
   const int64_t rows = ts.rows;
   if (kernel != POOLK_DENSE) {
-    const double tap_bytes = std::min((double)n_images * ts.Hc * ts.Wc * D * 4, (double)rows * D * 4 * 4);
+    const double tap_bytes = ts.trows ? (double)rows * D * 4 : std::min((double)n_images * ts.Hc * ts.Wc * D * 4, (double)rows * D * 4 * 4);
     ProfScope ps(h, st, "cls_pool_online", 2.0 * rows * (2.0 * HEADS * D * 2), tap_bytes + (double)rows * D * 4 + (double)N * HEADS * POOLW * 4);
-    if (kernel == POOLK_SPLIT4)
-      hipLaunchKernelGGL(cls_pool_online_kernel<4>, dim3(N), dim3(256), 0, st, ts.recs, ts.sub2line_g, ts.cpnt,
-                         a4, ts.first_pad, N, T, ts.nhwc, ts.Hc, ts.Wc, ts.align_corners, h->pool, pooled, 0);
-    else
-      hipLaunchKernelGGL(cls_pool_online_kernel<1>, dim3(cdiv(N, 4)), dim3(256), 0, st, ts.recs, ts.sub2line_g, ts.cpnt,
-                         a4, ts.first_pad, N, T, ts.nhwc, ts.Hc, ts.Wc, ts.align_corners, h->pool, pooled, kernel == POOLK_ONLINE_REV ? 1 : 0);
+    const int reverse = kernel == POOLK_ONLINE_REV ? 1 : 0;
+    auto launch = [&](auto kern, unsigned blocks, const float* src) {
+      hipLaunchKernelGGL(kern, dim3(blocks), dim3(256), 0, st, ts.recs, ts.sub2line_g, ts.cpnt, a4, ts.first_pad, N, T, src, ts.Hc, ts.Wc,
+                         ts.align_corners, h->pool, pooled, reverse);
+    };
+    if (kernel == POOLK_SPLIT4) {
+      if (ts.trows) launch(cls_pool_online_kernel<4, true>, N, ts.trows);
+      else launch(cls_pool_online_kernel<4, false>, N, ts.nhwc);
+    } else {
+      if (ts.trows) launch(cls_pool_online_kernel<1, true>, cdiv(N, 4), ts.trows);
+      else launch(cls_pool_online_kernel<1, false>, cdiv(N, 4), ts.nhwc);
+    }
     LT_LAUNCH_CHECK();
   } else {
     ProfScope ps(h, st, "cls_pool", 2.0 * rows * (2.0 * HEADS * D * 2), (double)rows * D * 8);
@@ -805,13 +840,13 @@
 
 
 namespace {
-struct DescWs { float *nhwc, *cpnt, *cscore, *sublines, *resp, *angle_sub; int* s2l_g; int64_t fwd_off, total; };
+struct DescWs { float *map, *cpnt, *cscore, *sublines, *resp, *angle_sub; int* s2l_g; int64_t fwd_off, total; };
 DescWs desc_layout(int n_images, int height, int width, int N, int64_t rows, char* base) {
   DescWs d;
   int64_t off = 0;
   auto take = [&](int64_t bytes) { char* p = base + off; off += align_up(bytes, 256); return p; };
   const int64_t P = (int64_t)(height / 8) * (width / 8);
-  d.nhwc = (float*)take(n_images * P * D * 4);
+  d.map = (float*)take(sample_rows_fits(height / 8, width / 8) ? rows * D * 4 : n_images * P * D * 4);
   d.cpnt = (float*)take(rows * 8);
   d.cscore = (float*)take(rows * 4);
   d.sublines = (float*)take((int64_t)N * 16);
@@ -861,14 +896,16 @@
   TokenFront f{d_recs, K, N, td, T, d_dense_desc, d_dense_score, n_images, height, width, align_corners, dense_is_nhwc,
                (double)width - 0.6, (double)height - 0.6, out.sublines ? out.sublines : dw.sublines, out.resp ? out.resp : dw.resp,
                out.angle_sub ? out.angle_sub : dw.angle_sub};
-  f.s2l_g = dw.s2l_g; f.nhwc_buf = dw.nhwc;
+  f.s2l_g = dw.s2l_g;
+  if (!dense_is_nhwc && sample_rows_fits(height / 8, width / 8)) { f.rows_buf = dw.map; f.cu_sub = cu_dev; }
+  else f.nhwc_buf = dw.map;
   f.map_always = true;
   f.tokenize_bytes = (double)n_real * 16;
   f.cpnt = dw.cpnt; f.cscore = dw.cscore; f.n_pad_images = n_images; f.first_pad = n_real;
-  const float* nhwc_map;
-  if (int e = token_front(h, st, f, out, k2s, d_sub2line, nhwc_map)) return e;
+  const float *nhwc_map, *trows;
+  if (int e = token_front(h, st, f, out, k2s, d_sub2line, nhwc_map, trows)) return e;
   TokenStage ts;
-  ts.cpnt = dw.cpnt; ts.cscore = dw.cscore; ts.nhwc = nhwc_map; ts.recs = d_recs; ts.sub2line_g = dw.s2l_g;
+  ts.cpnt = dw.cpnt; ts.cscore = dw.cscore; ts.nhwc = nhwc_map; ts.trows = trows; ts.recs = d_recs; ts.sub2line_g = dw.s2l_g;
   ts.rows = rows; ts.first_pad = n_real; ts.Hc = height / 8; ts.Wc = width / 8; ts.align_corners = align_corners;
   ts.pipe = pipe;
   if (int e = pipe_boundary(pipe, CUT_TOKENS, st)) return e;
@@ -1166,6 +1203,70 @@
   return e;
 }
 
+namespace {
+int check_compact_list(const char* who, hipStream_t st, const LinetrLineRec* d_recs, int K, const int32_t* d_sub2line, int N, int T,
+                       int64_t first_pad, int n_images, std::vector<int32_t>* cu_sub) {
+  std::vector<LinetrLineRec> recs(K);
+  std::vector<int32_t> s2l(N);
+  LT_HIP(hipStreamSynchronize(st));
+  LT_HIP(hipMemcpy(recs.data(), d_recs, (size_t)K * sizeof(LinetrLineRec), hipMemcpyDeviceToHost));
+  LT_HIP(hipMemcpy(s2l.data(), d_sub2line, (size_t)N * sizeof(int32_t), hipMemcpyDeviceToHost));
+  bool ordered = true;
+  for (int n = 0; n < N; ++n) {
+    if (s2l[n] < 0 || s2l[n] >= K) return fail(LINETR_E_ARG, "%s: sub-line %d maps to key-line %d, outside [0, %d)", who, n, s2l[n], K);
+    const LinetrLineRec& r = recs[s2l[n]];
+    const int64_t j = (int64_t)n - r.first_sub;
+    if (j < 0 || j >= r.n_sub || j * T >= r.n_tok)
+      return fail(LINETR_E_ARG, "%s: sub-line %d is not one of key-line %d's (first_sub %d, n_sub %d, n_tok %d)", who, n, s2l[n], r.first_sub, r.n_sub, r.n_tok);
+    if (r.first_tok < 0 || (int64_t)r.first_tok + r.n_tok > first_pad)
+      return fail(LINETR_E_ARG, "%s: key-line %d's tokens [%d, %d + %d) reach past first_pad = %lld", who, s2l[n], r.first_tok, r.first_tok, r.n_tok, (long long)first_pad);
+    if (r.image < 0 || r.image >= n_images) return fail(LINETR_E_ARG, "%s: key-line %d's image %d outside [0, %d)", who, s2l[n], r.image, n_images);
+    if (n > 0) {
+      const LinetrLineRec& q = recs[s2l[n - 1]];
+      ordered = ordered && q.image <= r.image && q.first_tok <= r.first_tok;
+    }
+  }
+  if (cu_sub) {
+    cu_sub->clear();
+    if (ordered) {
+      cu_sub->assign(n_images + 1, 0);
+      for (int n = 0; n < N; ++n) ++(*cu_sub)[recs[s2l[n]].image + 1];
+      for (int i = 0; i < n_images; ++i) (*cu_sub)[i + 1] += (*cu_sub)[i];
+    }
+  }
+  return LINETR_OK;
+}
+}
+
+extern "C" int linetr_debug_sample_rows(LinetrHandle* h, const LinetrLineRec* d_recs, int32_t K, const int32_t* d_sub2line, int32_t N,
+                                        int32_t T, const float* d_cpnt, int64_t first_pad, int32_t n_images, const float* d_map_nchw,
+                                        int32_t Hc, int32_t Wc, int32_t align_corners, float* d_rows, void* stream) {
+  if (!h) return fail(LINETR_E_ARG, "debug_sample_rows: null handle");
+  if (N < 0 || K < 0 || T < 1 || T > 4096) return fail(LINETR_E_ARG, "debug_sample_rows: bad sub-line count / max_tokens");
+  if (n_images < 1 || Hc < 1 || Wc < 1 || first_pad < 0 || first_pad > INT32_MAX / 8 || (int64_t)n_images * Hc * Wc > INT32_MAX / D)
+    return fail(LINETR_E_ARG, "debug_sample_rows: bad shape");
+  if (!sample_rows_fits(Hc, Wc))
+    return fail(LINETR_E_ARG, "debug_sample_rows: %d planes of a %d x %d map do not fit the LDS (linetr_describe takes the layout pass there)", SR_CH, Hc, Wc);
+  if (!d_cpnt || !d_map_nchw || !d_rows || (N > 0 && (!d_recs || !d_sub2line))) return fail(LINETR_E_ARG, "debug_sample_rows: null tensor");
+  if ((uintptr_t)d_recs % 8 || ((uintptr_t)d_sub2line | (uintptr_t)d_cpnt | (uintptr_t)d_map_nchw) % 4 || (uintptr_t)d_rows % 16)
+    return fail(LINETR_E_ARG, "debug_sample_rows: misaligned tensor (rows 16 bytes, records 8, the others 4)");
+  LT_HIP(hipSetDevice(h->device));
+  hipStream_t st = (hipStream_t)stream;
+  std::vector<int32_t> cu(n_images + 1, 0);
+  if (N > 0) {
+    if (int e = check_compact_list("debug_sample_rows", st, d_recs, K, d_sub2line, N, T, first_pad, n_images, &cu)) return e;
+    if (cu.empty()) return fail(LINETR_E_ARG, "debug_sample_rows: the sub-lines are not ordered by image and token");
+  }
+  int* d_cu = nullptr;
+  LT_HIP(hipMalloc((void**)&d_cu, cu.size() * sizeof(int32_t)));
+  int e = LINETR_OK;
+  if (hipMemcpy(d_cu, cu.data(), cu.size() * sizeof(int32_t), hipMemcpyHostToDevice) != hipSuccess) e = fail(LINETR_E_HIP, "debug_sample_rows: upload failed");
+  if (!e) e = sample_rows_launch(h, st, d_cpnt, d_recs, d_sub2line, d_cu, first_pad, n_images, d_map_nchw, Hc, Wc, align_corners, d_rows);
+  (void)hipStreamSynchronize(st);
+  (void)hipFree(d_cu);
+  return e;
+}
+
 extern "C" int linetr_debug_cls_pool(LinetrHandle* h, int32_t kernel, const LinetrLineRec* d_recs, int32_t K, const int32_t* d_sub2line,
                                      int32_t N, int32_t T, const float* d_cpnt, const float* d_a4, int64_t first_pad, int32_t n_images,
                                      const float* d_map, int32_t dense_is_nhwc, int32_t Hc, int32_t Wc, int32_t align_corners,
@@ -1198,28 +1299,24 @@
   if ((uintptr_t)d_recs % 8 || ((uintptr_t)d_sub2line | (uintptr_t)d_cpnt | (uintptr_t)d_map) % 4 || (dense_is_nhwc && (uintptr_t)d_map % 16))
     return fail(LINETR_E_ARG, "debug_cls_pool: misaligned tensor (records 8 bytes, an NHWC map 16, the others 4)");
   LT_HIP(hipSetDevice(h->device));
-  {
-    std::vector<LinetrLineRec> recs(K);
-    std::vector<int32_t> s2l(N);
-    LT_HIP(hipStreamSynchronize(st));
-    LT_HIP(hipMemcpy(recs.data(), d_recs, (size_t)K * sizeof(LinetrLineRec), hipMemcpyDeviceToHost));
-    LT_HIP(hipMemcpy(s2l.data(), d_sub2line, (size_t)N * sizeof(int32_t), hipMemcpyDeviceToHost));
-    for (int n = 0; n < N; ++n) {
-      if (s2l[n] < 0 || s2l[n] >= K) return fail(LINETR_E_ARG, "debug_cls_pool: sub-line %d maps to key-line %d, outside [0, %d)", n, s2l[n], K);
-      const LinetrLineRec& r = recs[s2l[n]];
-      const int64_t j = (int64_t)n - r.first_sub;
-      if (j < 0 || j >= r.n_sub || j * T >= r.n_tok)
-        return fail(LINETR_E_ARG, "debug_cls_pool: sub-line %d is not one of key-line %d's (first_sub %d, n_sub %d, n_tok %d)", n, s2l[n], r.first_sub, r.n_sub, r.n_tok);
-      if (r.first_tok < 0 || (int64_t)r.first_tok + r.n_tok > first_pad)
-        return fail(LINETR_E_ARG, "debug_cls_pool: key-line %d's tokens [%d, %d + %d) reach past first_pad = %lld", s2l[n], r.first_tok, r.first_tok, r.n_tok, (long long)first_pad);
-      if (r.image < 0 || r.image >= n_images) return fail(LINETR_E_ARG, "debug_cls_pool: key-line %d's image %d outside [0, %d)", s2l[n], r.image, n_images);
-    }
-  }
+  std::vector<int32_t> cu;
+  if (int e = check_compact_list("debug_cls_pool", st, d_recs, K, d_sub2line, N, T, first_pad, n_images, &cu)) return e;
+  const bool from_rows = !dense_is_nhwc && sample_rows_fits(Hc, Wc) && !cu.empty();
   float* buf = nullptr;
-  if (!dense_is_nhwc) LT_HIP(hipMalloc((void**)&buf, (size_t)n_images * Hc * Wc * D * sizeof(float)));
+  const int64_t rows_bytes = align_up((first_pad + n_images) * D * 4, 256);
+  if (from_rows) LT_HIP(hipMalloc((void**)&buf, (size_t)(rows_bytes + cu.size() * sizeof(int32_t))));
+  else if (!dense_is_nhwc) LT_HIP(hipMalloc((void**)&buf, (size_t)n_images * Hc * Wc * D * sizeof(float)));
   ts.cpnt = d_cpnt; ts.recs = d_recs; ts.sub2line_g = d_sub2line; ts.rows = first_pad + n_images; ts.first_pad = first_pad;
   ts.Hc = Hc; ts.Wc = Wc; ts.align_corners = align_corners;
-  int e = nhwc_map(h, st, d_map, dense_is_nhwc, n_images, Hc * Wc, buf, ts.nhwc);
+  int e = LINETR_OK;
+  if (from_rows) {
+    int* d_cu = (int*)((char*)buf + rows_bytes);
+    if (hipMemcpy(d_cu, cu.data(), cu.size() * sizeof(int32_t), hipMemcpyHostToDevice) != hipSuccess) e = fail(LINETR_E_HIP, "debug_cls_pool: upload failed");
+    if (!e) e = sample_rows_launch(h, st, d_cpnt, d_recs, d_sub2line, d_cu, first_pad, n_images, d_map, Hc, Wc, align_corners, buf);
+    ts.trows = buf;
+  } else {
+    e = nhwc_map(h, st, d_map, dense_is_nhwc, n_images, Hc * Wc, buf, ts.nhwc);
+  }
   if (!e) e = cls_pool_launch(h, st, kernel, ts, n_images, N, T, d_a4, d_pooled);
   (void)hipStreamSynchronize(st);
   if (buf) (void)hipFree(buf);
diff --git a/linetr_amd/csrc/lt_model.h b/linetr_amd/csrc/lt_model.h
--- a/linetr_amd/csrc/lt_model.h
+++ b/linetr_amd/csrc/lt_model.h
@@ -271,7 +271,8 @@
   }
 }
 
-template <int SPLIT>
+constexpr int ROW_AHEAD = 2;
+template <int SPLIT, bool ROWS = false>
 __global__ __launch_bounds__(256, 3) void cls_pool_online_kernel(
     const LinetrLineRec* __restrict__ recs, const int* __restrict__ sub2line_g, const float* __restrict__ cpnt,
     const float* __restrict__ a4, int64_t first_pad, int N, int T, const float* __restrict__ nhwc, int Hc, int Wc,
@@ -288,7 +289,6 @@
   const int ntk = n_valid + (n_pad > 0 ? 1 : 0);
   const int64_t tok0 = (int64_t)r.first_tok + (int64_t)j * T;
   const int64_t padrow = first_pad + r.image;
-  const float* nhwc_img = nhwc + (int64_t)r.image * Hc * Wc * D;
   f32x4 u[4], u2[4];
 #pragma unroll
   for (int h = 0; h < 4; ++h) {
@@ -305,35 +305,7 @@
     ab[h] = f32x4{0.f, 0.f, 0.f, 0.f};
   }
   auto row_of = [&](int jj) -> int64_t { return jj < n_valid ? tok0 + jj : padrow; };
-  int t_off[4];
-  float t_w[4];
-  auto fill_taps = [&](int chunk) {
-    const int jj = chunk + lane;
-    const int64_t row = row_of(jj < ntk ? jj : ntk - 1);
-    tap_coords(cpnt[row * 2], cpnt[row * 2 + 1], Hc, Wc, align_corners, t_off, t_w);
-  };
-  auto issue = [&](int jj, TapSet& t, f32x4& a) {
-    int off[4];
-    float wt[4];
-#pragma unroll
-    for (int k = 0; k < 4; ++k) {
-      off[k] = __builtin_amdgcn_readlane(t_off[k], jj & 63);
-      wt[k] = __builtin_bit_cast(float, __builtin_amdgcn_readlane(__builtin_bit_cast(int, t_w[k]), jj & 63));
-    }
-    taps_load(nhwc_img, off, wt, lane, t);
-    a = *reinterpret_cast<const f32x4*>(a4 + row_of(jj) * D + lane * 4);
-  };
-  TapSet cur, nxt;
-  f32x4 a_cur, a_nxt;
-  const int jj0 = SPLIT == 1 ? 0 : wv;
-  fill_taps(0);
-  if (jj0 < ntk) issue(jj0, cur, a_cur);
-  for (int jj = jj0; jj < ntk; jj += SPLIT) {
-    if (jj + SPLIT < ntk) {
-      if (((jj + SPLIT) >> 6) != (jj >> 6)) fill_taps((jj + SPLIT) & ~63);
-      issue(jj + SPLIT, nxt, a_nxt);
-    }
-    const f32x4 dv = taps_finish<true>(cur);
+  auto absorb = [&](int jj, const f32x4& dv, const f32x4& a_cur) {
     const float mult = jj < n_valid ? 1.f : (float)n_pad;
     float sc[4];
 #pragma unroll
@@ -363,8 +335,63 @@
         ab[h][c] += e * a_cur[c];
       }
     }
-    cur = nxt;
-    a_cur = a_nxt;
+  };
+  const int jj0 = SPLIT == 1 ? 0 : wv;
+  if constexpr (ROWS) {
+    const float* rows = nhwc;
+    f32x4 d_q[ROW_AHEAD], a_q[ROW_AHEAD];
+    auto issue = [&](int jj, f32x4& d, f32x4& a) {
+      const int64_t row = row_of(jj);
+      d = *reinterpret_cast<const f32x4*>(rows + row * D + lane * 4);
+      a = *reinterpret_cast<const f32x4*>(a4 + row * D + lane * 4);
+    };
+#pragma unroll
+    for (int i = 0; i < ROW_AHEAD; ++i)
+      if (jj0 + i * SPLIT < ntk) issue(jj0 + i * SPLIT, d_q[i], a_q[i]);
+    for (int jb = jj0; jb < ntk; jb += ROW_AHEAD * SPLIT) {
+#pragma unroll
+      for (int i = 0; i < ROW_AHEAD; ++i) {
+        const int jj = jb + i * SPLIT;
+        if (jj < ntk) {
+          const f32x4 d_cur = d_q[i], a_cur = a_q[i];
+          if (jj + ROW_AHEAD * SPLIT < ntk) issue(jj + ROW_AHEAD * SPLIT, d_q[i], a_q[i]);
+          absorb(jj, desc_normalize<true>(d_cur), a_cur);
+        }
+      }
+    }
+  } else {
+    const float* nhwc_img = nhwc + (int64_t)r.image * Hc * Wc * D;
+    int t_off[4];
+    float t_w[4];
+    auto fill_taps = [&](int chunk) {
+      const int jj = chunk + lane;
+      const int64_t row = row_of(jj < ntk ? jj : ntk - 1);
+      tap_coords(cpnt[row * 2], cpnt[row * 2 + 1], Hc, Wc, align_corners, t_off, t_w);
+    };
+    auto issue = [&](int jj, TapSet& t, f32x4& a) {
+      int off[4];
+      float wt[4];
+#pragma unroll
+      for (int k = 0; k < 4; ++k) {
+        off[k] = __builtin_amdgcn_readlane(t_off[k], jj & 63);
+        wt[k] = __builtin_bit_cast(float, __builtin_amdgcn_readlane(__builtin_bit_cast(int, t_w[k]), jj & 63));
+      }
+      taps_load(nhwc_img, off, wt, lane, t);
+      a = *reinterpret_cast<const f32x4*>(a4 + row_of(jj) * D + lane * 4);
+    };
+    TapSet cur, nxt;
+    f32x4 a_cur, a_nxt;
+    fill_taps(0);
+    if (jj0 < ntk) issue(jj0, cur, a_cur);
+    for (int jj = jj0; jj < ntk; jj += SPLIT) {
+      if (jj + SPLIT < ntk) {
+        if (((jj + SPLIT) >> 6) != (jj >> 6)) fill_taps((jj + SPLIT) & ~63);
+        issue(jj + SPLIT, nxt, a_nxt);
+      }
+      absorb(jj, taps_finish<true>(cur), a_cur);
+      cur = nxt;
+      a_cur = a_nxt;
+    }
   }
   float* out = pooled + (int64_t)n * 4 * POOLW;
   if constexpr (SPLIT > 1) {
diff --git a/linetr_amd/csrc/lt_token.h b/linetr_amd/csrc/lt_token.h
--- a/linetr_amd/csrc/lt_token.h
+++ b/linetr_amd/csrc/lt_token.h
@@ -173,7 +173,7 @@
   return __builtin_fmaf(g + 1.f, (float)size / 2.f, -0.5f);
 }
 
-__device__ __forceinline__ void tap_coords(float px, float py, int Hc, int Wc, int align_corners, int (&off)[4],
+__device__ __forceinline__ void tap_coords(float px, float py, int Hc, int Wc, int align_corners, int ld, int (&off)[4],
                                            float (&wt)[4]) {
 #pragma clang fp contract(off)
   const float s = 8.f;
@@ -191,9 +191,42 @@
     const int yy = y0 + (k >> 1), xx = x0 + (k & 1);
     const bool in = xx >= 0 && xx < Wc && yy >= 0 && yy < Hc;
     const int yc = min(max(yy, 0), Hc - 1), xc = min(max(xx, 0), Wc - 1);
-    off[k] = yc * Wc + xc;
+    off[k] = yc * ld + xc;
     wt[k] = in ? wv[k] : 0.f;
   }
+}
+
+__device__ __forceinline__ void tap_coords(float px, float py, int Hc, int Wc, int align_corners, int (&off)[4],
+                                           float (&wt)[4]) {
+  tap_coords(px, py, Hc, Wc, align_corners, Wc, off, wt);
+}
+
+__device__ __forceinline__ float taps_combine(float nw, float ne, float sw, float se, const float (&w)[4]) {
+#pragma clang fp contract(off)
+  float v = nw * w[0];
+  v = __builtin_fmaf(ne, w[1], v);
+  v = __builtin_fmaf(sw, w[2], v);
+  v = __builtin_fmaf(se, w[3], v);
+  return v;
+}
+
+template <bool RCP = false>
+__device__ __forceinline__ f32x4 desc_normalize(f32x4 o) {
+#pragma clang fp contract(off)
+  float sq = 0.f;
+#pragma unroll
+  for (int c = 0; c < 4; ++c) sq += o[c] * o[c];
+  sq = wave_sum(sq);
+  const float nrm = fmaxf(sqrtf(sq), 1e-12f);
+  if constexpr (RCP) {
+    const float inv = 1.f / nrm;
+#pragma unroll
+    for (int c = 0; c < 4; ++c) o[c] = o[c] * inv;
+  } else {
+#pragma unroll
+    for (int c = 0; c < 4; ++c) o[c] = o[c] / nrm;
+  }
+  return o;
 }
 
 __device__ __forceinline__ void taps_load(const float* __restrict__ nhwc_img, const int (&off)[4], const float (&wt)[4],
@@ -216,29 +249,10 @@
 
 template <bool RCP = false>
 __device__ __forceinline__ f32x4 taps_finish(const TapSet& t) {
-#pragma clang fp contract(off)
   f32x4 o;
-  float sq = 0.f;
-#pragma unroll
-  for (int c = 0; c < 4; ++c) {
-    float v = t.v[0][c] * t.w[0];
-    v = __builtin_fmaf(t.v[1][c], t.w[1], v);
-    v = __builtin_fmaf(t.v[2][c], t.w[2], v);
-    v = __builtin_fmaf(t.v[3][c], t.w[3], v);
-    o[c] = v;
-    sq += v * v;
-  }
-  sq = wave_sum(sq);
-  const float nrm = fmaxf(sqrtf(sq), 1e-12f);
-  if constexpr (RCP) {
-    const float inv = 1.f / nrm;
-#pragma unroll
-    for (int c = 0; c < 4; ++c) o[c] = o[c] * inv;
-  } else {
-#pragma unroll
-    for (int c = 0; c < 4; ++c) o[c] = o[c] / nrm;
-  }
-  return o;
+#pragma unroll
+  for (int c = 0; c < 4; ++c) o[c] = taps_combine(t.v[0][c], t.v[1][c], t.v[2][c], t.v[3][c], t.w);
+  return desc_normalize<RCP>(o);
 }
 
 __device__ __forceinline__ f32x4 sample_one(float px, float py, const float* __restrict__ nhwc_img, int Hc, int Wc,
@@ -292,6 +306,87 @@
   *reinterpret_cast<f32x4*>(desc + tok * D + lane * 4) = o;
 }
 
+constexpr int SR_CH = 8;
+constexpr int SR_THREADS = 1024;
+constexpr int SR_GROUPS = D / SR_CH;
+static_assert(SR_GROUPS == 32, "the block -> (image, channel group) map below is written for 32 groups");
+__host__ __device__ inline int sample_rows_ld(int Wc) { return Wc + ((11 - (Wc & 7)) & 7); }
+inline int64_t sample_rows_lds_bytes(int Hc, int Wc) { return (int64_t)SR_CH * Hc * sample_rows_ld(Wc) * 4; }
+
+__global__ __launch_bounds__(SR_THREADS) void sample_rows_nchw_kernel(
+    const float* __restrict__ cpnt, const LinetrLineRec* __restrict__ recs, const int* __restrict__ sub2line_g,
+    const int* __restrict__ cu_sub, int64_t first_pad, const float* __restrict__ nchw, int Hc, int Wc, int align_corners,
+    float* __restrict__ rows) {
+  extern __shared__ __attribute__((aligned(16))) float sr_planes[];
+  const int tid = threadIdx.x;
+  const int img = blockIdx.x >> 5, grp = (blockIdx.x & 7) * 4 + ((blockIdx.x >> 3) & 3);
+  const int ld = sample_rows_ld(Wc), plane = Hc * ld;
+  const int s0 = cu_sub[img], s1 = cu_sub[img + 1];
+  int64_t t0 = 0, t1 = 0;
+  if (s1 > s0) {
+    const LinetrLineRec z = recs[sub2line_g[s1 - 1]];
+    t0 = recs[sub2line_g[s0]].first_tok;
+    t1 = (int64_t)z.first_tok + z.n_tok;
+  }
+  t0 = t0 > 0 ? t0 : 0;
+  t1 = t1 < first_pad ? t1 : first_pad;
+  const int nt = t1 > t0 ? (int)(t1 - t0) : 0;
+  {
+    const float* src = nchw + ((int64_t)img * D + grp * SR_CH) * Hc * Wc;
+    const bool vec = (Wc & 3) == 0 && ((uintptr_t)nchw & 15) == 0;
+    const int Wq = (Wc + 3) >> 2, nq = SR_CH * Hc * Wq;
+    const int drp = SR_THREADS / Wq, dxq = SR_THREADS - drp * Wq;
+    int rp = tid / Wq, xq = tid - rp * Wq;
+    for (int q = tid; q < nq; q += SR_THREADS) {
+      const int x = xq * 4;
+      const float* g = src + (int64_t)rp * Wc + x;
+      float* l = sr_planes + rp * ld + x;
+      f32x4 v;
+      if (vec) v = *reinterpret_cast<const f32x4*>(g);
+      else {
+#pragma unroll
+        for (int k = 0; k < 4; ++k) v[k] = x + k < Wc ? g[k] : 0.f;
+      }
+#pragma unroll
+      for (int k = 0; k < 4; ++k)
+        if (x + k < Wc) l[k] = v[k];
+      rp += drp;
+      xq += dxq;
+      if (xq >= Wq) { xq -= Wq; ++rp; }
+    }
+  }
+  __syncthreads();
+  for (int j = tid; j <= nt; j += SR_THREADS) {
+    const int64_t row = j < nt ? t0 + j : first_pad + img;
+    int off[4];
+    float wt[4];
+    tap_coords(cpnt[row * 2], cpnt[row * 2 + 1], Hc, Wc, align_corners, ld, off, wt);
+    f32x4 o[SR_CH / 4];
+#pragma unroll
+    for (int c = 0; c < SR_CH; ++c) {
+      const float* pl = sr_planes + c * plane;
+      o[c >> 2][c & 3] = taps_combine(pl[off[0]], pl[off[1]], pl[off[2]], pl[off[3]], wt);
+    }
+    float* dst = rows + row * D + grp * SR_CH;
+#pragma unroll
+    for (int i = 0; i < SR_CH / 4; ++i) *reinterpret_cast<f32x4*>(dst + i * 4) = o[i];
+  }
+}
+
+__global__ __launch_bounds__(256) void desc_from_rows_kernel(const float* __restrict__ rows, const int* __restrict__ sub2line_g,
+                                                             const LinetrLineRec* __restrict__ recs, int64_t n_slots, int T,
+                                                             int64_t first_pad, float* __restrict__ desc) {
+  const int64_t slot = (int64_t)blockIdx.x * 4 + (threadIdx.x >> 6);
+  if (slot >= n_slots) return;
+  const int lane = threadIdx.x & 63;
+  const int n = (int)(slot / T);
+  const LinetrLineRec r = recs[sub2line_g[n]];
+  const int ti = (n - r.first_sub) * T + (int)(slot - (int64_t)n * T);
+  const int64_t row = ti < r.n_tok ? (int64_t)r.first_tok + ti : first_pad + r.image;
+  const f32x4 o = desc_normalize<false>(*reinterpret_cast<const f32x4*>(rows + row * D + lane * 4));
+  *reinterpret_cast<f32x4*>(desc + slot * D + lane * 4) = o;
+}
+
 constexpr int KP_DESC_N = 64;
 constexpr int KP_DESC_LS = KP_DESC_N + 1;
 constexpr size_t KP_DESC_LDS = (size_t)D * KP_DESC_LS * 4;
diff --git a/linetr_amd/engine.py b/linetr_amd/engine.py
--- a/linetr_amd/engine.py
+++ b/linetr_amd/engine.py
@@ -1080,6 +1080,22 @@
                                                 ptr(desc_dense), ptr(out), C.byref(used), self._stream()), self._L)
         return out, used.value
 
+    def debug_sample_rows(self, recs, sub2line, N, T, cpnt, first_pad, n_images, dense_nchw, Hc, Wc, out, *, align_corners=False):
+        for t in (cpnt, dense_nchw, out):
+            if t.dtype != torch.float32 or t.device != self.device or not t.is_contiguous():
+                raise ValueError("contiguous float32 tensors on the engine's device expected")
+        rows = first_pad + n_images
+        if out.numel() < rows * D or cpnt.numel() < rows * 2 or dense_nchw.numel() < n_images * Hc * Wc * D:
+            raise ValueError("out / cpnt / dense_nchw are smaller than first_pad + n_images rows / n_images maps")
+        if N and (recs.dtype != torch.uint8 or sub2line.dtype != torch.int32 or sub2line.numel() < N):
+            raise ValueError("recs: uint8 bytes of LineRec[K]; sub2line: int32 [N]")
+        ptr = lambda t: t.data_ptr() if t is not None else None
+        nat.check(self._L.linetr_debug_sample_rows(self._h, ptr(recs), recs.numel() // nat.REC_DTYPE.itemsize if recs is not None else 0,
+                                                   ptr(sub2line), int(N), int(T), cpnt.data_ptr(), int(first_pad), int(n_images),
+                                                   dense_nchw.data_ptr(), int(Hc), int(Wc), int(bool(align_corners)), out.data_ptr(),
+                                                   self._stream()), self._L)
+        return out
+
     def to_st(self, X):
         X = self._f32(X)
         rows, K = X.shape
```

Result: no change. 10.44 million line-descriptors/s (median of 2 runs) (-0.0%).
